# wzf2000/GAMER

Hardware: AMD Instinct MI355X
Metric: train-step sequences/sec, Qwen3Multi SMB decoder, his_len=100 (higher is better)
Workload: dtype f32 tensors/accumulators, products = 3 x fp16 pieces (split3)

## Files before the change

gamer_amd/_lib.py:

```python
from __future__ import annotations

import ctypes as C
import os
import re
from typing import Optional

import torch

_HERE = os.path.dirname(os.path.abspath(__file__))
LIB_PATH = os.path.join(_HERE, "lib", "libgamer_hip.so")
if os.environ.get("GAMER_LIB_PATH"):
    LIB_PATH = os.path.abspath(os.environ["GAMER_LIB_PATH"])
HEADER_PATH = os.path.join(os.path.dirname(_HERE), "include", "gamer_hip.h")

_lib: Optional[C.CDLL] = None

c_void_p, c_int, c_float, c_int64, c_uint64 = C.c_void_p, C.c_int, C.c_float, C.c_int64, C.c_uint64


class GemmDesc(C.Structure):
    _fields_ = [
        ("A", c_void_p), ("a_rs", c_int64), ("a_ks", c_int64),
        ("B", c_void_p), ("b_rs", c_int64), ("b_ks", c_int64),
        ("C", c_void_p), ("ldc", c_int64),
        ("M", c_int), ("N", c_int), ("K", c_int),
        ("alpha", c_float),
        ("accumulate", c_int),
        ("groups", c_int),
        ("group_mode", c_int),
        ("group_offsets", c_void_p),
        ("strideB", c_int64), ("strideC", c_int64),
        ("kchunk", c_int),
        ("resid", c_void_p),
        ("row_map", c_void_p),
        ("p_drop", c_float),
        ("seed", c_uint64),
        ("rowdot_other", c_void_p),
        ("rowdot_out", c_void_p),
        ("rowdot_S", c_int),
        ("qk_wq", c_void_p), ("qk_wk", c_void_p),
        ("qk_eps", c_float),
        ("qk_cos", c_void_p), ("qk_sin", c_void_p),
        ("qk_bias_q", c_void_p), ("qk_bias_k", c_void_p), ("qk_bias_v", c_void_p),
        ("qk_act_idx", c_void_p),
        ("qk_pos_ids", c_void_p),
        ("qk_q_rot", c_void_p), ("qk_k_rot", c_void_p),
        ("qk_S", c_int), ("qk_nq", c_int), ("qk_nkv", c_int),
        ("b_planes", c_void_p), ("b_plane_stride", c_int64),
        ("amax_a", c_void_p), ("amax_b", c_void_p),
        ("amax_c", c_void_p), ("amax_c_col0", c_int),
        ("wgrad_ws", c_void_p), ("wgrad_ws_floats", c_int64),
        ("sw_gu", c_void_p), ("sw_ld", c_int64),
        ("group_div", c_int), ("sw_tbl", c_void_p), ("b_planes_t", c_void_p),
        ("sw_hm", c_void_p), ("sw_row_group", c_void_p),
        ("norm_x", c_void_p), ("norm_w", c_void_p), ("norm_eps", c_float),
        ("norm_dst_rows", c_void_p), ("norm_src_rows", c_void_p),
        ("bias_idx", c_void_p), ("bias_q", c_void_p), ("bias_k", c_void_p), ("bias_v", c_void_p),
        ("bias_rows", c_int), ("bias_nq", c_int), ("bias_nkv", c_int),
    ]


class GemmBf16Desc(C.Structure):
    _fields_ = [
        ("A", c_void_p), ("lda", c_int64),
        ("B", c_void_p), ("ldb", c_int64),
        ("C", c_void_p), ("ldc", c_int64),
        ("M", c_int), ("N", c_int), ("K", c_int),
        ("accumulate", c_int),
        ("groups", c_int),
        ("group_mode", c_int),
        ("group_offsets", c_void_p),
        ("strideB", c_int64), ("strideC", c_int64),
        ("kchunk", c_int),
        ("resid", c_void_p),
        ("row_map", c_void_p),
        ("p_drop", c_float),
        ("seed", c_uint64),
        ("rowdot_other", c_void_p),
        ("rowdot_out", c_void_p),
        ("rowdot_S", c_int),
        ("qk_wq", c_void_p), ("qk_wk", c_void_p), ("qk_eps", c_float),
        ("qk_cos", c_void_p), ("qk_sin", c_void_p),
        ("qk_bias_q", c_void_p), ("qk_bias_k", c_void_p), ("qk_bias_v", c_void_p),
        ("qk_act_idx", c_void_p), ("qk_pos_ids", c_void_p),
        ("qk_q_rot", c_void_p), ("qk_k_rot", c_void_p),
        ("qk_S", c_int), ("qk_nq", c_int), ("qk_nkv", c_int),
        ("sw_gu", c_void_p), ("sw_ld", c_int64),
        ("wgrad_ws", c_void_p), ("wgrad_ws_floats", c_int64),
    ]


P, I, F, L, U = c_void_p, c_int, c_float, c_int64, c_uint64

_SIGNATURES = {
    "gamer_router_fwd": [P, P, P, P, I, I, I, I, I, I, P, P, P, P, P, P, P, P, P, P, P, P],
    "gamer_expert_lists": [P, I, I, I, P, P, P, P, P],
    "gamer_causal_prep": [P, I, I, P, P, P, P, P, P],
    "gamer_session_prep": [P, P, P, I, I, I, I, P, P, P, P, P, P, P],
    "gamer_moe_router_prep": [P, P, P, I, P, I, I, I, I, I, I, I, P, P, P, P, P, P, P, P, P],
    "gamer_embedding_fwd": [P, P, I, I, I, P, P],
    "gamer_embedding_bwd": [P, P, I, I, I, I, P, P],
    "gamer_embedding_bwd_ordered": [P, P, I, I, I, I, P, P, L, P],
    "gamer_embedding_bwd_ordered_ws_bytes": [I, I, I],
    "gamer_rmsnorm_fwd": [P, P, I, I, F, P, P, I, P],
    "gamer_rmsnorm_bwd": [P, P, P, I, P, I, I, F, I, P, P, I, P, P, F, U, P],
    "gamer_colsum_reduce": [P, I, I, I, P, P],
    "gamer_colsum_reduce_batched": [P, L, I, I, I, P, I, P],
    "gamer_rowtable_fwd": [P, P, P, I, I, P, I, I, P],
    "gamer_rowtable_bwd": [P, I, I, P, P, I, I, I, P, P, L, P],
    "gamer_gemm_f32": [C.POINTER(GemmDesc), P],
    "gamer_gemm_f32_split": [C.POINTER(GemmDesc), c_int, P],
    "gamer_split3_guard": [I],
    "gamer_gemm_bf16": [C.POINTER(GemmBf16Desc), P],
    "gamer_cast_params_bf16": [P, P, P, P, I, I, P],
    "gamer_attn_fwd_bf16": [P, I, P, I, P, I, P, P, I, I, I, I, F, F, U, P, P, P, P, P, P, P],
    "gamer_attn_bwd_bf16": [P, I, P, I, P, I, P, P, P, P, P, I, I, I, I, F, F, U, P, P, I, P, I, P, I, P, I, P, P, P, P],
    "gamer_session_spans": [P, P, P, P, P, I, I, I, I, P, P, P, P, P, P, P, P, P],
    "gamer_qknorm_rope_fwd": [P, I, I, I, I, P, P, F, P, P, P, P, P, P, P, P, P, P],
    "gamer_qknorm_rope_bwd": [P, P, P, I, I, I, I, P, P, F, P, P, P, P, P, I, P, P, P, P, P, P, P, P, L, P],
    "gamer_attn_row_order": [P, I, I, P, P, P, P],
    "gamer_attn_fwd": [P, I, P, I, P, I, P, P, P, P, I, I, I, I, F, F, U, P, P, P, P, P, I, P, P],
    "gamer_attn_bwd": [P, I, P, I, P, I, P, P, P, P, P, P, P, I, I, I, I, F, F, U, P, P, I, P, I, P, I, P, P, P, P, P, I, P],
    "gamer_split3_planes": [P, P, L, L, P],
    "gamer_absmax_f32": [P, I, L, I, I, L, P, P],
    "gamer_absmax_multi_f32": [P, P, I, P, P],
    "gamer_split2h_planes_multi": [P, P, I, P, P, P],
    "gamer_amax_sink": [P, P],
    "gamer_amax_sink3": [P, P, P],
    "gamer_attn_split_amax": [P, P, P, P],
    "gamer_attn_fwd_split": [P, I, P, I, P, I, P, P, P, I, I, I, I, F, F, U, P, P, P, P, P, I, P, P],
    "gamer_attn_bwd_split": [P, I, P, I, P, I, P, P, P, P, P, P, P, I, I, I, I, F, F, U, P, P, I, P, I, P, I, P, P, P, I, P, P, P],
    "gamer_residual_dropout_fwd": [P, P, P, I, I, F, U, P, P],
    "gamer_residual_dropout_bwd": [P, P, I, I, F, U, P, P],
    "gamer_swiglu_fwd": [P, P, L, F, U, P, P],
    "gamer_swiglu_bwd": [P, P, P, L, F, U, P],
    "gamer_swiglu_fwd_ld": [P, L, I, I, F, U, P, P],
    "gamer_swiglu_bwd_ld": [P, L, I, I, P, F, U, P],
    "gamer_swiglu_fwd_ld_tbl": [P, L, I, I, F, U, P, P, P, P],
    "gamer_pba_router": [P, I, I, I, I, I, I, I, P, I, I, I, I, I, P, P, P, P, P],
    "gamer_relu_tbl_fwd": [P, L, I, I, F, U, P, P, P, I, P],
    "gamer_relu_tbl_bwd": [P, L, I, I, P, F, U, P, P, I, P],
# ... 156 lines not shown
```

gamer_amd/csrc/common.h:

```cpp
#pragma once
#include <hip/hip_runtime.h>
#include <stdint.h>
#include <stdio.h>
#include <stdarg.h>
#include <stdlib.h>
#include <atomic>
#include <type_traits>

#include "../../include/gamer_hip.h"

namespace gamer {

void set_error(const char* fmt, ...);

#define GAMER_CHECK_ARG(cond, ...)                       \
    do {                                                 \
        if (!(cond)) {                                   \
            gamer::set_error(__VA_ARGS__);               \
            return -1;                                   \
        }                                                \
    } while (0)

#define GAMER_CHECK_LAUNCH(name)                                                        \
    do {                                                                                \
// ... 221 lines not shown
struct AttnDropout {
    uint32_t k0, k1, thr;
    float scale;
    __device__ __forceinline__ AttnDropout(float p, uint64_t seed) {
        k0 = mix32((uint32_t)seed ^ 0x9e3779b9U) ^ mix32((uint32_t)(seed >> 32) + 0x7f4a7c15U);
        k1 = mix32(k0 + 0x632be5abU);
        const float t = p * 4294967296.f;
        thr = t >= 4294967040.f ? 0xffffffffU : (uint32_t)t;
        scale = p > 0.f ? 1.f / (1.f - p) : 1.f;
    }
    __device__ __forceinline__ uint32_t row_word(uint32_t row) const {
        return (mix32(row * 0x9e3779b1U + k0) & 0xffffffU) | 0x800001U;
    }
    __device__ __forceinline__ uint32_t key_word(uint32_t j) const { return mix32(j * 0x85ebca6bU + k1) & 0xffffffU; }
    __device__ __forceinline__ bool keep(uint32_t a, uint32_t b) const { return __umul24(a, b) >= thr; }
};

__device__ __forceinline__ float xor32_max(float v) {
    const auto sw = __builtin_amdgcn_permlane32_swap(__float_as_uint(v), __float_as_uint(v), false, false);
    return fmaxf(__uint_as_float(sw[0]), __uint_as_float(sw[1]));
}
__device__ __forceinline__ float xor32_sum(float v) {
    const auto sw = __builtin_amdgcn_permlane32_swap(__float_as_uint(v), __float_as_uint(v), false, false);
    return __uint_as_float(sw[0]) + __uint_as_float(sw[1]);
}

__device__ __forceinline__ int wave_sum_i32(int v) {
#pragma unroll
    for (int o = 32; o > 0; o >>= 1) v += __shfl_xor(v, o, 64);
    return v;
}
__device__ __forceinline__ int wave_max_i32(int v) {
#pragma unroll
    for (int o = 32; o > 0; o >>= 1) v = max(v, __shfl_xor(v, o, 64));
    return v;
}
__device__ __forceinline__ int wave_min_i32(int v) {
#pragma unroll
    for (int o = 32; o > 0; o >>= 1) v = min(v, __shfl_xor(v, o, 64));
    return v;
}

#define GAMER_DPP_ROW_REDUCE(OP, v)                                                                   \
    v = OP(v, __builtin_amdgcn_update_dpp(v, v, 0xB1, 0xf, 0xf, false));      \
    v = OP(v, __builtin_amdgcn_update_dpp(v, v, 0x4E, 0xf, 0xf, false));      \
    v = OP(v, __builtin_amdgcn_update_dpp(v, v, 0x141, 0xf, 0xf, false));         \
    v = OP(v, __builtin_amdgcn_update_dpp(v, v, 0x140, 0xf, 0xf, false));
__device__ __forceinline__ int wave_min_i32_dpp(int v) {
    GAMER_DPP_ROW_REDUCE(min, v)
    return min(min(__builtin_amdgcn_readlane(v, 0), __builtin_amdgcn_readlane(v, 16)),
               min(__builtin_amdgcn_readlane(v, 32), __builtin_amdgcn_readlane(v, 48)));
}
__device__ __forceinline__ int wave_max_i32_dpp(int v) {
    GAMER_DPP_ROW_REDUCE(max, v)
    return max(max(__builtin_amdgcn_readlane(v, 0), __builtin_amdgcn_readlane(v, 16)),
               max(__builtin_amdgcn_readlane(v, 32), __builtin_amdgcn_readlane(v, 48)));
}

__device__ __forceinline__ float row16_sum_dpp(float v) {
#define GAMER_DPP_F(ctrl) __int_as_float(__builtin_amdgcn_update_dpp(__float_as_int(v), __float_as_int(v), ctrl, 0xf, 0xf, false))
    v += GAMER_DPP_F(0xB1);
    v += GAMER_DPP_F(0x4E);
    v += GAMER_DPP_F(0x141);
    v += GAMER_DPP_F(0x140);
#undef GAMER_DPP_F
    return v;
}

__device__ __forceinline__ float sigmoid_f(float x) { return __builtin_amdgcn_rcpf(1.f + __expf(-x)); }
__device__ __forceinline__ float silu_f(float x) { return x * sigmoid_f(x); }
__device__ __forceinline__ float dsilu_f(float x) {
    const float s = sigmoid_f(x);
    return s * (1.f + x * (1.f - s));
}

bool gemm_as_eligible(const gamer_gemm_desc* d, bool a_kc, bool b_kc, const uint16_t* b_planes);
int launch_gemm_as(const gamer_gemm_desc* d, const uint16_t* b_planes, bool b_kc, hipStream_t st);
int launch_gemm_bias_rows(const gamer_gemm_desc* d, hipStream_t st);
bool gemm_os_eligible(const gamer_gemm_desc* d, bool a_kc, bool b_kc, const uint16_t* b_planes);
int launch_gemm_os(const gamer_gemm_desc* d, const uint16_t* b_planes, int guard, hipStream_t st, bool fwd_t = false);
bool gemm_os_fwd_eligible(const gamer_gemm_desc* d, bool a_kc, bool b_kc);
bool gemm_wg_eligible(const gamer_gemm_desc* d, bool a_kc, bool b_kc);
int launch_gemm_wg(const gamer_gemm_desc* d, hipStream_t st);

int launch_wgrad_reduce(const float* ws, float* C, int64_t ldc, int M, int N, int groups, const int32_t* group_offsets, int K,
                        int kchunk, int64_t strideC, hipStream_t st);

}
```

gamer_amd/csrc/gemm.hip:

```cpp
#include "common.h"
#include <stdlib.h>

namespace gamer {

constexpr int BM = 128, BN = 128, BK = 32;
constexpr int GEMM_THREADS = 256;
constexpr int KC_LD = BK + 4;
constexpr int TILE_FLOATS = BM * KC_LD;
constexpr int GEMM_LDS_BYTES = 4 * TILE_FLOATS * (int)sizeof(float);

typedef float f32x16 __attribute__((ext_vector_type(16)));

constexpr int SP_KC_ROW = 80;
constexpr int SP_KC_IMG = BM * SP_KC_ROW;
constexpr int SP_RC_IMG = BK * 256;
constexpr int SP_OPERAND = 3 * SP_KC_IMG;
constexpr int SP_LDS_BYTES = 2 * SP_OPERAND;

#ifndef SP_ABLATE
#define SP_ABLATE 0
#endif
__device__ __forceinline__ uint32_t pack_hi16(uint32_t w0, uint32_t w1) { return __builtin_amdgcn_perm(w1, w0, 0x07060302u); }
__device__ __forceinline__ void split3(float x, uint32_t (&w)[3]) {
    if (SP_ABLATE & 1) { w[0] = w[1] = w[2] = __float_as_uint(x); return; }
// ... 105 lines not shown
__device__ __forceinline__ bf16x8 read_frag_half(const unsigned char* __restrict__ img, int rbase, int lane) {
    const int r32 = lane & 31, h = lane >> 5;
    if (KC) {
        return *reinterpret_cast<const bf16x8*>(img + (rbase + r32) * SPH_KC_ROW + (h << 4));
    } else {
        const int q = (lane >> 2) & 3, pp = lane & 3, gsel = (lane >> 4) & 1;
        const int row = rbase + 16 * gsel + 4 * pp;
        bf16x8 out;
#pragma unroll
        for (int c = 0; c < 2; ++c) {
            const int k = 8 * h + 4 * c + q;
            const bf16x4 v = __builtin_amdgcn_ds_read_tr16_b64_v4bf16(
                (bf16x4 __attribute__((address_space(3)))*)(img + sp_rc_off(k, row)));
            out[4 * c + 0] = v[0]; out[4 * c + 1] = v[1]; out[4 * c + 2] = v[2]; out[4 * c + 3] = v[3];
        }
        return out;
    }
}

template <bool KC>
__device__ __forceinline__ bf16x8 read_frag_split(const unsigned char* __restrict__ img, int rbase, int sub, int lane) {
    const int r32 = lane & 31, h = lane >> 5;
    if (KC) {
        return *reinterpret_cast<const bf16x8*>(img + (rbase + r32) * SP_KC_ROW + ((2 * sub + h) << 4));
    } else {
        const int q = (lane >> 2) & 3, pp = lane & 3, gsel = (lane >> 4) & 1;
        const int row = rbase + 16 * gsel + 4 * pp;
        bf16x8 out;
#pragma unroll
        for (int c = 0; c < 2; ++c) {
            const int k = 16 * sub + 8 * h + 4 * c + q;
            const bf16x4 v = __builtin_amdgcn_ds_read_tr16_b64_v4bf16(
                (bf16x4 __attribute__((address_space(3)))*)(img + sp_rc_off(k, row)));
            out[4 * c + 0] = v[0]; out[4 * c + 1] = v[1]; out[4 * c + 2] = v[2]; out[4 * c + 3] = v[3];
        }
        return out;
    }
}

__device__ unsigned long long* g_gemm_stamp = nullptr;
__device__ __forceinline__ unsigned long long stamp_now() {
    unsigned long long t;
    asm volatile("s_memtime %0\n\ts_waitcnt lgkmcnt(0)" : "=s"(t) :: "memory");
    return t;
}

struct GemmParams {
    const float* A; int64_t a_rs, a_ks;
    const float* B; int64_t b_rs, b_ks;
    float* C; int64_t ldc;
    int M, N, K;
    float alpha;
    int accumulate;
    int groups;
    const int32_t* group_offsets;
    int64_t strideB, strideC;
    int kchunk;
    int m_tiles, n_tiles;
    const float* resid;
    const int32_t* row_map;
    float p_drop;
    uint64_t seed;
    const float* rowdot_other;
    float* rowdot_out;
    int rowdot_S;
    const float* qk_wq; const float* qk_wk;
    float qk_eps;
    const float* qk_cos; const float* qk_sin;
    const float* qk_bias_q; const float* qk_bias_k; const float* qk_bias_v;
    const int32_t* qk_act_idx;
    const int32_t* qk_pos_ids;
    float* qk_q_rot; float* qk_k_rot;
    int qk_S, qk_nq, qk_nkv;
    const uint32_t* amax_a; const uint32_t* amax_b;
    const uint16_t* b_planes;
    int64_t b_plane_stride;
    int guard;
    uint32_t* amax_c;
    int amax_c_col0;
    float* wgrad_ws;
    float* sw_gu; int64_t sw_ld;
    int group_div;
    const float* sw_tbl;
};

constexpr float SPLIT3_GUARD_RATIO = 1.f / 65536.f;
#ifndef GAMER_GEMM_CAMAX_BUILD
#define GAMER_GEMM_CAMAX_BUILD 1
#endif
#ifndef GAMER_SPLIT3_GUARD_BUILD
#define GAMER_SPLIT3_GUARD_BUILD 1
#endif
static int g_split3_guard = 1;

__device__ __forceinline__ int xcd_remap(int id, int n) {
    const int q = n >> 3, r = n & 7;
    const int xcd = id & 7, idx = id >> 3;
    const int base = xcd < r ? xcd * (q + 1) : r * (q + 1) + (xcd - r) * q;
    return base + idx;
}

template <bool INTERIOR>
__device__ __forceinline__ void load_kc(const float* __restrict__ p, int64_t rs, int row0, int row_end, int k0,
                                        int k_end, int tid, float4 (&r)[4]) {
#pragma unroll
    for (int j = 0; j < 4; ++j) {
        const int f = tid + GEMM_THREADS * j;
        const int row = row0 + (f >> 3);
        const int k = k0 + ((f & 7) << 2);
        if (INTERIOR) {
            r[j] = *reinterpret_cast<const float4*>(p + (int64_t)row * rs + k);
            continue;
        }
        float4 v = make_float4(0.f, 0.f, 0.f, 0.f);
        if (row < row_end && k < k_end) {
            v = *reinterpret_cast<const float4*>(p + (int64_t)row * rs + k);
            if (k + 3 >= k_end) {
                if (k + 1 >= k_end) v.y = 0.f;
                if (k + 2 >= k_end) v.z = 0.f;
                v.w = 0.f;
            }
        }
        r[j] = v;
    }
}
template <bool INTERIOR>
__device__ __forceinline__ void load_rc(const float* __restrict__ p, int64_t ks, int row0, int row_end, int k0,
                                        int k_end, int tid, float4 (&r)[4]) {
#pragma unroll
    for (int j = 0; j < 4; ++j) {
        const int f = tid + GEMM_THREADS * j;
        const int k = k0 + (f >> 5);
        const int row = row0 + ((f & 31) << 2);
        if (INTERIOR) {
            r[j] = *reinterpret_cast<const float4*>(p + (int64_t)k * ks + row);
            continue;
        }
        float4 v = make_float4(0.f, 0.f, 0.f, 0.f);
        if (k < k_end && row < row_end) {
            v = *reinterpret_cast<const float4*>(p + (int64_t)k * ks + row);
            if (row + 3 >= row_end) {
                if (row + 1 >= row_end) v.y = 0.f;
                if (row + 2 >= row_end) v.z = 0.f;
                v.w = 0.f;
            }
        }
        r[j] = v;
    }
}
__device__ __forceinline__ void store_kc(float* __restrict__ lds, int tid, const float4 (&r)[4]) {
#pragma unroll
    for (int j = 0; j < 4; ++j) {
        const int f = tid + GEMM_THREADS * j;
        *reinterpret_cast<float4*>(lds + (f >> 3) * KC_LD + ((f & 7) << 2)) = r[j];
    }
}
__device__ __forceinline__ void store_rc(float* __restrict__ lds, int tid, const float4 (&r)[4]) {
#pragma unroll
    for (int j = 0; j < 4; ++j) {
        const int f = tid + GEMM_THREADS * j;
        *reinterpret_cast<float4*>(lds + (f >> 5) * BM + ((f & 31) << 2)) = r[j];
    }
}

template <bool KC>
__device__ __forceinline__ void read_frag(const float* __restrict__ lds, int row, int kk, int h, float (&f)[4]) {
    if (KC) {
        const float4 v = *reinterpret_cast<const float4*>(lds + row * KC_LD + 8 * kk + 4 * h);
        f[0] = v.x; f[1] = v.y; f[2] = v.z; f[3] = v.w;
    } else {
#pragma unroll
        for (int s = 0; s < 4; ++s) f[s] = lds[(8 * kk + 4 * h + s) * BM + row];
    }
}

template <bool A_KC, bool B_KC, int MODE, bool ACCUM, bool STAMP, int NBUF, int EPI, int SPLIT = 0, bool PP = false>
__device__ __forceinline__ void
gemm_f32_tile(const GemmParams& p, float* __restrict__ smem_all, const int vblock, const int vgrid) {

    const int grp = PP ? (int)(threadIdx.x >> 8) : 0;
    const int tid = threadIdx.x & (GEMM_THREADS - 1);
    float* const smem = smem_all + (PP ? grp * (GEMM_LDS_BYTES / 4) : 0);
    const int lane = tid & 63;
    const int wid = tid >> 6;
    const int wm = wid >> 1, wn = wid & 1;
    const int r32 = lane & 31, h = lane >> 5;

    const int Lx = xcd_remap(vblock, vgrid);
    const int L = (PP && MODE == 0) ? 2 * Lx + grp : Lx;

    int row0, row_end;
    int col0;
    int kbeg, kend;
    const float* Bp = p.B;
    const float* Bsrc = p.B;
    float* Cp = p.C;
    int64_t ws_block = 0;
    int tile_group = 0;
    if (MODE == 0) {
        const int mt = L / p.n_tiles;
        col0 = (L % p.n_tiles) * BN;
        int g = 0, seg_beg = 0, seg_end = p.M, tiles_before = 0;
        bool found = false;
        if (p.group_offsets) {
            int prev = p.group_offsets[0];
            for (int gi = 0; gi < p.groups; ++gi) {
                const int nxt = p.group_offsets[gi + 1];
                const int tiles = (nxt - prev + BM - 1) / BM;
                if (!found && mt < tiles_before + tiles) {
                    g = gi; seg_beg = prev; seg_end = nxt; found = true;
                }
                if (!found) tiles_before += tiles;
                prev = nxt;
            }
        } else {
            found = mt < (p.M + BM - 1) / BM;
        }
        if (!found) return;
        row0 = seg_beg + (mt - tiles_before) * BM;
        row_end = seg_end;
        kbeg = 0;
        kend = p.K;
        tile_group = g;
        Bp += (int64_t)(g / p.group_div) * p.strideB;
        Bsrc = Bp;
        if (SPLIT == 3 && p.b_planes) Bp = reinterpret_cast<const float*>(p.b_planes) + (Bp - p.B);
    } else {
        const int tiles_mn = p.m_tiles * p.n_tiles;
        const int per_chunk = PP ? (tiles_mn + 1) / 2 : tiles_mn;
        const int chunk = L / per_chunk;
        const int tile = PP ? 2 * (L % per_chunk) + grp : L % per_chunk;
        if (PP && tile >= tiles_mn) return;
        ws_block = (int64_t)chunk * tiles_mn + tile;
        row0 = (tile / p.n_tiles) * BM;
        row_end = p.M;
        col0 = (tile % p.n_tiles) * BN;
        int g = 0, seg_beg = 0, seg_end = p.K, chunks_before = 0;
        bool found = false;
        if (p.group_offsets) {
            int prev = p.group_offsets[0];
            for (int gi = 0; gi < p.groups; ++gi) {
                const int nxt = p.group_offsets[gi + 1];
                const int chunks = (nxt - prev + p.kchunk - 1) / p.kchunk;
                if (!found && chunk < chunks_before + chunks) {
                    g = gi; seg_beg = prev; seg_end = nxt; found = true;
                }
                if (!found) chunks_before += chunks;
                prev = nxt;
            }
        } else {
            found = chunk < (p.K + p.kchunk - 1) / p.kchunk;
        }
        if (!found) return;
        kbeg = seg_beg + (chunk - chunks_before) * p.kchunk;
        kend = min(seg_end, kbeg + p.kchunk);
        Cp += (int64_t)g * p.strideC;
    }
    const int col_end = p.N;

    f32x16 acc[2][2];
#pragma unroll
    for (int i = 0; i < 2; ++i)
#pragma unroll
        for (int j = 0; j < 2; ++j)
#pragma unroll
            for (int r = 0; r < 16; ++r) acc[i][j][r] = 0.f;

    const int nkt = (kend - kbeg + BK - 1) / BK;
    const bool a_in = row0 + BM <= row_end, b_in = col0 + BN <= col_end;
    float4 ra[4], rb[4];
    float scale_a = 1.f, scale_b = 1.f, unscale = 1.f;
    constexpr bool GUARD = GAMER_SPLIT3_GUARD_BUILD && SPLIT == 3 && MODE == 0 && A_KC && !PP && !STAMP;
    float rmax[4] = {0.f, 0.f, 0.f, 0.f};
    uint32_t amax_a_bits = 0;
    if (SPLIT == 3) {
        float ia, ib;
        amax_a_bits = amax_read(p.amax_a);
        scale_from_amax(amax_a_bits, scale_a, ia);
        scale_from_amax(amax_read(p.amax_b), scale_b, ib);
        unscale = ia * ib;
    }
    auto load_tile = [&](int k0) {
        const bool k_in = k0 + BK <= kend;
        if (a_in && k_in) {
            if (A_KC) load_kc<true>(p.A, p.a_rs, row0, row_end, k0, kend, tid, ra);
            else load_rc<true>(p.A, p.a_ks, row0, row_end, k0, kend, tid, ra);
        } else {
            if (A_KC) load_kc<false>(p.A, p.a_rs, row0, row_end, k0, kend, tid, ra);
            else load_rc<false>(p.A, p.a_ks, row0, row_end, k0, kend, tid, ra);
        }
        if (b_in && k_in) {
            if (B_KC) load_kc<true>(Bp, p.b_rs, col0, col_end, k0, kend, tid, rb);
            else load_rc<true>(Bp, p.b_ks, col0, col_end, k0, kend, tid, rb);
        } else {
            if (B_KC) load_kc<false>(Bp, p.b_rs, col0, col_end, k0, kend, tid, rb);
            else load_rc<false>(Bp, p.b_ks, col0, col_end, k0, kend, tid, rb);
        }
    };
    constexpr int H2_B_OFF = 2 * (A_KC ? SP_KC_IMG : SP_RC_IMG);
    constexpr int H2_STAGE = H2_B_OFF + 2 * (B_KC ? SP_KC_IMG : SP_RC_IMG);
    auto store_tile_from = [&](float* dst, const float4 (&qa)[4], const float4 (&qb)[4]) {
        if (SPLIT == 3) {
            unsigned char* d8 = reinterpret_cast<unsigned char*>(dst);
            if (A_KC) store_kc_h2(d8, tid, qa, scale_a); else store_rc_h2(d8, tid, qa, scale_a);
            if (GUARD) {
#pragma unroll
// ... 397 lines not shown
            if (wave_live) {
                const int ar0 = row0 + wm * 64 + r32, bc0 = col0 + wn * 64 + r32;
#pragma unroll 1
                for (int k = kbeg; k < kend; k += 2) {
                    const int kk = k + h;
                    const bool kin = kk < kend;
                    float av[2], bv[2];
#pragma unroll
                    for (int i = 0; i < 2; ++i) {
                        const int row = ar0 + i * 32;
                        av[i] = (kin && row < row_end) ? p.A[(int64_t)row * p.a_rs + kk] : 0.f;
                    }
#pragma unroll
                    for (int j = 0; j < 2; ++j) {
                        const int col = bc0 + j * 32;
                        bv[j] = (kin && col < col_end) ? (B_KC ? Bsrc[(int64_t)col * p.b_rs + kk] : Bsrc[(int64_t)kk * p.b_ks + col]) : 0.f;
                    }
#pragma unroll
                    for (int i = 0; i < 2; ++i)
#pragma unroll
                        for (int j = 0; j < 2; ++j)
                            acc[i][j] = __builtin_amdgcn_mfma_f32_32x32x2f32(av[i], bv[j], acc[i][j], 0, 0, 0);
                }
            }
        }
    }

    const bool interior = a_in && b_in;
    const float alpha_eff = (SPLIT == 3 && !redo) ? p.alpha * unscale : p.alpha;
    if (MODE == 0 && (NBUF == 2 || SPLIT) && interior && (p.ldc & 3) == 0) {
        float* patch = smem + wid * (64 * 68);
        float4 oth[EPI == 2 ? 16 : 1];
        if (EPI == 2) {
            const float* ob = p.rowdot_other + (int64_t)(row0 + wm * 64 + (lane >> 4)) * p.ldc + col0 + wn * 64 + ((lane & 15) << 2);
#pragma unroll
            for (int it = 0; it < 16; ++it) oth[it] = *reinterpret_cast<const float4*>(ob + (int64_t)it * 4 * p.ldc);
        }
        if (SPLIT != 3 && p.alpha == 1.f) {
#pragma unroll
            for (int i = 0; i < 2; ++i)
#pragma unroll
                for (int j = 0; j < 2; ++j)
#pragma unroll
                    for (int r = 0; r < 16; ++r)
                        patch[(i * 32 + (r & 3) + 8 * (r >> 2) + 4 * h) * 68 + j * 32 + r32] = acc[i][j][r];
        } else {
#pragma unroll
            for (int i = 0; i < 2; ++i)
#pragma unroll
                for (int j = 0; j < 2; ++j)
#pragma unroll
                    for (int r = 0; r < 16; ++r)
                        patch[(i * 32 + (r & 3) + 8 * (r >> 2) + 4 * h) * 68 + j * 32 + r32] = alpha_eff * acc[i][j][r];
        }
        __builtin_amdgcn_s_waitcnt(0xc07f);
        const int c4 = (lane & 15) << 2;
        const DropoutRng rng((EPI == 1 || EPI == 4) ? p.p_drop : 0.f, p.seed);
        const int row_first = row0 + wm * 64 + (lane >> 4);
        const int col = col0 + wn * 64 + c4;
        float* dst0 = Cp + (int64_t)row_first * p.ldc + col;
        const int64_t step = 4 * p.ldc;
        const int qk_pos0 = EPI == 3 ? row_first % max(p.qk_S, 1) : 0;
        const bool amax_on = GAMER_GEMM_CAMAX_BUILD && p.amax_c != nullptr && !ACCUM && col0 + wn * 64 >= p.amax_c_col0;
        float cmax = 0.f;
        int pre_rc[EPI == 1 ? 16 : 1];
        float4 pre_x[EPI == 1 ? 16 : (EPI == 4 ? 8 : 1)], pre_b[EPI == 4 ? 8 : 1];
        if (EPI == 1) {
            if (p.row_map) {
#pragma unroll
                for (int it = 0; it < 16; ++it) pre_rc[it] = p.row_map[row_first + 4 * it];
            } else {
#pragma unroll
                for (int it = 0; it < 16; ++it) pre_rc[it] = row_first + 4 * it;
            }
#pragma unroll
            for (int it = 0; it < 16; ++it) pre_x[it] = *reinterpret_cast<const float4*>(p.resid + (int64_t)pre_rc[it] * p.ldc + col);
        }
        float4 tb_g = make_float4(0.f, 0.f, 0.f, 0.f), tb_u = tb_g;
        if (EPI == 4 && p.sw_tbl) {
            const float* tb = p.sw_tbl + (int64_t)tile_group * 2 * p.N + col;
            tb_g = *reinterpret_cast<const float4*>(tb);
            tb_u = *reinterpret_cast<const float4*>(tb + p.N);
        }
        auto pre_sw = [&](int it0) {
#pragma unroll
            for (int it = 0; it < 8; ++it) {
                const float* ga = p.sw_gu + (int64_t)(row_first + 4 * (it0 + it)) * p.sw_ld + col;
                pre_x[EPI == 4 ? it : 0] = *reinterpret_cast<const float4*>(ga);
                pre_b[EPI == 4 ? it : 0] = *reinterpret_cast<const float4*>(ga + p.N);
            }
        };
        if (EPI == 4) pre_sw(0);
#pragma unroll
        for (int it = 0; it < 16; ++it) {
            if (EPI == 4 && it == 8) pre_sw(8);
            const int lr = (lane >> 4) + 4 * it;
            const float4 v = *reinterpret_cast<const float4*>(patch + lr * 68 + c4);
            if (EPI == 3) {
                const int row = row_first + 4 * it;
                const int hd = (col0 + wn * 64) >> 6;
                const int g = lane & 15;
                float4 x = v;
                const bool cross = p.qk_bias_q != nullptr;
                const int a = cross ? p.qk_act_idx[row] : 0;
                if (hd < p.qk_nq + p.qk_nkv) {
                    const bool isq = hd < p.qk_nq;
                    if (cross) {
                        const float4 b4 = isq ? reinterpret_cast<const float4*>(p.qk_bias_q + (int64_t)a * p.qk_nq * 64 + hd * 64)[g]
                                              : reinterpret_cast<const float4*>(p.qk_bias_k + (int64_t)a * p.qk_nkv * 64 + (hd - p.qk_nq) * 64)[g];
                        x.x += b4.x; x.y += b4.y; x.z += b4.z; x.w += b4.w;
                    }
                    *reinterpret_cast<float4*>(dst0 + it * step) = x;
                    float ss = x.x * x.x + x.y * x.y + x.z * x.z + x.w * x.w;
                    ss = row16_sum_dpp(ss);
                    const float rstd = rsqrtf(ss * (1.f / 64.f) + p.qk_eps);
                    const float4 w4 = reinterpret_cast<const float4*>(isq ? p.qk_wq : p.qk_wk)[g];
                    float4 y;
                    y.x = w4.x * (x.x * rstd); y.y = w4.y * (x.y * rstd); y.z = w4.z * (x.z * rstd); y.w = w4.w * (x.w * rstd);
                    float4 pr;
                    pr.x = __shfl_xor(y.x, 8, 64); pr.y = __shfl_xor(y.y, 8, 64); pr.z = __shfl_xor(y.z, 8, 64); pr.w = __shfl_xor(y.w, 8, 64);
                    int pos = qk_pos0 + 4 * it;
                    if (p.qk_S >= 64) pos = pos >= p.qk_S ? pos - p.qk_S : pos;
                    else pos %= p.qk_S;
                    if (p.qk_pos_ids) pos = p.qk_pos_ids[row];
                    const float4 cc = reinterpret_cast<const float4*>(p.qk_cos + pos * 64)[g];
                    const float4 sn = reinterpret_cast<const float4*>(p.qk_sin + pos * 64)[g];
                    const float sgn = g < 8 ? -1.f : 1.f;
                    float4 o;
                    o.x = y.x * cc.x + sgn * pr.x * sn.x; o.y = y.y * cc.y + sgn * pr.y * sn.y;
                    o.z = y.z * cc.z + sgn * pr.z * sn.z; o.w = y.w * cc.w + sgn * pr.w * sn.w;
                    float* rot = isq ? p.qk_q_rot + (int64_t)row * p.qk_nq * 64 + hd * 64
                                     : p.qk_k_rot + (int64_t)row * p.qk_nkv * 64 + (hd - p.qk_nq) * 64;
                    *reinterpret_cast<float4*>(rot + 4 * g) = o;
                } else {
                    if (cross) {
                        const float4 b4 = reinterpret_cast<const float4*>(p.qk_bias_v + (int64_t)a * p.qk_nkv * 64 +
                                                                          (hd - p.qk_nq - p.qk_nkv) * 64)[g];
                        x.x += b4.x; x.y += b4.y; x.z += b4.z; x.w += b4.w;
                    }
                    *reinterpret_cast<float4*>(dst0 + it * step) = x;
                }
            } else if (EPI == 4) {
                const int row = row_first + 4 * it;
                float* ga = p.sw_gu + (int64_t)row * p.sw_ld + col;
                float* ua = ga + p.N;
                float4 a = pre_x[EPI == 4 ? (it & 7) : 0], b = pre_b[EPI == 4 ? (it & 7) : 0];
                a.x += tb_g.x; a.y += tb_g.y; a.z += tb_g.z; a.w += tb_g.w;
                b.x += tb_u.x; b.y += tb_u.y; b.z += tb_u.z; b.w += tb_u.w;
                float m[4];
                rng.mult4((uint32_t)(((int64_t)row * p.N + col) >> 2), m);
                const float d0 = m[0] * v.x, d1 = m[1] * v.y, d2 = m[2] * v.z, d3 = m[3] * v.w;
                float4 dg, du;
                dg.x = d0 * b.x * dsilu_f(a.x); du.x = d0 * silu_f(a.x);
                dg.y = d1 * b.y * dsilu_f(a.y); du.y = d1 * silu_f(a.y);
                dg.z = d2 * b.z * dsilu_f(a.z); du.z = d2 * silu_f(a.z);
                dg.w = d3 * b.w * dsilu_f(a.w); du.w = d3 * silu_f(a.w);
                *reinterpret_cast<float4*>(ga) = dg;
                *reinterpret_cast<float4*>(ua) = du;
                if (amax_on) {
                    asm("v_max3_f32 %0, %0, |%1|, |%2|\n\tv_max3_f32 %0, %0, |%3|, |%4|" : "+v"(cmax) : "v"(dg.x), "v"(dg.y), "v"(dg.z), "v"(dg.w));
                    asm("v_max3_f32 %0, %0, |%1|, |%2|\n\tv_max3_f32 %0, %0, |%3|, |%4|" : "+v"(cmax) : "v"(du.x), "v"(du.y), "v"(du.z), "v"(du.w));
                }
            } else if (EPI == 1) {
                const int64_t e = (int64_t)pre_rc[EPI == 1 ? it : 0] * p.ldc + col;
                float* dst = Cp + e;
                const float4 x = pre_x[EPI == 1 ? it : 0];
                float m[4];
                rng.mult4((uint32_t)(e >> 2), m);
                float4 o;
                o.x = x.x + m[0] * v.x; o.y = x.y + m[1] * v.y; o.z = x.z + m[2] * v.z; o.w = x.w + m[3] * v.w;
                *reinterpret_cast<float4*>(dst) = o;
            } else {
                float* dst = dst0 + it * step;
                if (EPI != 1 && EPI != 3 && amax_on)
                    asm("v_max3_f32 %0, %0, |%1|, |%2|\n\tv_max3_f32 %0, %0, |%3|, |%4|" : "+v"(cmax) : "v"(v.x), "v"(v.y), "v"(v.z), "v"(v.w));
                if (EPI == 2) {
                    const float4 o4 = oth[EPI == 2 ? it : 0];
                    float d = v.x * o4.x + v.y * o4.y + v.z * o4.z + v.w * o4.w;
                    d = row16_sum_dpp(d);
                    if ((lane & 15) == 0) {
                        const int row = row_first + 4 * it;
                        const int heads = p.N >> 6, head = (col0 + wn * 64) >> 6;
                        p.rowdot_out[((int64_t)(row / p.rowdot_S) * heads + head) * p.rowdot_S + row % p.rowdot_S] = d;
                    }
                }
                if (ACCUM) {
                    float4 o = *reinterpret_cast<const float4*>(dst);
                    o.x += v.x; o.y += v.y; o.z += v.z; o.w += v.w;
                    *reinterpret_cast<float4*>(dst) = o;
                } else {
                    *reinterpret_cast<float4*>(dst) = v;
                }
            }
        }
        if (EPI != 1 && EPI != 3 && amax_on) {
            uint32_t mw = __float_as_uint(cmax);
#pragma unroll
            for (int o2 = 32; o2 > 0; o2 >>= 1) mw = max(mw, (uint32_t)__shfl_xor((int)mw, o2, 64));
            if (lane == 0 && mw) amax_publish(mw, p.amax_c, (uint32_t)(vblock * 4 + wid));
        }
    } else if (MODE == 1 && p.wgrad_ws != nullptr) {
        float* blk = p.wgrad_ws + ws_block * (int64_t)(BM * BN);
#pragma unroll
        for (int i = 0; i < 2; ++i)
#pragma unroll
            for (int j = 0; j < 2; ++j) {
                const int lc = wn * 64 + j * 32 + r32;
                const int lr0 = wm * 64 + i * 32 + 4 * h;
#pragma unroll
                for (int r = 0; r < 16; ++r) blk[(lr0 + (r & 3) + 8 * (r >> 2)) * BN + lc] = alpha_eff * acc[i][j][r];
            }
    } else {
        float emax = 0.f;
        if (EPI == 4 && p.sw_tbl != nullptr) {
            const float* tb0 = p.sw_tbl + (int64_t)tile_group * 2 * p.N;
            const int nr = min(BM, row_end - row0), nc = min(BN, p.N - col0);
            for (int i = threadIdx.x; i < nr * nc; i += GEMM_THREADS) {
                const int rr = row0 + i / nc, cc = col0 + i % nc;
                float* ga = p.sw_gu + (int64_t)rr * p.sw_ld + cc;
                ga[0] += tb0[cc];
                ga[p.N] += tb0[p.N + cc];
            }
            __syncthreads();
        }
        auto emit = [&](int row, int col, float v) {
            if (EPI == 4) {
                float* ga = p.sw_gu + (int64_t)row * p.sw_ld + col;
                float a = ga[0], b = ga[p.N];
                const int64_t e = (int64_t)row * p.N + col;
                const DropoutRng rng(p.p_drop, p.seed);
                float m[4];
                rng.mult4((uint32_t)(e >> 2), m);
                const float d = m[e & 3] * v;
                const float dg = d * b * dsilu_f(a), du = d * silu_f(a);
                ga[0] = dg; ga[p.N] = du;
                if (GAMER_GEMM_CAMAX_BUILD && p.amax_c != nullptr) emax = fmaxf(emax, fmaxf(fabsf(dg), fabsf(du)));
                return;
            }
            if (GAMER_GEMM_CAMAX_BUILD && EPI != 1 && MODE == 0 && !ACCUM && p.amax_c != nullptr && col >= p.amax_c_col0) emax = fmaxf(emax, fabsf(v));
            if (EPI == 1) {
                const int64_t rc = p.row_map ? p.row_map[row] : row;
                const int64_t e = rc * p.ldc + col;
                const DropoutRng rng(p.p_drop, p.seed);
                float m[4];
                rng.mult4((uint32_t)(e >> 2), m);
                Cp[e] = p.resid[e] + m[e & 3] * v;
            } else {
                float* dst = Cp + (int64_t)row * p.ldc + col;
                if (MODE == 1) atomicAdd(dst, v);
                else if (ACCUM) *dst += v;
                else *dst = v;
            }
        };
#pragma unroll
        for (int i = 0; i < 2; ++i) {
#pragma unroll
            for (int j = 0; j < 2; ++j) {
                const int col = col0 + wn * 64 + j * 32 + r32;
                const int rbase = row0 + wm * 64 + i * 32 + 4 * h;
                if (interior) {
#pragma unroll
                    for (int r = 0; r < 16; ++r) emit(rbase + (r & 3) + 8 * (r >> 2), col, alpha_eff * acc[i][j][r]);
                } else {
#pragma unroll
                    for (int r = 0; r < 16; ++r) {
                        const int rr = (r & 3) + 8 * (r >> 2);
                        if (rbase + rr < row_end && col < col_end) emit(rbase + rr, col, alpha_eff * acc[i][j][r]);
                    }
                }
            }
        }
        if (GAMER_GEMM_CAMAX_BUILD && MODE == 0 && !ACCUM && p.amax_c != nullptr) {
            uint32_t mw = __float_as_uint(emax);
#pragma unroll
            for (int o2 = 32; o2 > 0; o2 >>= 1) mw = max(mw, (uint32_t)__shfl_xor((int)mw, o2, 64));
            if (lane == 0 && mw) amax_publish(mw, p.amax_c, (uint32_t)(vblock * 4 + wid));
        }
    }
    if (STAMP) {
        unsigned long long* st = g_gemm_stamp;
        if (st && threadIdx.x == 0) {
            const unsigned long long t_end = stamp_now();
            unsigned long long* rec = st + 8ull * vblock;
            rec[0] = t_ph[0]; rec[1] = t_ph[1]; rec[2] = t_ph[2]; rec[3] = t_ph[3];
            rec[4] = t_loop_end - t_begin;
            rec[5] = t_end - t_loop_end;
            rec[6] = t_begin;
            rec[7] = t_end;
        }
    }
}

template <bool A_KC, bool B_KC, int MODE, bool ACCUM, bool STAMP, int NBUF, int EPI, int SPLIT = 0, bool PP = false>
__global__ void __launch_bounds__(PP ? 2 * GEMM_THREADS : GEMM_THREADS, (NBUF == 1 && SPLIT == 0) ? 3 : 2)
gemm_f32_kernel(const GemmParams p, const int vgrid) {
    extern __shared__ __attribute__((aligned(16))) float smem_all[];
    for (int v = blockIdx.x; v < vgrid; v += gridDim.x) {
        gemm_f32_tile<A_KC, B_KC, MODE, ACCUM, STAMP, NBUF, EPI, SPLIT, PP>(p, smem_all, v, vgrid);
        if (v + (int)gridDim.x < vgrid) __syncthreads();
    }
}

template <bool A_KC, bool B_KC, int MODE, bool ACCUM, bool STAMP, int NBUF, int EPI = 0, int SPLIT = 0, bool PP = false>
static int launch_gemm_t(const GemmParams& p, int blocks, hipStream_t st, int lds) {
    static int persist = -1;
    if (persist < 0) { const char* e = getenv("GAMER_GEMM_PERSIST"); persist = e ? atoi(e) : 0; }
    const int grid = (persist > 0 && SPLIT != 0 && !PP && !STAMP && blocks > persist) ? persist : blocks;
    return launch<gemm_f32_kernel<A_KC, B_KC, MODE, ACCUM, STAMP, NBUF, EPI, SPLIT, PP>>("gamer_gemm_f32", dim3(grid), dim3(PP ? 2 * GEMM_THREADS : GEMM_THREADS),
                                                                                        lds, st, p, blocks);
}

template <bool A_KC, bool B_KC, int MODE, int SPLIT>
static int launch_gemm_split(const GemmParams& p, int blocks, hipStream_t st) {
    constexpr int h2_stage = 2 * ((A_KC ? SP_KC_IMG : SP_RC_IMG) + (B_KC ? SP_KC_IMG : SP_RC_IMG));
    const int lds = (SPLIT == 3 && SP_WIDE3 && A_KC && B_KC && 2 * h2_stage > GEMM_LDS_BYTES) ? 2 * h2_stage : GEMM_LDS_BYTES;
    static_assert(SP_LDS_BYTES <= GEMM_LDS_BYTES, "split images must fit the fp32 kernel's LDS allocation");
    const bool acc = MODE == 0 && p.accumulate;
    static int stamp = -1, pp = 0;
    if (stamp < 0) {
        const char* e = getenv("GAMER_GEMM_STAMP");
        stamp = (e && e[0] == '1') ? 1 : 0;
        const char* e2 = getenv("GAMER_GEMM_PP");
        pp = (SP_PINGPONG && e2 && e2[0] == '1') ? 1 : 0;
    }
    (void)pp;
#if SP_PINGPONG
    if ((SPLIT == 6 || SPLIT == 3) && pp && !(MODE == 0 && p.b_planes)) {
        int pblocks;
        if (MODE == 0) pblocks = (blocks + 1) / 2;
        else {
            const int tiles_mn = p.m_tiles * p.n_tiles;
            pblocks = blocks / tiles_mn * ((tiles_mn + 1) / 2);
        }
        const int plds = 2 * GEMM_LDS_BYTES;
        if (stamp) return launch_gemm_t<A_KC, B_KC, MODE, false, true, 2, 0, SPLIT, true>(p, pblocks, st, plds);
        if (MODE == 0 && p.resid) return launch_gemm_t<A_KC, B_KC, MODE, false, false, 2, 1, SPLIT, true>(p, pblocks, st, plds);
        if (MODE == 0 && p.rowdot_out) return launch_gemm_t<A_KC, B_KC, MODE, false, false, 2, 2, SPLIT, true>(p, pblocks, st, plds);
        if (MODE == 0 && A_KC && B_KC && p.qk_q_rot) return launch_gemm_t<A_KC, B_KC, MODE, false, false, 2, 3, SPLIT, true>(p, pblocks, st, plds);
        if (acc) return launch_gemm_t<A_KC, B_KC, MODE, true, false, 2, 0, SPLIT, true>(p, pblocks, st, plds);
        return launch_gemm_t<A_KC, B_KC, MODE, false, false, 2, 0, SPLIT, true>(p, pblocks, st, plds);
    }
#endif
    if (stamp && SPLIT == 6) return launch_gemm_t<A_KC, B_KC, MODE, false, true, 2, 0, SPLIT>(p, blocks, st, lds);
    if constexpr (SPLIT == 3 && MODE == 0 && A_KC) {
        if (p.sw_gu) return launch_gemm_t<A_KC, B_KC, MODE, false, false, 2, 4, SPLIT>(p, blocks, st, lds);
    }
    if (MODE == 0 && p.resid) return launch_gemm_t<A_KC, B_KC, MODE, false, false, 2, 1, SPLIT>(p, blocks, st, lds);
    if (MODE == 0 && p.rowdot_out) return launch_gemm_t<A_KC, B_KC, MODE, false, false, 2, 2, SPLIT>(p, blocks, st, lds);
    if (MODE == 0 && A_KC && B_KC && p.qk_q_rot) return launch_gemm_t<A_KC, B_KC, MODE, false, false, 2, 3, SPLIT>(p, blocks, st, lds);
    if (acc) return launch_gemm_t<A_KC, B_KC, MODE, true, false, 2, 0, SPLIT>(p, blocks, st, lds);
    return launch_gemm_t<A_KC, B_KC, MODE, false, false, 2, 0, SPLIT>(p, blocks, st, lds);
}

template <bool A_KC, bool B_KC, int MODE>
static int launch_gemm(const GemmParams& p, int blocks, hipStream_t st, int split = 0) {
    if (split == 6) return launch_gemm_split<A_KC, B_KC, MODE, 6>(p, blocks, st);
    if (split == 9) return launch_gemm_split<A_KC, B_KC, MODE, 9>(p, blocks, st);
    if (split == 3) return launch_gemm_split<A_KC, B_KC, MODE, 3>(p, blocks, st);
    static int stamp = -1, solo = 0, nbuf = 2;
    if (stamp < 0) {
        const char* e = getenv("GAMER_GEMM_STAMP");
        stamp = (e && e[0] == '1') ? 1 : 0;
        const char* s2 = getenv("GAMER_GEMM_SOLO");
        solo = (s2 && s2[0] == '1') ? 1 : 0;
        const char* s3 = getenv("GAMER_GEMM_NBUF");
        nbuf = (s3 && s3[0] == '1') ? 1 : 2;
    }
    const int lds = solo ? 150 * 1024 : GEMM_LDS_BYTES;
    const bool acc = MODE == 0 && p.accumulate;
    if (stamp) return launch_gemm_t<A_KC, B_KC, MODE, false, true, 2>(p, blocks, st, lds);
    if (MODE == 0 && p.resid) return launch_gemm_t<A_KC, B_KC, MODE, false, false, 2, 1>(p, blocks, st, lds);
    if (MODE == 0 && p.rowdot_out) return launch_gemm_t<A_KC, B_KC, MODE, false, false, 2, 2>(p, blocks, st, lds);
    if (MODE == 0 && A_KC && B_KC && p.qk_q_rot) return launch_gemm_t<A_KC, B_KC, MODE, false, false, 2, 3>(p, blocks, st, lds);
    if (nbuf == 1) {
        const int lds1 = 2 * TILE_FLOATS * (int)sizeof(float);
        if (acc) return launch_gemm_t<A_KC, B_KC, MODE, true, false, 1>(p, blocks, st, lds1);
        return launch_gemm_t<A_KC, B_KC, MODE, false, false, 1>(p, blocks, st, lds1);
    }
    if (acc) return launch_gemm_t<A_KC, B_KC, MODE, true, false, 2>(p, blocks, st, lds);
    return launch_gemm_t<A_KC, B_KC, MODE, false, false, 2>(p, blocks, st, lds);
}

__global__ void __launch_bounds__(256)
wgrad_reduce_kernel(const float* __restrict__ ws, float* __restrict__ C, int64_t ldc, int M, int N, int m_tiles, int n_tiles,
                    int groups, const int32_t* __restrict__ group_offsets, int K, int kchunk, int64_t strideC) {
    const int tiles_mn = m_tiles * n_tiles;
    int id = blockIdx.x;
    const int strip = id & 15; id >>= 4;
    const int tile = id % tiles_mn, g = id / tiles_mn;
    int c_beg = 0, c_n;
    if (group_offsets) {
        int prev = group_offsets[0];
        c_n = 0;
        for (int gi = 0; gi <= g; ++gi) {
            const int nxt = group_offsets[gi + 1];
            const int chunks = (nxt - prev + kchunk - 1) / kchunk;
            if (gi < g) c_beg += chunks; else c_n = chunks;
            prev = nxt;
        }
    } else {
        c_n = (K + kchunk - 1) / kchunk;
    }
    const int lr = strip * 8 + (threadIdx.x >> 5), lc = (threadIdx.x & 31) << 2;
    const float4* src = reinterpret_cast<const float4*>(ws + ((int64_t)c_beg * tiles_mn + tile) * (int64_t)(BM * BN) + lr * BN + lc);
    const int64_t step4 = (int64_t)tiles_mn * (BM * BN) / 4;
    float4 s = make_float4(0.f, 0.f, 0.f, 0.f);
    int c = 0;
    for (; c + 4 <= c_n; c += 4) {
        const float4 a0 = src[(int64_t)c * step4], a1 = src[(int64_t)(c + 1) * step4], a2 = src[(int64_t)(c + 2) * step4],
                     a3 = src[(int64_t)(c + 3) * step4];
        s.x = (((s.x + a0.x) + a1.x) + a2.x) + a3.x; s.y = (((s.y + a0.y) + a1.y) + a2.y) + a3.y;
        s.z = (((s.z + a0.z) + a1.z) + a2.z) + a3.z; s.w = (((s.w + a0.w) + a1.w) + a2.w) + a3.w;
    }
    for (; c < c_n; ++c) {
        const float4 a0 = src[(int64_t)c * step4];
        s.x += a0.x; s.y += a0.y; s.z += a0.z; s.w += a0.w;
    }
    const int row = (tile / n_tiles) * BM + lr, col = (tile % n_tiles) * BN + lc;
    if (row < M && c_n > 0) {
        float* dst = C + (int64_t)g * strideC + (int64_t)row * ldc + col;
        const float v[4] = {s.x, s.y, s.z, s.w};
#pragma unroll
        for (int e = 0; e < 4; ++e)
            if (col + e < N) dst[e] += v[e];
    }
}

int launch_wgrad_reduce(const float* ws, float* C, int64_t ldc, int M, int N, int groups, const int32_t* group_offsets, int K,
// ... 2 lines not shown
    const int64_t rblocks = (int64_t)groups * m_tiles * n_tiles * 16;
    hipLaunchKernelGGL(wgrad_reduce_kernel, dim3((int)rblocks), dim3(256), 0, st, ws, C, ldc, M, N, m_tiles, n_tiles, groups,
                       group_offsets, K, kchunk, strideC);
    return (int)hipGetLastError();
}

__global__ void __launch_bounds__(256)
split3_planes_kernel(const float4* __restrict__ x, uint16_t* __restrict__ planes, int64_t n4, int64_t stride) {
    for (int64_t i = (int64_t)blockIdx.x * 256 + threadIdx.x; i < n4; i += (int64_t)gridDim.x * 256) {
        uint2 img[3];
        split3_quad(x[i], img);
#pragma unroll
        for (int s = 0; s < 3; ++s) *reinterpret_cast<uint2*>(planes + s * stride + 4 * i) = img[s];
    }
}

}

using namespace gamer;

extern "C" int gamer_split3_planes(const float* x, gamer_bf16* planes, int64_t n, int64_t plane_stride, void* stream) {
    GAMER_CHECK_ARG(x && planes && n > 0 && n % 4 == 0 && plane_stride >= n && plane_stride % 4 == 0 && aligned16(x) &&
                    (reinterpret_cast<uintptr_t>(planes) & 7u) == 0,
                    "gamer_split3_planes: n=%lld and plane_stride=%lld must be multiples of 4 (stride >= n), x 16-byte and planes 8-byte aligned",
                    (long long)n, (long long)plane_stride);
    const int64_t n4 = n / 4;
    int blocks = (int)((n4 + 255) / 256);
    if (blocks > 4096) blocks = 4096;
    hipLaunchKernelGGL(split3_planes_kernel, dim3(blocks), dim3(256), 0, (hipStream_t)stream, reinterpret_cast<const float4*>(x),
                       reinterpret_cast<uint16_t*>(planes), n4, plane_stride);
    GAMER_CHECK_LAUNCH("gamer_split3_planes");
    return 0;
}

extern "C" int gamer_debug_gemm_stamp(void* p) {
    unsigned long long* v = (unsigned long long*)p;
    return (int)hipMemcpyToSymbol(HIP_SYMBOL(g_gemm_stamp), &v, sizeof(v));
}

static inline bool diag_build_switches() {
    static EnvSwitch stamp("GAMER_GEMM_STAMP"), nbuf("GAMER_GEMM_NBUF");
    return stamp.is_set() || nbuf.is_set();
}
static inline bool diag_pp_switch() { static EnvSwitch pp("GAMER_GEMM_PP"); return pp.is_set(); }
static int gemm_entry(const gamer_gemm_desc* d, void* stream, int split) {
    GAMER_CHECK_ARG(d, "gamer_gemm_f32: null descriptor");
    GAMER_CHECK_ARG(d->A && d->B && d->C, "gamer_gemm_f32: null matrix pointer");
    GAMER_CHECK_ARG(d->M > 0 && d->N > 0 && d->K > 0, "gamer_gemm_f32: bad shape M=%d N=%d K=%d", d->M, d->N, d->K);
    GAMER_CHECK_ARG((d->a_rs == 1) != (d->a_ks == 1) || (d->a_rs == 1 && d->a_ks == 1 && (d->M == 1 || d->K == 1)),
                    "gamer_gemm_f32: exactly one of a_rs/a_ks must be 1 (rs=%lld ks=%lld)", (long long)d->a_rs, (long long)d->a_ks);
    GAMER_CHECK_ARG((d->b_rs == 1) != (d->b_ks == 1) || (d->b_rs == 1 && d->b_ks == 1 && (d->N == 1 || d->K == 1)),
                    "gamer_gemm_f32: exactly one of b_rs/b_ks must be 1 (rs=%lld ks=%lld)", (long long)d->b_rs, (long long)d->b_ks);
    const bool a_kc = d->a_ks == 1, b_kc = d->b_ks == 1;
    const int64_t a_ld = a_kc ? d->a_rs : d->a_ks, b_ld = b_kc ? d->b_rs : d->b_ks;
    GAMER_CHECK_ARG(a_ld % 4 == 0 && b_ld % 4 == 0 && d->ldc >= d->N,
                    "gamer_gemm_f32: leading dims must be multiples of 4 (lda=%lld ldb=%lld ldc=%lld)",
                    (long long)a_ld, (long long)b_ld, (long long)d->ldc);
    GAMER_CHECK_ARG(aligned16(d->A) && aligned16(d->B), "gamer_gemm_f32: A and B must be 16-byte aligned");
    GAMER_CHECK_ARG(d->groups >= 1 && (d->groups == 1 || d->group_offsets), "gamer_gemm_f32: groups=%d needs group_offsets", d->groups);
    GAMER_CHECK_ARG(d->strideB % 4 == 0, "gamer_gemm_f32: strideB must be a multiple of 4");
    GAMER_CHECK_ARG(d->group_mode == 0 || d->group_mode == 1, "gamer_gemm_f32: group_mode=%d", d->group_mode);

    GemmParams p;
    p.A = d->A; p.a_rs = d->a_rs; p.a_ks = d->a_ks;
    p.B = d->B; p.b_rs = d->b_rs; p.b_ks = d->b_ks;
    p.C = d->C; p.ldc = d->ldc;
    p.M = d->M; p.N = d->N; p.K = d->K;
    p.alpha = d->alpha; p.accumulate = d->accumulate;
    p.groups = d->groups; p.group_offsets = d->group_offsets;
    p.strideB = d->strideB; p.strideC = d->strideC;
    p.kchunk = d->kchunk;
    p.resid = d->resid; p.row_map = d->row_map; p.p_drop = d->p_drop; p.seed = d->seed;
    p.rowdot_other = d->rowdot_other; p.rowdot_out = d->rowdot_out; p.rowdot_S = d->rowdot_S;
    p.qk_wq = d->qk_wq; p.qk_wk = d->qk_wk; p.qk_eps = d->qk_eps; p.qk_cos = d->qk_cos; p.qk_sin = d->qk_sin;
    p.qk_bias_q = d->qk_bias_q; p.qk_bias_k = d->qk_bias_k; p.qk_bias_v = d->qk_bias_v;
    p.qk_act_idx = d->qk_act_idx; p.qk_pos_ids = d->qk_pos_ids; p.qk_q_rot = d->qk_q_rot; p.qk_k_rot = d->qk_k_rot;
    p.qk_S = d->qk_S; p.qk_nq = d->qk_nq; p.qk_nkv = d->qk_nkv;
    p.amax_a = d->amax_a; p.amax_b = d->amax_b;
    p.guard = g_split3_guard;
    p.amax_c = d->amax_c; p.amax_c_col0 = d->amax_c_col0;
    p.wgrad_ws = nullptr;
    p.sw_gu = d->sw_gu; p.sw_ld = d->sw_ld;
    p.group_div = d->group_div > 1 ? d->group_div : 1; p.sw_tbl = d->sw_tbl;
    GAMER_CHECK_ARG(d->group_div <= 1 || (d->group_mode == 0 && d->group_offsets && d->groups % d->group_div == 0),
                    "gamer_gemm_f32: group_div = %d needs group_mode 0, group_offsets and groups (%d) a multiple of it", d->group_div, d->groups);
    GAMER_CHECK_ARG(!d->sw_tbl || ((d->sw_gu || d->sw_hm) && aligned16(d->sw_tbl)),
                    "gamer_gemm_f32: sw_tbl is an option of the SwiGLU epilogues (sw_gu, sw_hm)");
    GAMER_CHECK_ARG(!d->sw_gu || (split == 3 && d->group_mode == 0 && !d->accumulate && !d->resid && !d->rowdot_out && !d->qk_q_rot &&
                                  d->alpha == 1.f && d->N % 4 == 0 && d->sw_ld >= 2 * (int64_t)d->N && d->sw_ld % 4 == 0 &&
                                  aligned16(d->sw_gu) && d->p_drop >= 0.f && d->p_drop < 1.f),
                    "gamer_gemm_f32: the SwiGLU-backward epilogue (sw_gu) is built for gamer_gemm_f32_split(terms = 3), a plain input-"
                    "gradient GEMM with alpha = 1, N %% 4 == 0, sw_ld >= 2 N (N=%d sw_ld=%lld)", d->N, (long long)d->sw_ld);
    GAMER_CHECK_ARG(!d->amax_c || (d->group_mode == 0 && !d->accumulate && !d->resid && !d->qk_q_rot && d->amax_c_col0 >= 0 &&
                                   d->amax_c_col0 % 64 == 0),
                    "gamer_gemm_f32: amax_c needs a plain or row-dot Linear-forward / input-gradient GEMM (no accumulate, residual or "
                    "q|k|v epilogue) and amax_c_col0 a multiple of 64 (amax_c_col0=%d)", d->amax_c_col0);
    GAMER_CHECK_ARG(split != 3 || (d->amax_a && d->amax_b), "gamer_gemm_f32_split: terms = 3 needs amax_a and amax_b (gamer_absmax_f32)");
    p.b_planes = (split && d->group_mode == 0) ? (const uint16_t*)d->b_planes : nullptr;
    p.b_plane_stride = d->b_plane_stride;
    GAMER_CHECK_ARG(!p.b_planes || split == 3 || ((reinterpret_cast<uintptr_t>(p.b_planes) & 7u) == 0 && d->b_plane_stride % 4 == 0 && d->b_plane_stride > 0),
                    "gamer_gemm_f32_split: b_planes must be 8-byte aligned with b_plane_stride %% 4 == 0");
    GAMER_CHECK_ARG(!p.b_planes || split != 3 || (reinterpret_cast<uintptr_t>(p.b_planes) & 15u) == 0,
                    "gamer_gemm_f32_split: terms = 3 takes b_planes as packed pieces at B's offsets (16-byte aligned)");
    if (split == 3 && p.b_planes && ((b_kc ? d->K : d->N) % 4) != 0) p.b_planes = nullptr;
    GAMER_CHECK_ARG(!d->qk_q_rot || (d->qk_k_rot && d->qk_wq && d->qk_wk && d->qk_cos && d->qk_sin && d->group_mode == 0 &&
                                     d->groups == 1 && a_kc && b_kc && !d->resid && !d->rowdot_out && !d->accumulate &&
                                     d->alpha == 1.f && d->M % BM == 0 && d->qk_nq > 0 && d->qk_nkv > 0 && d->qk_S > 0 &&
                                     d->N == (d->qk_nq + 2 * d->qk_nkv) * 64 && d->N % BN == 0 && d->ldc % 4 == 0 &&
                                     aligned16(d->C) && aligned16(d->qk_q_rot) && aligned16(d->qk_k_rot) &&
                                     (!d->qk_bias_q || (d->qk_bias_k && d->qk_bias_v && d->qk_act_idx)) &&
                                     !diag_build_switches()),
                    "gamer_gemm_f32: the q|k|v epilogue needs a Linear-forward layout, one group, M %% 128 == 0 (M=%d), "
                    "N = (nq + 2 nkv) * 64 a multiple of 128 (N=%d), alpha = 1 and no other epilogue", d->M, d->N);
    GAMER_CHECK_ARG(!d->rowdot_out || (d->rowdot_other && d->rowdot_S > 0 && d->group_mode == 0 && d->groups == 1 &&
                                       !d->resid && !d->accumulate && d->M % BM == 0 && d->N % BN == 0 &&
                                       d->M % d->rowdot_S == 0 && d->ldc % 4 == 0 && aligned16(d->rowdot_other) &&
                                       aligned16(d->C) && !diag_build_switches()),
                    "gamer_gemm_f32: the row-dot epilogue needs full 128 x 128 tiles (M=%d N=%d), one group, ldc %% 4 == 0",
                    d->M, d->N);
    GAMER_CHECK_ARG(!d->resid || (d->group_mode == 0 && !d->accumulate && a_kc && b_kc && d->ldc % 4 == 0 &&
                                  aligned16(d->resid) && aligned16(d->C) && d->p_drop >= 0.f && d->p_drop < 1.f),
                    "gamer_gemm_f32: the fused residual epilogue needs a Linear-forward layout, ldc %% 4 == 0, no accumulate");
    GAMER_CHECK_ARG(!d->sw_hm || (d->group_mode == 0 && a_kc && b_kc && !d->accumulate && !d->resid && !d->rowdot_out && !d->qk_q_rot &&
                                  !d->sw_gu && d->alpha == 1.f && d->N % 8 == 0 && d->ldc >= d->N && d->ldc % 4 == 0 && aligned16(d->sw_hm) &&
                                  aligned16(d->C) && (!d->sw_tbl || d->sw_row_group) && d->p_drop >= 0.f && d->p_drop < 1.f),
                    "gamer_gemm_f32: the SwiGLU-forward epilogue (sw_hm) needs a Linear-forward layout with N = 2 I (N=%d), alpha = 1, no other "
                    "epilogue, and sw_row_group with sw_tbl", d->N);
    GAMER_CHECK_ARG(!d->norm_x || (d->norm_w && d->group_mode == 0 && a_kc && b_kc && d->norm_eps > 0.f && d->K % 4 == 0 && d->K <= 1024 &&
                                   aligned16(d->norm_x) && aligned16(d->norm_w) &&
                                   (d->norm_dst_rows != nullptr) == (d->norm_src_rows != nullptr)),
                    "gamer_gemm_f32: the RMSNorm prologue (norm_x) needs a Linear-forward layout, norm_w, norm_eps > 0, K %% 4 == 0 (K=%d) "
                    "and norm_dst_rows / norm_src_rows both or neither", d->K);
    GAMER_CHECK_ARG(!d->bias_idx || (d->bias_q && d->bias_k && d->bias_v && d->group_mode == 0 && d->groups == 1 && a_kc && b_kc &&
                                     !d->accumulate && !d->resid && !d->rowdot_out && !d->qk_q_rot && !d->sw_gu && !d->sw_hm &&
                                     d->bias_rows >= 1 && d->bias_nq > 0 && d->bias_nkv > 0 && d->bias_nq % 4 == 0 && d->bias_nkv % 4 == 0 &&
                                     d->N == d->bias_nq + 2 * d->bias_nkv && d->ldc % 4 == 0 && aligned16(d->C) && aligned16(d->bias_q) &&
                                     aligned16(d->bias_k) && aligned16(d->bias_v)),
                    "gamer_gemm_f32: the bias-row epilogue (bias_idx) needs a plain Linear-forward GEMM with one group, three tables and "
                    "N = bias_nq + 2 bias_nkv in multiples of 4 (N=%d)", d->N);
    if (split == 3 && gemm_as_eligible(d, a_kc, b_kc, p.b_planes)) return launch_gemm_as(d, p.b_planes, b_kc, (hipStream_t)stream);
    if (d->norm_x || d->bias_idx) {
        gamer_gemm_desc d2 = *d;
        if (d->norm_x) {
            if (d->amax_a) gamer_amax_sink(const_cast<uint32_t*>(d->amax_a), nullptr);
            GAMER_TRY(gamer_rmsnorm_fwd(d->norm_x, d->norm_w, d->M, d->K, d->norm_eps, d->norm_dst_rows, const_cast<float*>(d->A), (int)d->a_rs,
                                        stream));
            d2.norm_x = nullptr; d2.norm_w = nullptr; d2.norm_dst_rows = nullptr; d2.norm_src_rows = nullptr;
        }
        if (d->bias_idx) { d2.bias_idx = nullptr; d2.amax_c = nullptr; }
        GAMER_TRY(gemm_entry(&d2, stream, split));
        return d->bias_idx ? launch_gemm_bias_rows(d, (hipStream_t)stream) : 0;
    }
    if (d->sw_hm) {
        gamer_gemm_desc d2 = *d;
        d2.sw_hm = nullptr; d2.sw_row_group = nullptr; d2.sw_tbl = nullptr; d2.amax_c = nullptr;
        const int rc = gemm_entry(&d2, stream, split);
        if (rc) return rc;
        if (d->amax_c) gamer_amax_sink(d->amax_c, nullptr);
        return d->sw_tbl ? gamer_swiglu_fwd_ld_tbl(d->C, d->ldc, d->M, d->N / 2, d->p_drop, d->seed, d->sw_hm, d->sw_tbl, d->sw_row_group, stream)
                         : gamer_swiglu_fwd_ld(d->C, d->ldc, d->M, d->N / 2, d->p_drop, d->seed, d->sw_hm, stream);
    }
    if (split == 3 && gemm_os_eligible(d, a_kc, b_kc, p.b_planes)) return launch_gemm_os(d, p.b_planes, g_split3_guard, (hipStream_t)stream);
    if (split == 3 && gemm_os_fwd_eligible(d, a_kc, b_kc))
        return launch_gemm_os(d, reinterpret_cast<const uint16_t*>(d->b_planes_t), g_split3_guard, (hipStream_t)stream, true);
    p.n_tiles = (d->N + BN - 1) / BN;
    hipStream_t st = (hipStream_t)stream;

    if (d->group_mode == 0) {
        p.m_tiles = (d->M + BM - 1) / BM + (d->group_offsets ? d->groups : 0);
        const int64_t blocks = (int64_t)p.m_tiles * p.n_tiles;
        GAMER_CHECK_ARG(blocks < (1LL << 31), "gamer_gemm_f32: grid too large");
        if (a_kc && b_kc) return launch_gemm<true, true, 0>(p, (int)blocks, st, split);
        if (a_kc && !b_kc) return launch_gemm<true, false, 0>(p, (int)blocks, st, split);
        if (!a_kc && !b_kc) return launch_gemm<false, false, 0>(p, (int)blocks, st, split);
        GAMER_CHECK_ARG(false, "gamer_gemm_f32: layout (A row-contiguous, B k-contiguous) is not built");
    } else {
        GAMER_CHECK_ARG(!a_kc && !b_kc, "gamer_gemm_f32: group_mode 1 (wgrad) needs row-contiguous A and B");
        GAMER_CHECK_ARG(d->kchunk >= BK && d->kchunk % BK == 0, "gamer_gemm_f32: kchunk=%d must be a positive multiple of 32", d->kchunk);
        p.m_tiles = (d->M + BM - 1) / BM;
        const int64_t chunks = (d->K + d->kchunk - 1) / d->kchunk + (d->group_offsets ? d->groups : 0);
        const int64_t blocks = chunks * p.m_tiles * p.n_tiles;
        GAMER_CHECK_ARG(blocks < (1LL << 31), "gamer_gemm_f32: grid too large");
        p.wgrad_ws = d->wgrad_ws;
        if (p.wgrad_ws) {
            const int64_t need = chunks * p.m_tiles * p.n_tiles * (int64_t)(BM * BN);
            GAMER_CHECK_ARG(d->wgrad_ws_floats >= need && aligned16(d->wgrad_ws),
                            "gamer_gemm_f32: wgrad_ws holds %lld floats, this weight gradient needs %lld (chunks x tiles x 16384)",
                            (long long)d->wgrad_ws_floats, (long long)need);
            GAMER_CHECK_ARG(!diag_pp_switch(), "gamer_gemm_f32: the deterministic weight gradient is not built for the ping-pong form");
        }
        const int rc = (split == 3 && p.wgrad_ws && gemm_wg_eligible(d, a_kc, b_kc)) ? launch_gemm_wg(d, st)
                                                                                     : launch_gemm<false, false, 1>(p, (int)blocks, st, split);
        if (rc || !p.wgrad_ws) return rc;
        const int64_t rblocks = (int64_t)d->groups * p.m_tiles * p.n_tiles * 16;
        hipLaunchKernelGGL(wgrad_reduce_kernel, dim3((int)rblocks), dim3(256), 0, st, p.wgrad_ws, d->C, d->ldc, d->M, d->N, p.m_tiles,
                           p.n_tiles, d->groups, d->group_offsets, d->K, d->kchunk, d->strideC);
        GAMER_CHECK_LAUNCH("gamer_gemm_f32/wgrad_reduce");
        return 0;
    }
    return 0;
}

__device__ __forceinline__ uint32_t amax4(uint32_t m, const uint4 v) {
    return max(max(m, v.x & 0x7fffffffu), max(max(v.y & 0x7fffffffu, v.z & 0x7fffffffu), v.w & 0x7fffffffu));
}
__device__ __forceinline__ void amax_commit(uint32_t m, uint32_t* __restrict__ out) {
    __shared__ uint32_t part[4];
#pragma unroll
    for (int o = 32; o > 0; o >>= 1) m = max(m, (uint32_t)__shfl_xor((int)m, o, 64));
    if ((threadIdx.x & 63) == 0) part[threadIdx.x >> 6] = m;
    __syncthreads();
    if (threadIdx.x == 0) {
        m = max(max(part[0], part[1]), max(part[2], part[3]));
        if (m) amax_publish(m, out, blockIdx.x);
    }
}
__global__ void __launch_bounds__(256)
absmax_flat_kernel(const uint4* __restrict__ x, int64_t n4, uint32_t* __restrict__ out) {
    uint32_t m = 0;
    const int64_t step = (int64_t)gridDim.x * 256;
    int64_t i = (int64_t)blockIdx.x * 256 + threadIdx.x;
    for (; i + step < n4; i += 2 * step) {
        const uint4 a = x[i], b = x[i + step];
        m = amax4(amax4(m, a), b);
    }
    if (i < n4) m = amax4(m, x[i]);
    amax_commit(m, out);
}
__global__ void __launch_bounds__(256)
absmax_rows_kernel(const float* __restrict__ x, int batch, int64_t stride, int rows, int cols, int64_t ld, uint32_t* __restrict__ out) {
    const int lane = threadIdx.x & 63;
    const int64_t waves = (int64_t)gridDim.x * 4, nrows = (int64_t)batch * rows;
    uint32_t m = 0;
    for (int64_t w = (int64_t)blockIdx.x * 4 + (threadIdx.x >> 6); w < nrows; w += waves) {
        const int64_t b = w / rows, r = w - b * rows;
        const float* src = x + b * stride + r * ld;
        for (int c = lane << 2; c < cols; c += 256) {
            if (c + 3 < cols) m = amax4(m, *reinterpret_cast<const uint4*>(src + c));
            else for (int q = 0; c + q < cols; ++q) m = max(m, __float_as_uint(src[c + q]) & 0x7fffffffu);
        }
    }
    amax_commit(m, out);
}
extern "C" int gamer_absmax_f32(const float* x, int batch, int64_t stride, int rows, int cols, int64_t ld, uint32_t* out, void* stream) {
    GAMER_CHECK_ARG(x && out && batch >= 1 && rows >= 1 && cols >= 1 && ld >= cols && ld % 4 == 0 && stride % 4 == 0 &&
                    (reinterpret_cast<uintptr_t>(x) & 15u) == 0, "gamer_absmax_f32: bad arguments (rows=%d cols=%d ld=%lld)",
                    rows, cols, (long long)ld);
    if (ld == cols && (batch == 1 || stride == (int64_t)rows * ld)) {
        const int64_t n4 = (int64_t)batch * rows * cols / 4;
        int64_t blocks = (n4 + 511) / 512;
        if (blocks < 1) blocks = 1;
        if (blocks > 2048) blocks = 2048;
        hipLaunchKernelGGL(absmax_flat_kernel, dim3((int)blocks), dim3(256), 0, (hipStream_t)stream,
                           reinterpret_cast<const uint4*>(x), n4, out);
// ... 101 lines not shown
```

gamer_amd/csrc/gemm_as.hip:

```cpp
#include "common.h"
#include <stdlib.h>
#include <atomic>

namespace gamer {

typedef float f32x16 __attribute__((ext_vector_type(16)));
typedef uint32_t u32x4a __attribute__((ext_vector_type(4)));

#ifndef AS_WAVES
#define AS_WAVES 4
#endif
#ifndef AS_NT
#define AS_NT 1
#endif
#ifndef AS_DEPTH
#define AS_DEPTH 1
#endif
#ifndef AS_ABLATE
#define AS_ABLATE 0
#endif
constexpr int AS_SLAB = 32 * AS_NT;
constexpr int AS_PANEL = AS_SLAB * 64;

__device__ __forceinline__ int as_f(int row) { return (((row >> 1) & 1) << 2) | (((row >> 3) & 1) << 1) | ((row >> 2) & 1); }
__device__ __forceinline__ int as_off(int row, int col) { return row * 64 + ((((col >> 3) ^ as_f(row))) << 3) + (col & 7); }

struct AsParams {
    const float* A; int64_t lda;
    const uint16_t* Wp;
    int64_t ldw;
    float* C; int64_t ldc;
    int M, N, K;
    float alpha;
    const uint32_t* amax_w;
    uint32_t* amax_c; int amax_c_col0;
    int groups; const int32_t* group_offsets; int64_t strideW;
    int accumulate;
    const float* rowdot_other; float* rowdot_out; int rowdot_S;
    float* sw_gu; int64_t sw_ld; float p_drop; uint64_t seed;
    float* hm; const float* tbl; int group_div;
    const float* norm_w; float norm_eps; float* h; int64_t ldh; const int32_t* src_rows; uint32_t* amax_h;
    const int32_t* act_idx; const float* bias_q; const float* bias_k; const float* bias_v; int bias_c1, bias_c2, nb1;
};

template <int KP, bool WRC, int EPI, int NW, bool NORM = false, bool BIAS = false>
__global__ void __launch_bounds__(64 * NW, AS_DEPTH == 2 ? 1 : 8 / NW)
gemm_as_kernel(const AsParams p) {
    static_assert(!(NORM || BIAS) || !WRC, "the norm prologue and the bias epilogue are built for W k-contiguous");
    static_assert(!BIAS || EPI == 0, "the bias epilogue belongs to the plain store");
    constexpr int AS_WAVES_K = NW, AS_THREADS_K = 64 * NW;
    extern __shared__ __attribute__((aligned(16))) unsigned char as_raw[];
    bf16_t* const wimg = reinterpret_cast<bf16_t*>(as_raw);
    __shared__ uint32_t amax_word;
    const int tid = threadIdx.x, lane = tid & 63, w = tid >> 6;
    const int r = lane & 31, h = lane >> 5;
    int row0 = blockIdx.x * (32 * AS_WAVES_K), row_end = p.M, grp = 0;
    if (p.group_offsets) {
        int prev = p.group_offsets[0], tiles_before = 0;
        bool found = false;
        for (int gi = 0; gi < p.groups; ++gi) {
            const int nxt = p.group_offsets[gi + 1];
            const int tiles = (nxt - prev + 32 * AS_WAVES_K - 1) / (32 * AS_WAVES_K);
            if (!found && (int)blockIdx.x < tiles_before + tiles) {
                grp = gi; row0 = prev + ((int)blockIdx.x - tiles_before) * (32 * AS_WAVES_K); row_end = nxt; found = true;
            }
            if (!found) tiles_before += tiles;
            prev = nxt;
        }
        if (!found) return;
    }
    const int m = row0 + w * 32 + r;
    const bool valid_m = m < row_end;
    if (tid == 0) amax_word = 0;

    bf16x8 af[2][KP * 4];
    float row_inv;
    {
        int64_t src_row = valid_m ? m : row_end - 1;
        if (NORM && p.src_rows) src_row = p.src_rows[src_row];
        const float* arow = p.A + src_row * p.lda + 8 * h;
        float4 raw[KP * 8];
#pragma unroll
        for (int s = 0; s < KP * 4; ++s) {
            raw[2 * s] = *reinterpret_cast<const float4*>(arow + 16 * s);
            raw[2 * s + 1] = *reinterpret_cast<const float4*>(arow + 16 * s + 4);
        }
        if constexpr (NORM) {
            float ss = 0.f;
#pragma unroll
            for (int i = 0; i < KP * 8; ++i) ss += raw[i].x * raw[i].x + raw[i].y * raw[i].y + raw[i].z * raw[i].z + raw[i].w * raw[i].w;
            ss = xor32_sum(ss);
            const float rstd = rsqrtf(ss * (1.f / (float)(KP * 64)) + p.norm_eps);
            float* hrow = p.h + (int64_t)m * p.ldh + 8 * h;
            const float* wrow = p.norm_w + 8 * h;
#pragma unroll
            for (int s = 0; s < KP * 4; ++s) {
#pragma unroll
                for (int j = 0; j < 2; ++j) {
                    const float4 w4 = *reinterpret_cast<const float4*>(wrow + 16 * s + 4 * j);
                    float4 x = raw[2 * s + j];
                    x.x = w4.x * (x.x * rstd); x.y = w4.y * (x.y * rstd); x.z = w4.z * (x.z * rstd); x.w = w4.w * (x.w * rstd);
                    raw[2 * s + j] = x;
                    if (valid_m) *reinterpret_cast<float4*>(hrow + 16 * s + 4 * j) = x;
                }
            }
        }
        float mx = 0.f;
#pragma unroll
        for (int i = 0; i < KP * 8; ++i) {
            if (!valid_m) raw[i] = make_float4(0.f, 0.f, 0.f, 0.f);
            mx = fmaxf(fmaxf(fmaxf(mx, fabsf(raw[i].x)), fabsf(raw[i].y)), fmaxf(fabsf(raw[i].z), fabsf(raw[i].w)));
        }
        mx = xor32_max(mx);
        if constexpr (NORM) {
            if (p.amax_h) {
                uint32_t hm = __float_as_uint(mx);
#pragma unroll
                for (int o2 = 16; o2 > 0; o2 >>= 1) hm = max(hm, (uint32_t)__shfl_xor((int)hm, o2, 64));
                if (lane == 0 && hm) amax_publish(hm, p.amax_h, blockIdx.x * AS_WAVES_K + w);
            }
        }
        float s_row = 1.f;
        row_inv = 1.f;
        if (mx > 0.f) scale_from_amax(__float_as_uint(mx), s_row, row_inv);
#pragma unroll
// ... 11 lines not shown
        }
    }
    float w_s, w_inv;
    scale_from_amax(amax_read(p.amax_w), w_s, w_inv);
    const float out_scale = row_inv * w_inv * p.alpha;

    const int n_slabs = (p.N + AS_SLAB - 1) / AS_SLAB;
    constexpr int QPR = KP * 16;
    constexpr int NLD = AS_SLAB * QPR / AS_THREADS_K;
    uint4 rw[NLD], rw2[NLD];
    int lds_off[NLD], nl_[NLD];
    const uint4* wsrc[NLD];
#pragma unroll
    for (int i = 0; i < NLD; ++i) {
        const int f = tid + AS_THREADS_K * i;
        if (!WRC) {
            const int nl = f / QPR, g = f % QPR;
            nl_[i] = nl;
            lds_off[i] = (g >> 4) * AS_PANEL + as_off(nl, (4 * g) & 63);
            wsrc[i] = reinterpret_cast<const uint4*>(p.Wp) + (((int64_t)(grp / p.group_div) * p.strideW + (int64_t)nl * p.ldw + 4 * g) >> 2);
        } else {
            const int k = f / (AS_SLAB / 4), nq = f % (AS_SLAB / 4);
            nl_[i] = 4 * nq;
            lds_off[i] = k * AS_SLAB + 4 * nq;
            wsrc[i] = reinterpret_cast<const uint4*>(p.Wp) + (((int64_t)(grp / p.group_div) * p.strideW + (int64_t)k * p.ldw + 4 * nq) >> 2);
        }
    }
    const int64_t slab_stride = WRC ? (AS_SLAB >> 2) : (((int64_t)AS_SLAB * p.ldw) >> 2);
    auto load_slab_into = [&](int j, uint4 (&dst)[NLD]) {
        const bool full = (j + 1) * AS_SLAB <= p.N;
#pragma unroll
        for (int i = 0; i < NLD; ++i) {
            const uint4* src = wsrc[i] + (int64_t)j * slab_stride;
            if (!full && j * AS_SLAB + nl_[i] >= p.N) src = wsrc[i];
            dst[i] = *src;
        }
    };
    auto store_slab_from = [&](int j, int buf, const uint4 (&rw)[NLD]) {
        bf16_t* img = wimg + buf * (2 * KP * AS_PANEL);
        const bool full = (j + 1) * AS_SLAB <= p.N;
#pragma unroll
        for (int i = 0; i < NLD; ++i) {
            const bool ok = full || j * AS_SLAB + nl_[i] < p.N;
            *reinterpret_cast<uint2*>(img + lds_off[i]) = ok ? make_uint2(rw[i].x, rw[i].y) : make_uint2(0u, 0u);
            *reinterpret_cast<uint2*>(img + KP * AS_PANEL + lds_off[i]) = ok ? make_uint2(rw[i].z, rw[i].w) : make_uint2(0u, 0u);
        }
    };
    auto load_slab = [&](int j) { load_slab_into(j, rw); };
    auto store_slab = [&](int j, int buf) { store_slab_from(j, buf, rw); };
    int row_off[4];
#pragma unroll
    for (int s = 0; s < 4; ++s) row_off[s] = as_off(r, 16 * s + 8 * h);
    const int tr_lane = (8 * h + ((lane >> 2) & 3)) * AS_SLAB + 16 * ((lane >> 4) & 1) + 4 * (lane & 3);
    auto read_tr = [&](const bf16_t* base) -> bf16x8 {
        bf16x8 out;
#pragma unroll
        for (int c = 0; c < 2; ++c) {
            const bf16x4 v = __builtin_amdgcn_ds_read_tr16_b64_v4bf16((bf16x4 __attribute__((address_space(3)))*)(base + c * 4 * AS_SLAB));
            out[4 * c + 0] = v[0]; out[4 * c + 1] = v[1]; out[4 * c + 2] = v[2]; out[4 * c + 3] = v[3];
        }
        return out;
    };
    float hd_dot = 0.f;
    float emax = 0.f;
    float4 gsave[EPI == 5 ? 4 * AS_NT : 1];
    float* const tbl_lds = reinterpret_cast<float*>(as_raw + (size_t)(AS_DEPTH == 2 ? 3 : 2) * 2 * KP * AS_PANEL * sizeof(bf16_t));
    if (EPI == 5 && p.tbl) {
        const float4* src = reinterpret_cast<const float4*>(p.tbl + (int64_t)grp * p.N);
        for (int i = tid; i < p.N / 4; i += AS_THREADS_K) reinterpret_cast<float4*>(tbl_lds)[i] = src[i];
    }
    int bias_row = 0;
    if constexpr (BIAS) {
        const int n4 = p.N >> 2;
        for (int i = tid; i < p.nb1 * n4; i += AS_THREADS_K) {
            const int a = i / n4, c = 4 * (i - a * n4);
            const float* src = c < p.bias_c1 ? p.bias_q + (int64_t)a * p.bias_c1 + c
                             : c < p.bias_c2 ? p.bias_k + (int64_t)a * (p.bias_c2 - p.bias_c1) + (c - p.bias_c1)
                                             : p.bias_v + (int64_t)a * (p.N - p.bias_c2) + (c - p.bias_c2);
            reinterpret_cast<float4*>(tbl_lds)[i] = *reinterpret_cast<const float4*>(src);
        }
        if (valid_m) bias_row = min(max(p.act_idx[m], 0), p.nb1 - 1) * p.N;
    }

    float cmax = 0.f;
    float* crow = p.C + (int64_t)m * p.ldc;
    f32x16 acc[AS_NT];
    auto mfma_slab = [&](const int j, const int buf) {
        const bf16_t* img = wimg + buf * (2 * KP * AS_PANEL);
#pragma unroll
            for (int i = 0; i < 16; ++i)
#pragma unroll
                for (int nt = 0; nt < AS_NT; ++nt) acc[nt][i] = 0.f;
#pragma unroll
            for (int ks = 0; ks < KP * 4; ++ks) {
                const int pn = ks >> 2, s = ks & 3;
#pragma unroll
                for (int nt = 0; nt < AS_NT; ++nt) {
                    bf16x8 w0, w1;
                    if (!WRC) {
                        w0 = *reinterpret_cast<const bf16x8*>(img + pn * AS_PANEL + nt * 32 * 64 + row_off[s]);
                        w1 = *reinterpret_cast<const bf16x8*>(img + (KP + pn) * AS_PANEL + nt * 32 * 64 + row_off[s]);
                    } else {
                        w0 = read_tr(img + ks * 16 * AS_SLAB + nt * 32 + tr_lane);
                        w1 = read_tr(img + KP * AS_PANEL + ks * 16 * AS_SLAB + nt * 32 + tr_lane);
                    }
                    if (AS_ABLATE & 2) { asm volatile("" :: "v"(w0), "v"(w1)); continue; }
                    acc[nt] = __builtin_amdgcn_mfma_f32_32x32x16_f16(__builtin_bit_cast(f16x8, w1), __builtin_bit_cast(f16x8, af[0][ks]), acc[nt], 0, 0, 0);
                    acc[nt] = __builtin_amdgcn_mfma_f32_32x32x16_f16(__builtin_bit_cast(f16x8, w0), __builtin_bit_cast(f16x8, af[1][ks]), acc[nt], 0, 0, 0);
                    acc[nt] = __builtin_amdgcn_mfma_f32_32x32x16_f16(__builtin_bit_cast(f16x8, w0), __builtin_bit_cast(f16x8, af[0][ks]), acc[nt], 0, 0, 0);
                }
            }
    };
    auto epilogue_slab = [&](const int j) {
            float part = 0.f;
            if (valid_m) {
                const bool track = EPI != 5 && p.amax_c != nullptr && j * AS_SLAB >= p.amax_c_col0;
#pragma unroll
                for (int nt = 0; nt < AS_NT; ++nt)
#pragma unroll
                    for (int g4 = 0; g4 < 4; ++g4) {
                        const int col = j * AS_SLAB + nt * 32 + 8 * g4 + 4 * h;
                        if (col < p.N) {
                            float4 t4 = make_float4(acc[nt][4 * g4] * out_scale, acc[nt][4 * g4 + 1] * out_scale,
                                                    acc[nt][4 * g4 + 2] * out_scale, acc[nt][4 * g4 + 3] * out_scale);
                            if (AS_ABLATE & 1) { asm volatile("" :: "v"(t4.x), "v"(t4.y), "v"(t4.z), "v"(t4.w)); continue; }
                            if constexpr (BIAS) {
                                asm volatile("" : "+v"(t4.x), "+v"(t4.y), "+v"(t4.z), "+v"(t4.w));
                                const float4 b4 = *reinterpret_cast<const float4*>(tbl_lds + bias_row + col);
                                t4.x += b4.x; t4.y += b4.y; t4.z += b4.z; t4.w += b4.w;
                            }
                            if (EPI == 4) {
                                float* ga = p.sw_gu + (int64_t)m * p.sw_ld + col;
                                const float4 a4 = *reinterpret_cast<const float4*>(ga), b4 = *reinterpret_cast<const float4*>(ga + p.N);
                                const DropoutRng rng(p.p_drop, p.seed);
                                float mu[4];
                                rng.mult4((uint32_t)(((int64_t)m * p.N + col) >> 2), mu);
                                const float d0 = mu[0] * t4.x, d1 = mu[1] * t4.y, d2 = mu[2] * t4.z, d3 = mu[3] * t4.w;
                                const float4 dg = make_float4(d0 * b4.x * dsilu_f(a4.x), d1 * b4.y * dsilu_f(a4.y), d2 * b4.z * dsilu_f(a4.z),
                                                              d3 * b4.w * dsilu_f(a4.w));
                                const float4 du = make_float4(d0 * silu_f(a4.x), d1 * silu_f(a4.y), d2 * silu_f(a4.z), d3 * silu_f(a4.w));
                                *reinterpret_cast<float4*>(ga) = dg;
                                *reinterpret_cast<float4*>(ga + p.N) = du;
                                emax = fmaxf(fmaxf(fmaxf(emax, fmaxf(fabsf(dg.x), fabsf(du.x))), fmaxf(fabsf(dg.y), fabsf(du.y))),
                                             fmaxf(fmaxf(fabsf(dg.z), fabsf(du.z)), fmaxf(fabsf(dg.w), fabsf(du.w))));
                                continue;
                            }
                            if (p.accumulate) {
                                const float4 o = *reinterpret_cast<const float4*>(crow + col);
                                t4.x += o.x; t4.y += o.y; t4.z += o.z; t4.w += o.w;
                            }
                            if (col + 4 <= p.N) {
                                *reinterpret_cast<float4*>(crow + col) = t4;
                            } else {
                                const float e[4] = {t4.x, t4.y, t4.z, t4.w};
                                for (int q = 0; q < 4 && col + q < p.N; ++q) crow[col + q] = e[q];
                            }
                            if (EPI == 2) {
                                const float4 o4 = *reinterpret_cast<const float4*>(p.rowdot_other + (int64_t)m * p.ldc + col);
                                part += (t4.x * o4.x + t4.y * o4.y) + (t4.z * o4.z + t4.w * o4.w);
                            }
                            if (EPI == 5) {
                                const int half = p.N >> 1;
                                float4 x4 = t4;
                                if (p.tbl) {
                                    const float4 tb = *reinterpret_cast<const float4*>(tbl_lds + col);
                                    x4.x += tb.x; x4.y += tb.y; x4.z += tb.z; x4.w += tb.w;
                                }
                                if (col < half) {
                                    gsave[EPI == 5 ? nt * 4 + g4 : 0] = x4;
                                } else {
                                    const float4 g = gsave[EPI == 5 ? nt * 4 + g4 : 0];
                                    const int hc = col - half;
                                    const DropoutRng rng(p.p_drop, p.seed);
                                    float mu[4];
                                    rng.mult4((uint32_t)(((int64_t)m * half + hc) >> 2), mu);
                                    const float4 o = make_float4(mu[0] * (silu_f(g.x) * x4.x), mu[1] * (silu_f(g.y) * x4.y),
                                                                 mu[2] * (silu_f(g.z) * x4.z), mu[3] * (silu_f(g.w) * x4.w));
                                    *reinterpret_cast<float4*>(p.hm + (int64_t)m * half + hc) = o;
                                    emax = fmaxf(fmaxf(fmaxf(emax, fabsf(o.x)), fabsf(o.y)), fmaxf(fabsf(o.z), fabsf(o.w)));
                                }
                            }
                            if (track) cmax = fmaxf(fmaxf(fmaxf(cmax, fabsf(t4.x)), fabsf(t4.y)), fmaxf(fabsf(t4.z), fabsf(t4.w)));
                        }
                    }
            }
            if (EPI == 2) {
                const float sl = xor32_sum(part);
                constexpr int SPH = 64 / AS_SLAB;
                hd_dot = (j % SPH == 0) ? sl : hd_dot + sl;
                if (j % SPH == SPH - 1 && valid_m && h == 0) {
                    const int heads = p.N >> 6, head = (j * AS_SLAB) >> 6;
                    p.rowdot_out[((int64_t)(m / p.rowdot_S) * heads + head) * p.rowdot_S + m % p.rowdot_S] = hd_dot;
                }
            }
    };
    if (AS_DEPTH == 1) {
        load_slab(0);
        store_slab(0, 0);
        __syncthreads();
        auto slab_of = [&](int i) { return EPI == 5 ? (i >> 1) + (i & 1) * (n_slabs >> 1) : i; };
#pragma unroll 1
        for (int i = 0; i < n_slabs; ++i) {
            const int j = slab_of(i), buf = i & 1, jn = slab_of(min(i + 1, n_slabs - 1));
            if (!(AS_ABLATE & 4)) load_slab(jn);
            __builtin_amdgcn_sched_barrier(0);
            mfma_slab(j, buf);
            __builtin_amdgcn_sched_barrier(0);
            if (!(AS_ABLATE & 4)) store_slab(jn, buf ^ 1);
            epilogue_slab(j);
            __syncthreads();
        }
    } else {
        load_slab_into(0, rw);
        store_slab_from(0, 0, rw);
        if (n_slabs > 1) load_slab_into(1, rw);
        if (n_slabs > 2) load_slab_into(2, rw2);
        __syncthreads();
        int bufc = 0;
#pragma unroll 1
        for (int j = 0; j < n_slabs; j += 2) {
            const int b1 = bufc == 2 ? 0 : bufc + 1, b2 = b1 == 2 ? 0 : b1 + 1;
            mfma_slab(j, bufc); epilogue_slab(j);
            if (j + 1 < n_slabs) store_slab_from(j + 1, b1, rw);
            if (j + 3 < n_slabs) load_slab_into(j + 3, rw);
            __syncthreads();
            if (j + 1 >= n_slabs) break;
            mfma_slab(j + 1, b1); epilogue_slab(j + 1);
            if (j + 2 < n_slabs) store_slab_from(j + 2, b2, rw2);
            if (j + 4 < n_slabs) load_slab_into(j + 4, rw2);
            __syncthreads();
            bufc = b2;
        }
    }
    if (p.amax_c) {
        uint32_t mw = __float_as_uint((EPI == 4 || EPI == 5) ? emax : cmax);
#pragma unroll
        for (int o2 = 32; o2 > 0; o2 >>= 1) mw = max(mw, (uint32_t)__shfl_xor((int)mw, o2, 64));
        if (lane == 0 && mw) atomicMax(&amax_word, mw);
        __syncthreads();
        if (tid == 0 && amax_word) amax_publish(amax_word, p.amax_c, blockIdx.x);
    }
}

static std::atomic<long long> g_as_launches{0};
static std::atomic<long long> g_as_fused_launches{0};

static inline bool gemm_as_enabled() {
    static EnvSwitch sw("GAMER_GEMM_AS");
    return sw.get(1) != 0;
}

bool gemm_as_eligible(const gamer_gemm_desc* d, bool a_kc, bool b_kc, const uint16_t* b_planes) {
    if (!gemm_as_enabled() || !a_kc || !b_planes || !d->amax_b) return false;
    if (d->group_mode != 0 || d->resid || d->qk_q_rot) return false;
    if ((d->group_div > 1 || d->sw_tbl) && !d->sw_hm) return false;
    if (d->norm_x) {
        static EnvSwitch swn("GAMER_GEMM_AS_NORM");
        if (swn.get(1) == 0 || !b_kc || !d->norm_w || !aligned16(d->norm_x) || !aligned16(d->norm_w) || !aligned16(d->A) ||
            (d->norm_dst_rows != nullptr) != (d->norm_src_rows != nullptr))
            return false;
    }
    if (d->bias_idx) {
        static EnvSwitch swb("GAMER_GEMM_AS_BIAS");
        if (swb.get(1) == 0 || !b_kc || d->sw_hm || d->groups != 1 || d->accumulate || d->bias_rows < 1 ||
            (int64_t)d->bias_rows * d->N * (int64_t)sizeof(float) > 16384)
            return false;
    }
    if (d->sw_hm) {
        static EnvSwitch sw5("GAMER_GEMM_AS_SWIGLU");
        if (sw5.get(1) == 0 || !b_kc || d->accumulate || d->rowdot_out || d->sw_gu || d->N % (2 * AS_SLAB) != 0 || d->alpha != 1.f ||
            !aligned16(d->sw_hm) || (d->sw_tbl && (!aligned16(d->sw_tbl) || !d->group_offsets)) || d->p_drop < 0.f || d->p_drop >= 1.f)
            return false;
        if (d->group_div > 1 && (!d->group_offsets || d->groups % d->group_div != 0)) return false;
    }
    static EnvSwitch min_m("GAMER_GEMM_AS_MIN_M");
    if (d->K % 64 != 0 || d->K < 64 || d->K > 256 || d->M < min_m.get(16384)) return false;
    if (d->a_rs % 4 != 0 || d->ldc % 4 != 0 || !aligned16(d->C) || !aligned16(b_planes)) return false;
    if (d->groups != 1 && (!d->group_offsets || d->strideC != 0)) return false;
    if (d->groups == 1 && d->group_offsets) return false;
    if (b_kc) {
        if (d->accumulate || d->rowdot_out || d->sw_gu || d->b_rs % 4 != 0) return false;
        if (d->groups != 1 && d->amax_c && !d->sw_hm) return false;
        if (d->amax_c && !d->sw_hm && d->amax_c_col0 % AS_SLAB != 0) return false;
        return true;
    }
    static EnvSwitch rc("GAMER_GEMM_AS_RC");
    const int rc_mode = rc.get(1);
    if (rc_mode == 0) return false;
    if (d->K != 256 || d->N % 4 != 0 || d->b_ks % 4 != 0) return false;
    if ((d->sw_gu || d->rowdot_out) && rc_mode < 2) return false;
    if (d->sw_gu) {
        return !d->amax_c || d->amax_c_col0 == 0;
    }
    if (d->groups != 1) return false;
    if (d->rowdot_out) return !d->accumulate && d->N % 64 == 0 && 64 % AS_SLAB == 0 && (!d->amax_c || d->amax_c_col0 % AS_SLAB == 0);
    return !d->amax_c || (!d->accumulate && d->amax_c_col0 % AS_SLAB == 0);
}

template <int KP, bool WRC, int EPI>
static int launch_as(int nw, dim3 grid, size_t shmem, hipStream_t st, const AsParams& p) {
    const char* who = "gamer_gemm_f32_split/activation-stationary";
    [[maybe_unused]] const bool norm = p.norm_w != nullptr, bias = p.act_idx != nullptr;
    if constexpr (WRC) {
        return with_flags([&](auto eight) { return launch<gemm_as_kernel<KP, WRC, EPI, eight() ? 8 : 4>>(who, grid, dim3(eight() ? 512 : 256), shmem, st, p); },
                          nw == 8);
    } else if constexpr (EPI == 5) {
        return with_flags([&](auto nm) { return launch<gemm_as_kernel<KP, WRC, EPI, 4, nm()>>(who, grid, dim3(64 * 4), shmem, st, p); }, norm);
    } else {
        return with_flags([&](auto eight, auto nm, auto bs) {
            return launch<gemm_as_kernel<KP, WRC, EPI, eight() ? 8 : 4, nm(), bs()>>(who, grid, dim3(eight() ? 512 : 256), shmem, st, p); },
                          nw == 8, norm, bias);
    }
}

int launch_gemm_as(const gamer_gemm_desc* d, const uint16_t* b_planes, bool b_kc, hipStream_t st) {
    AsParams p;
    p.A = d->A; p.lda = d->a_rs;
    p.Wp = b_planes; p.ldw = b_kc ? d->b_rs : d->b_ks;
    p.C = d->C; p.ldc = d->ldc;
    p.M = d->M; p.N = d->N; p.K = d->K;
    p.alpha = d->alpha;
    p.amax_w = d->amax_b;
    p.amax_c = d->amax_c; p.amax_c_col0 = d->amax_c_col0;
    p.groups = d->groups; p.group_offsets = d->groups > 1 ? d->group_offsets : nullptr; p.strideW = d->strideB;
    p.accumulate = d->accumulate;
    p.rowdot_other = d->rowdot_other; p.rowdot_out = d->rowdot_out; p.rowdot_S = d->rowdot_S;
    p.sw_gu = d->sw_gu; p.sw_ld = d->sw_ld; p.p_drop = d->p_drop; p.seed = d->seed;
    p.hm = d->sw_hm; p.tbl = d->sw_hm ? d->sw_tbl : nullptr; p.group_div = d->group_div > 1 ? d->group_div : 1;
    const bool norm = b_kc && d->norm_x, bias = b_kc && d->bias_idx;
    p.norm_w = norm ? d->norm_w : nullptr; p.norm_eps = d->norm_eps; p.src_rows = norm ? d->norm_src_rows : nullptr;
    p.h = const_cast<float*>(d->A); p.ldh = d->a_rs; p.amax_h = norm ? const_cast<uint32_t*>(d->amax_a) : nullptr;
    if (norm) { p.A = d->norm_x; p.lda = d->K; }
    p.act_idx = bias ? d->bias_idx : nullptr; p.bias_q = d->bias_q; p.bias_k = d->bias_k; p.bias_v = d->bias_v;
    p.bias_c1 = d->bias_nq; p.bias_c2 = d->bias_nq + d->bias_nkv; p.nb1 = d->bias_rows;
    const int kp = d->K / 64;
    const size_t shmem = (size_t)(AS_DEPTH == 2 ? 3 : 2) * 2 * kp * AS_PANEL * sizeof(bf16_t) + (d->sw_hm ? (size_t)d->N * sizeof(float) : 0) +
                         (bias ? (size_t)d->bias_rows * d->N * sizeof(float) : 0);
    static EnvSwitch wv("GAMER_GEMM_AS_WAVES");
    const int nw = d->sw_hm ? 4 : (wv.is_set() ? (wv.get(4) == 8 ? 8 : 4) : ((b_kc && d->groups == 1 && d->N >= 512 && AS_WAVES == 4) ? 8 : AS_WAVES));
    const dim3 grid((d->M + 32 * nw - 1) / (32 * nw) + (p.group_offsets ? d->groups : 0));
    int rc;
    if (b_kc && d->sw_hm) {
        switch (kp) {
            case 1: rc = launch_as<1, false, 5>(nw, grid, shmem, st, p); break;
            case 2: rc = launch_as<2, false, 5>(nw, grid, shmem, st, p); break;
            case 3: rc = launch_as<3, false, 5>(nw, grid, shmem, st, p); break;
            default: rc = launch_as<4, false, 5>(nw, grid, shmem, st, p); break;
        }
    } else if (b_kc) {
        switch (kp) {
            case 1: rc = launch_as<1, false, 0>(nw, grid, shmem, st, p); break;
            case 2: rc = launch_as<2, false, 0>(nw, grid, shmem, st, p); break;
            case 3: rc = launch_as<3, false, 0>(nw, grid, shmem, st, p); break;
            default: rc = launch_as<4, false, 0>(nw, grid, shmem, st, p); break;
        }
    } else if (d->sw_gu) {
        rc = launch_as<4, true, 4>(nw, grid, shmem, st, p);
    } else if (d->rowdot_out) {
        rc = launch_as<4, true, 2>(nw, grid, shmem, st, p);
    } else {
        rc = launch_as<4, true, 0>(nw, grid, shmem, st, p);
    }
    if (rc) return rc;
    g_as_launches.fetch_add(1, std::memory_order_relaxed);
    if (norm || bias) g_as_fused_launches.fetch_add(1, std::memory_order_relaxed);
    return 0;
}

__global__ void __launch_bounds__(256)
gemm_bias_rows_kernel(float* __restrict__ Cm, int64_t ldc, int M, int N, const int32_t* __restrict__ idx, const float* __restrict__ bq,
                      const float* __restrict__ bk, const float* __restrict__ bv, int c1, int c2, int nb1, uint32_t* __restrict__ amax_c,
                      int col0) {
    __shared__ uint32_t amax_lds[4];
    uint32_t am = 0;
    const int n4 = N >> 2;
    const int64_t total = (int64_t)M * n4;
    for (int64_t i = (int64_t)blockIdx.x * 256 + threadIdx.x; i < total; i += (int64_t)gridDim.x * 256) {
        const int m = (int)(i / n4), c = 4 * (int)(i - (int64_t)m * n4);
        const int a = min(max(idx[m], 0), nb1 - 1);
        const float* src = c < c1 ? bq + (int64_t)a * c1 + c : c < c2 ? bk + (int64_t)a * (c2 - c1) + (c - c1) : bv + (int64_t)a * (N - c2) + (c - c2);
        const float4 b4 = *reinterpret_cast<const float4*>(src);
        float4* dst = reinterpret_cast<float4*>(Cm + (int64_t)m * ldc + c);
        float4 x = *dst;
        x.x += b4.x; x.y += b4.y; x.z += b4.z; x.w += b4.w;
        *dst = x;
        if (c >= col0) am = amax_f4(am, x);
    }
    amax_block_commit(am, amax_c, amax_lds);
}

int launch_gemm_bias_rows(const gamer_gemm_desc* d, hipStream_t st) {
    const int64_t total = (int64_t)d->M * (d->N >> 2);
    const int blocks = total > 8192 * 256 ? 8192 : (int)((total + 255) / 256);
    return launch<gemm_bias_rows_kernel>("gamer_gemm_f32/bias rows", dim3(blocks), dim3(256), 0, st, d->C, d->ldc, d->M, d->N, d->bias_idx,
                                         d->bias_q, d->bias_k, d->bias_v, d->bias_nq, d->bias_nq + d->bias_nkv, d->bias_rows, d->amax_c,
                                         d->amax_c_col0);
}

}

extern "C" long long gamer_debug_gemm_as_launches(void) { return gamer::g_as_launches.load(std::memory_order_relaxed); }
extern "C" long long gamer_debug_gemm_as_fused_launches(void) { return gamer::g_as_fused_launches.load(std::memory_order_relaxed); }
```

gamer_amd/csrc/inject.hip:

```cpp
#include "common.h"

namespace gamer {

constexpr int INJ_MAX_NB1 = 16;
constexpr int INJ_MAX_EB = 256;

__global__ void __launch_bounds__(256)
inject_table_fwd_kernel(const float* __restrict__ Eb, const float* __restrict__ W, int64_t ldw, int col0, int rows_total, int twoI,
                        int NB1, int EB, float* __restrict__ tbl) {
    __shared__ float eb[INJ_MAX_NB1 * INJ_MAX_EB];
    for (int i = threadIdx.x; i < NB1 * EB; i += 256) eb[i] = Eb[i];
    __syncthreads();
    const int row = blockIdx.x * 256 + threadIdx.x;
    if (row >= rows_total) return;
    const int e = row / twoI, n = row - e * twoI;
    const float* w = W + (int64_t)row * ldw + col0;
    float acc[INJ_MAX_NB1];
#pragma unroll
    for (int b = 0; b < INJ_MAX_NB1; ++b) acc[b] = 0.f;
    for (int j = 0; j < EB; j += 4) {
        const float4 w4 = *reinterpret_cast<const float4*>(w + j);
#pragma unroll
        for (int b = 0; b < INJ_MAX_NB1; ++b) {
            if (b < NB1) {
                const float* e4 = eb + b * EB + j;
                acc[b] = fmaf(e4[0], w4.x, acc[b]); acc[b] = fmaf(e4[1], w4.y, acc[b]);
                acc[b] = fmaf(e4[2], w4.z, acc[b]); acc[b] = fmaf(e4[3], w4.w, acc[b]);
            }
        }
    }
#pragma unroll
    for (int b = 0; b < INJ_MAX_NB1; ++b)
        if (b < NB1) tbl[((int64_t)e * NB1 + b) * twoI + n] = acc[b];
}

constexpr int SEG_CH = 256;
__device__ __forceinline__ bool seg_find(const int32_t* __restrict__ offsets, int nseg, int wg, int& seg, int& r0, int& r1) {
    int prev = offsets[0], before = 0;
    for (int s = 0; s < nseg; ++s) {
        const int nxt = offsets[s + 1];
        const int chunks = (nxt - prev + SEG_CH - 1) / SEG_CH;
        if (wg < before + chunks) {
            seg = s; r0 = prev + (wg - before) * SEG_CH; r1 = min(nxt, r0 + SEG_CH);
            return true;
        }
        before += chunks;
        prev = nxt;
    }
    return false;
}
__global__ void __launch_bounds__(256)
segment_colsum_partial_kernel(const float* __restrict__ x, int64_t ld, int cols4, const int32_t* __restrict__ offsets, int nseg,
                              float4* __restrict__ partial) {
    int seg, r0, r1;
    if (!seg_find(offsets, nseg, blockIdx.x, seg, r0, r1)) return;
    for (int c = threadIdx.x; c < cols4; c += 256) {
        float4 a0 = make_float4(0.f, 0.f, 0.f, 0.f), a1 = a0, a2 = a0, a3 = a0;
        const float* p = x + (int64_t)r0 * ld + 4 * c;
        int r = r0;
        for (; r + 3 < r1; r += 4, p += 4 * ld) {
            const float4 v0 = *reinterpret_cast<const float4*>(p), v1 = *reinterpret_cast<const float4*>(p + ld);
            const float4 v2 = *reinterpret_cast<const float4*>(p + 2 * ld), v3 = *reinterpret_cast<const float4*>(p + 3 * ld);
            a0.x += v0.x; a0.y += v0.y; a0.z += v0.z; a0.w += v0.w; a1.x += v1.x; a1.y += v1.y; a1.z += v1.z; a1.w += v1.w;
            a2.x += v2.x; a2.y += v2.y; a2.z += v2.z; a2.w += v2.w; a3.x += v3.x; a3.y += v3.y; a3.z += v3.z; a3.w += v3.w;
        }
        for (; r < r1; ++r, p += ld) {
            const float4 v0 = *reinterpret_cast<const float4*>(p);
            a0.x += v0.x; a0.y += v0.y; a0.z += v0.z; a0.w += v0.w;
        }
        float4 s;
        s.x = (a0.x + a1.x) + (a2.x + a3.x); s.y = (a0.y + a1.y) + (a2.y + a3.y);
        s.z = (a0.z + a1.z) + (a2.z + a3.z); s.w = (a0.w + a1.w) + (a2.w + a3.w);
        partial[(int64_t)blockIdx.x * cols4 + c] = s;
    }
}
__global__ void __launch_bounds__(256)
segment_colsum_reduce_kernel(const float4* __restrict__ partial, int cols4, const int32_t* __restrict__ offsets, int nseg,
                             float4* __restrict__ out) {
    __shared__ float4 red[4][64];
    const int seg = blockIdx.x;
    int first = 0;
    for (int s = 0; s < seg; ++s) first += (offsets[s + 1] - offsets[s] + SEG_CH - 1) / SEG_CH;
    const int n = (offsets[seg + 1] - offsets[seg] + SEG_CH - 1) / SEG_CH;
    const int cl = threadIdx.x & 63, g = threadIdx.x >> 6;
    const int c = blockIdx.y * 64 + cl;
    float4 a = make_float4(0.f, 0.f, 0.f, 0.f), b = a;
    if (c < cols4) {
        int i = g;
        for (; i + 4 < n; i += 8) {
            const float4 v = partial[(int64_t)(first + i) * cols4 + c], w = partial[(int64_t)(first + i + 4) * cols4 + c];
            a.x += v.x; a.y += v.y; a.z += v.z; a.w += v.w; b.x += w.x; b.y += w.y; b.z += w.z; b.w += w.w;
        }
        if (i < n) {
            const float4 v = partial[(int64_t)(first + i) * cols4 + c];
            a.x += v.x; a.y += v.y; a.z += v.z; a.w += v.w;
        }
    }
    red[g][cl] = make_float4(a.x + b.x, a.y + b.y, a.z + b.z, a.w + b.w);
    __syncthreads();
    if (g == 0 && c < cols4) {
        float4 s = red[0][cl];
#pragma unroll
        for (int k = 1; k < 4; ++k) { s.x += red[k][cl].x; s.y += red[k][cl].y; s.z += red[k][cl].z; s.w += red[k][cl].w; }
        out[(int64_t)seg * cols4 + c] = s;
    }
}

__global__ void __launch_bounds__(256)
inject_table_bwd_w_kernel(const float* __restrict__ seg, const float* __restrict__ Eb, int rows_total, int twoI, int NB1, int EB,
                          float* __restrict__ dW, int64_t ldw, int col0) {
    __shared__ float eb[INJ_MAX_NB1 * INJ_MAX_EB];
    for (int i = threadIdx.x; i < NB1 * EB; i += 256) eb[i] = Eb[i];
    __syncthreads();
    const int q = EB / 4;
    const int64_t item = (int64_t)blockIdx.x * 256 + threadIdx.x;
    if (item >= (int64_t)rows_total * q) return;
    const int row = (int)(item / q), j = (int)(item % q) * 4;
    const int e = row / twoI, n = row - e * twoI;
    float* dst = dW + (int64_t)row * ldw + col0 + j;
    float4 a = *reinterpret_cast<const float4*>(dst);
    for (int b = 0; b < NB1; ++b) {
        const float s = seg[((int64_t)e * NB1 + b) * twoI + n];
        const float* e4 = eb + b * EB + j;
        a.x = fmaf(s, e4[0], a.x); a.y = fmaf(s, e4[1], a.y); a.z = fmaf(s, e4[2], a.z); a.w = fmaf(s, e4[3], a.w);
    }
    *reinterpret_cast<float4*>(dst) = a;
}
__global__ void __launch_bounds__(1024)
inject_table_bwd_e_kernel(const float* __restrict__ seg, const float* __restrict__ W, int64_t ldw, int col0, int E, int twoI, int NB1,
                          int EB, float* __restrict__ scratch) {
    __shared__ float red[16][64];
    const int b = blockIdx.x, e = blockIdx.y, jl = threadIdx.x & 63, part = threadIdx.x >> 6;
    const float* sg = seg + ((int64_t)e * NB1 + b) * twoI;
    for (int j0 = 0; j0 < EB; j0 += 64) {
        const int j = j0 + jl;
        float a0 = 0.f, a1 = 0.f, a2 = 0.f, a3 = 0.f;
        if (j < EB) {
            const float* w = W + (int64_t)e * twoI * ldw + col0 + j;
            int n = part;
            for (; n + 48 < twoI; n += 64) {
                a0 = fmaf(sg[n], w[(int64_t)n * ldw], a0); a1 = fmaf(sg[n + 16], w[(int64_t)(n + 16) * ldw], a1);
                a2 = fmaf(sg[n + 32], w[(int64_t)(n + 32) * ldw], a2); a3 = fmaf(sg[n + 48], w[(int64_t)(n + 48) * ldw], a3);
            }
            for (; n < twoI; n += 16) a0 = fmaf(sg[n], w[(int64_t)n * ldw], a0);
        }
        red[part][jl] = (a0 + a1) + (a2 + a3);
        __syncthreads();
        if (part == 0 && j < EB) {
            float s = red[0][jl];
#pragma unroll
            for (int p2 = 1; p2 < 16; ++p2) s += red[p2][jl];
            scratch[((int64_t)b * E + e) * EB + j] = s;
        }
        __syncthreads();
    }
}
__global__ void __launch_bounds__(256)
inject_table_bwd_e_reduce_kernel(const float* __restrict__ scratch, int E, int NB1, int EB, float* __restrict__ dEb) {
    const int i = blockIdx.x * 256 + threadIdx.x;
    if (i >= NB1 * EB) return;
    const int b = i / EB, j = i - b * EB;
    float s = 0.f;
    for (int e = 0; e < E; ++e) s += scratch[((int64_t)b * E + e) * EB + j];
    dEb[i] += s;
}

}

using namespace gamer;

#define ST(s) ((hipStream_t)(s))

extern "C" int gamer_inject_table_fwd(const float* Eb, const float* W, int64_t ldw, int col0, int E, int twoI, int NB1, int EB,
                                      float* tbl, void* stream) {
    GAMER_CHECK_ARG(Eb && W && tbl, "gamer_inject_table_fwd: null pointer");
    GAMER_CHECK_ARG(E > 0 && twoI > 0 && NB1 > 0 && NB1 <= INJ_MAX_NB1 && EB > 0 && EB % 4 == 0 && EB <= INJ_MAX_EB && col0 >= 0 &&
                    col0 % 4 == 0 && ldw % 4 == 0 && ldw >= col0 + EB && aligned16(W),
                    "gamer_inject_table_fwd: bad shape E=%d 2I=%d NB1=%d EB=%d col0=%d ldw=%lld", E, twoI, NB1, EB, col0, (long long)ldw);
    const int rows = E * twoI;
    hipLaunchKernelGGL(inject_table_fwd_kernel, dim3((rows + 255) / 256), dim3(256), 0, ST(stream), Eb, W, ldw, col0, rows, twoI, NB1, EB,
                       tbl);
    GAMER_CHECK_LAUNCH("gamer_inject_table_fwd");
    return 0;
}

extern "C" int64_t gamer_segment_colsum_ws_floats(int rows, int cols, int nseg) {
    return ((int64_t)(rows + SEG_CH - 1) / SEG_CH + nseg) * (int64_t)cols;
}

extern "C" int gamer_segment_colsum(const float* x, int64_t ld, int rows, int cols, const int32_t* offsets, int nseg, float* ws,
                                    int64_t ws_floats, float* out, void* stream) {
    GAMER_CHECK_ARG(x && offsets && ws && out, "gamer_segment_colsum: null pointer");
    GAMER_CHECK_ARG(rows > 0 && cols > 0 && cols % 4 == 0 && ld % 4 == 0 && ld >= cols && nseg > 0 && aligned16(x) && aligned16(ws) &&
                    aligned16(out), "gamer_segment_colsum: bad shape rows=%d cols=%d ld=%lld nseg=%d", rows, cols, (long long)ld, nseg);
    GAMER_CHECK_ARG(ws_floats >= gamer_segment_colsum_ws_floats(rows, cols, nseg),
                    "gamer_segment_colsum: ws holds %lld floats, needs %lld (gamer_segment_colsum_ws_floats)", (long long)ws_floats,
                    (long long)gamer_segment_colsum_ws_floats(rows, cols, nseg));
    const int wgs = (rows + SEG_CH - 1) / SEG_CH + nseg;
    hipLaunchKernelGGL(segment_colsum_partial_kernel, dim3(wgs), dim3(256), 0, ST(stream), x, ld, cols / 4, offsets, nseg, (float4*)ws);
    GAMER_CHECK_LAUNCH("gamer_segment_colsum/partial");
    hipLaunchKernelGGL(segment_colsum_reduce_kernel, dim3(nseg, (cols / 4 + 63) / 64), dim3(256), 0, ST(stream), (const float4*)ws,
                       cols / 4, offsets, nseg, (float4*)out);
    GAMER_CHECK_LAUNCH("gamer_segment_colsum/reduce");
    return 0;
}

extern "C" int gamer_inject_table_bwd(const float* seg, const float* Eb, const float* W, int64_t ldw, int col0, int E, int twoI, int NB1,
                                      int EB, float* dW, float* dEb, float* scratch, void* stream) {
    GAMER_CHECK_ARG(seg && Eb && W && dW && dEb && scratch, "gamer_inject_table_bwd: null pointer");
    GAMER_CHECK_ARG(E > 0 && twoI > 0 && NB1 > 0 && NB1 <= INJ_MAX_NB1 && EB > 0 && EB % 4 == 0 && EB <= INJ_MAX_EB && col0 >= 0 &&
                    col0 % 4 == 0 && ldw % 4 == 0 && ldw >= col0 + EB && aligned16(dW) && aligned16(W),
                    "gamer_inject_table_bwd: bad shape E=%d 2I=%d NB1=%d EB=%d col0=%d ldw=%lld", E, twoI, NB1, EB, col0, (long long)ldw);
    const int64_t items = (int64_t)E * twoI * (EB / 4);
    hipLaunchKernelGGL(inject_table_bwd_w_kernel, dim3((int)((items + 255) / 256)), dim3(256), 0, ST(stream), seg, Eb, E * twoI, twoI, NB1,
                       EB, dW, ldw, col0);
    GAMER_CHECK_LAUNCH("gamer_inject_table_bwd/dW");
    hipLaunchKernelGGL(inject_table_bwd_e_kernel, dim3(NB1, E), dim3(1024), 0, ST(stream), seg, W, ldw, col0, E, twoI, NB1, EB, scratch);
    GAMER_CHECK_LAUNCH("gamer_inject_table_bwd/dEb partial");
    hipLaunchKernelGGL(inject_table_bwd_e_reduce_kernel, dim3((NB1 * EB + 255) / 256), dim3(256), 0, ST(stream), scratch, E, NB1, EB, dEb);
    GAMER_CHECK_LAUNCH("gamer_inject_table_bwd/dEb");
    return 0;
}
```

gamer_amd/engine.py:

```python
from __future__ import annotations

import contextlib
import functools
import math
import os
from types import SimpleNamespace
from typing import Dict, List, Optional, Tuple

import torch

from . import ops
from .config import Qwen3MultiConfig

IGNORE_INDEX = -100


def _round_up(x: int, m: int) -> int:
    return (x + m - 1) // m * m


class _FlatLayout:

    def __init__(self, decay: List[Tuple[str, tuple]], nodecay: List[Tuple[str, tuple]]):
        self.entries: Dict[str, Tuple[int, tuple]] = {}
# ... 767 lines not shown
            self.shadow.refresh()
        if self.weight_planes is not None:
            ops.split3_planes(self.flat_p, self.weight_planes)
        use_drop = train if dropout is None else dropout
        c = self._pass(B, S, float(dropout_rate) if use_drop else 0.0,
                       float(self.cfg.attention_dropout) if use_drop else 0.0)
        if use_drop:
            self.dropout_step += 1
        ws = c.ws = self.ws = self.workspace(B, S, train)
        if self._amax is not None:
            self._amax.reset()
            if train:
                self._amax.stable(ws.xn, *[A[k] for A in ws.layers for k in ("h1", "h2", "ao", "ao_c", "hin", "hm") if k in A])
                if self.h2_attention:
                    self._amax.stable(*[A[k] for A in ws.layers for k in ("q", "k", "q_c", "k_c") if k in A],
                                      *[A[k][:, c.NQ + c.NKV:] for A in ws.layers for k in ("qkv", "qkv_c") if k in A])
        c.ids = input_ids.to(self.device, torch.int64).contiguous()
        c.am = attention_mask.to(self.device, torch.int64).contiguous() if attention_mask is not None else None
        c.lab = labels.to(self.device, torch.int64).contiguous() if labels is not None else None
        c.uniform_len, c.train = uniform_len, train
        if c.lab is not None:
            ws.bad_label.zero_()
            ops.check_labels(c.lab, self.cfg.vocab_size, IGNORE_INDEX, ws.bad_label)
        return c

    def _attention(self, c, qb, kb, vb, kl_, ql_, empty_, tile_empty_, seed_, ob, lseb, order_, span_):
        B, S, nq, nkv, NQ, NKV, QKV = c.B, c.S, c.nq, c.nkv, c.NQ, c.NKV, c.QKV
        if c.split_attn and (span_ is None or c.h2):
            ops.attn_fwd_split(qb, NQ, kb, NKV, vb, QKV, kl_, ql_, empty_, B, S, nq, nkv, c.scale, c.p_att, seed_, ob, lseb,
                               order=order_, h2=c.h2, uniform_len=c.uniform_len, q_span=span_)
        elif c.bf16:
            ord16 = (order_[0], order_[2], empty_) if (order_ is not None and span_ is None) else None
            ops.attn_fwd_bf16(qb, NQ, kb, NKV, vb, QKV, kl_, ql_, B, S, nq, nkv, c.scale, c.p_att, seed_, ob, lseb,
                              q_span=span_, order=ord16)
        else:
            ops.attn_fwd(qb, NQ, kb, NKV, vb, QKV, kl_, ql_, empty_, tile_empty_, B, S, nq, nkv, c.scale, c.p_att, seed_,
                         ob, lseb, order=order_, uniform_len=c.uniform_len, q_span=span_)

    def _self_attention(self, c, l: int, masks: dict, span, pos_ids, fuse_qkv: bool, kv_dest, kv_sink):
        W, Wm, A, xs = self.W[l], self.Wm[l], c.ws.layers[l], c.ws.x[l]
        T, H, NQ, NKV, QKV, eps = c.T, c.H, c.NQ, c.NKV, c.QKV, c.eps
        nrm = dict(norm=dict(x=xs[0], w=W.ln1, eps=eps)) if (c.fuse_norm and not fuse_qkv) else {}
        if not nrm:
            ops.rmsnorm_fwd(xs[0], W.ln1, eps, A["h1"])
        qkv_s, k_s = kv_dest(l, "self") if kv_dest is not None else (A["qkv"], A["k"])
        if fuse_qkv:
            ops.gemm(A["h1"], H, 1, Wm.self_attn["qkv"], H, 1, qkv_s, QKV, T, QKV, H,
                     qknorm=dict(wq=W.self_attn["qn"], wk=W.self_attn["kn"], eps=eps, cos=c.cos, sin=c.sin, q_rot=A["q"],
                                 k_rot=k_s, pos_ids=pos_ids, S=c.S, nq=c.nq, nkv=c.nkv))
        else:
            v_amax = dict(c_amax=(qkv_s[:, NQ + NKV:], NQ + NKV)) if (c.h2 and self.gemm_c_amax) else {}
            ops.linear_fwd(A["h1"], H, Wm.self_attn["qkv"], H, qkv_s, QKV, T, QKV, H, **v_amax, **nrm)
            ops.qknorm_rope_fwd(qkv_s, c.S, c.nq, c.nkv, W.self_attn["qn"], W.self_attn["kn"], eps, c.cos, c.sin, A["q"], k_s,
                                pos_ids=pos_ids)
        if kv_sink is not None:
            kv_sink(l, "self", k_s, qkv_s[:, NQ + NKV:])
        self._attention(c, A["q"], k_s, qkv_s[:, NQ + NKV:], masks["kl_self"], None, masks["empty_self"],
                        masks["tile_empty_self"], self._seed(l, 0), A["ao"], A["lse"], None, span)
        ops.gemm(A["ao"], NQ, 1, Wm.self_attn["o"], NQ, 1, xs[1], H, T, H, NQ, resid=xs[0], p_drop=c.p_res,
                 seed=self._seed(l, 1))

    def _head(self, c, x_last: Optional[torch.Tensor], num_items_in_batch, hidden_sink):
        ws, B, S, H, eps = c.ws, c.B, c.S, c.H, c.eps
        V = self.cfg.vocab_size
        if x_last is not None:
            xn = torch.empty_like(x_last, dtype=self.act_dtype)
            ops.rmsnorm_fwd(x_last, self.params["model.norm.weight"], eps, xn)
            small = torch.empty(B, ws.ldl, dtype=torch.float32, device=self.device)
            if c.bf16:
                small16 = torch.zeros(B, ws.ldl, dtype=torch.bfloat16, device=self.device)
                ops.linear_fwd(xn, H, self.shadow.params16["model.embed_tokens.weight"], H, small16, ws.ldl, B, V, H)
                small.copy_(small16)
            else:
                ops.linear_fwd(xn, H, self.params["model.embed_tokens.weight"], H, small, ws.ldl, B, V, H)
            self._saved = None
            self.last_logits_buf = small
            return None, small.view(B, 1, ws.ldl)[:, :, :V]
        nrm = dict(norm=dict(x=ws.x_final, w=self.params["model.norm.weight"], eps=eps)) if c.fuse_norm else {}
        if not nrm:
            ops.rmsnorm_fwd(ws.x_final, self.params["model.norm.weight"], eps, ws.xn)
        emb_m = self.shadow.params16["model.embed_tokens.weight"] if c.bf16 else self.params["model.embed_tokens.weight"]
        lab = c.lab
        head_alpha = (1.0 / self.temperature) if (lab is not None and ws.logits.dtype == torch.float32) else 1.0
        ops.linear_fwd(ws.xn, H, emb_m, H, ws.logits, ws.ldl, c.T, V, H, alpha=head_alpha, **nrm)
        if hidden_sink is not None:
            hidden_sink.append(ws.xn.view(B, S, H).clone())
        loss = None
        if lab is not None:
            ops.ce_fwd(ws.logits, ws.ldl, lab, V, 1.0 if head_alpha != 1.0 else self.temperature, IGNORE_INDEX, ws.lse_ce,
                       ws.row_loss, ws.loss_sum, ws.count)
            if torch.is_tensor(num_items_in_batch):
                num_items_in_batch = num_items_in_batch.to(self.device, torch.float32).reshape(1)
                loss = ws.loss_sum[0] / num_items_in_batch[0]
            elif num_items_in_batch is not None:
                loss = ws.loss_sum[0] / float(num_items_in_batch)
            else:
                loss = ws.loss_sum[0] / ws.count[0]
        self._saved = dict(ids=c.ids, labels=lab, num_items=num_items_in_batch, train=c.train, p_res=c.p_res, p_att=c.p_att,
                           B=B, S=S, dropout_step=self.dropout_step)
        return loss, ws.logits.view(B, S, ws.ldl)[:, :, :V]

    def check_inputs(self):
        n = int(self.ws.router["bad_token"].item())
        if n:
            raise IndexError(f"{n} item(s) start with a token that is not in config.behavior_maps "
                             "(the reference fails with an embedding IndexError, router.py:170-171)")
        n = int(self.ws.bad_label.item())
        if n:
            raise IndexError(f"{n} label(s) outside [0, vocab_size={self.cfg.vocab_size}) that are not -100 "
                             "(nn.CrossEntropyLoss raises 'Target out of bounds' in the reference)")
        if self.variant == "session" and self.ws.session is not None:
            n = int(self.ws.session["violations"].item())
            if n:
                raise ValueError(f"{n} row(s) with session ids that decrease along the sequence or RoPE positions "
                                 "outside [0, S): the session masks are built as causal key spans "
                                 "(gamer_session_spans), which needs the dataset's layout (SMB_dataset.py:194-222)")

    def zero_grad(self):
        ops.fill(self.flat_g, 0.0)

    @ops.scoped_f32_matmul(lambda self, *a: self.matmul, lambda self, *a: self._planes())
    @ops.scoped_amax(lambda self, *a: self._amax)
    def backward(self, dloss: float = 1.0, layer_done=None, dloss_dev: Optional[torch.Tensor] = None):
        sv = self._saved
        if sv is None or not sv["train"] or sv["labels"] is None:
            raise RuntimeError("backward() needs forward(train=True, labels=...) first")
        with ops.deterministic(True if self.deterministic else ops.DETERMINISTIC_WGRAD, bf16=True if self.deterministic else None):
            return self._backward(dloss, layer_done, dloss_dev)

    def _backward(self, dloss: float = 1.0, layer_done=None, dloss_dev: Optional[torch.Tensor] = None):
        cfg = self.cfg
        c = self._backward_head(dloss, dloss_dev, rows=self._ffn_rows(cfg.num_hidden_layers - 1))
        ws, B, S, T, H, I, E = c.ws, c.B, c.S, c.T, c.H, c.I, cfg.num_experts
        nq, nkv, NQ, NKV, QKV, eps, cos, sin, p_res = c.nq, c.nkv, c.NQ, c.NKV, c.QKV, c.eps, c.cos, c.sin, c.p_res
        NB1 = cfg.num_behavior + 1
        span_self = span_cross = pos_ids = None
        if self.variant == "session":
            span_self, span_cross, pos_ids = ws.session["span_self"], ws.session["span_cross"], ws.session["pos_ids"]
        r = ws.router
        NP = ws.norm_partial[-1]
        hold, fuse_delta, do_amax, fuse_swiglu_bwd = c.hold, c.fuse_delta, c.do_amax, c.fuse_swiglu_bwd
        dgrad, norm_bwd = functools.partial(self._dgrad, c), functools.partial(self._norm_bwd, c)
        attention_bwd = functools.partial(self._attention_bwd, c)
        t0, t1, t2, t3 = ws.tmpH
        bf16 = c.bf16
        for l in reversed(range(cfg.num_hidden_layers)):
            W, G, A, xs = self.W[l], self.G[l], ws.layers[l], ws.x[l]
            WT = self.WT[l] if bf16 else None
            din = W.din
            grp = dict(groups=E, group_offsets=ws.offsets)
            xlast = xs[2] if W.cross else xs[1]
            if not self._shipped_ffn_layer(W):
                self._ffn_bwd_plain(c, l, xlast)
            else:
                split_inj = W.inject and self.split_inject
                tb = ws._buf(f"l{l}_inject_tbl", (E * NB1, 2 * I)) if split_inj else None
                with hold(t0):
                    ops.linear_wgrad(t0, H, A["hm"], I, G.down, I, T, H, I, strideC=H * I, **grp)
                    if fuse_swiglu_bwd and split_inj:
                        ops.gemm(t0, H, 1, W.down, 1, I, ws.dhm, I, T, I, H, strideB=H * I, p_drop=p_res, seed=self._seed(l, 4),
                                 swiglu_bwd=(A["gu"], 2 * I), groups=E * NB1, group_offsets=ws.grp_offsets, group_div=NB1, sw_tbl=tb)
                    elif fuse_swiglu_bwd:
                        if bf16:
                            ops.linear_dgrad_t(t0, H, WT.down, WT.down.shape[1], ws.dhm, I, T, H, I, strideB=H * I, p_drop=p_res,
                                               seed=self._seed(l, 4), swiglu_bwd=(A["gu"], 2 * I), **grp)
                        else:
                            ops.gemm(t0, H, 1, W.down, 1, I, ws.dhm, I, T, I, H, strideB=H * I, p_drop=p_res, seed=self._seed(l, 4),
                                     swiglu_bwd=(A["gu"], 2 * I), **grp)
                    else:
                        dgrad(t0, H, W.down, WT.down if bf16 else None, I, ws.dhm, I, H, I, strideB=H * I, **grp)
                if not fuse_swiglu_bwd:
                    if split_inj:
                        ops.swiglu_bwd_ld_tbl(A["gu"], 2 * I, T, I, ws.dhm, p_res, self._seed(l, 4), tb, ws.row_group)
                    else:
                        ops.swiglu_bwd_ld(A["gu"], 2 * I, T, I, ws.dhm, p_res, self._seed(l, 4))
                if split_inj:
                    hin = A["hin"].view(-1)[:T * H].view(T, H)
                    dhin = ws.dhin.view(-1)[:T * H].view(T, H)
                    with hold(A["gu"]):
                        ops.linear_wgrad(A["gu"], 2 * I, hin, H, G.gu, din, T, 2 * I, H, strideC=2 * I * din, **grp)
                        dgrad(A["gu"], 2 * I, W.gu, None, din, dhin, H, 2 * I, H, strideB=2 * I * din, **grp)
                    seg = ws._buf("inject_segsum", (E * NB1, 2 * I))
                    seg_ws = ws._buf("inject_seg_ws", (ops.segment_colsum_ws_floats(T, 2 * I, E * NB1),))
                    ops.segment_colsum(A["gu"], 2 * I, T, 2 * I, ws.grp_offsets, E * NB1, seg_ws, seg)
                    ops.inject_table_bwd(seg, W.beh, W.gu, din, H, E, 2 * I, G.gu, G.beh,
                                         ws._buf("inject_scratch", (NB1 * E * cfg.behavior_embedding_dim,)))
                    norm_bwd(xlast, W.ln3, dhin, H, G.ln3, True, ws.slot, branch=None if W.cross else (self._seed(l, 1), None))
                else:
                    with hold(A["gu"]):
                        ops.linear_wgrad(A["gu"], 2 * I, A["hin"], din, G.gu, din, T, 2 * I, din, strideC=2 * I * din, **grp)
                        dgrad(A["gu"], 2 * I, W.gu, WT.gu if bf16 else None, din, ws.dhin, din, 2 * I, din, strideB=2 * I * din, **grp)
                    if W.inject:
                        ops.rowtable_bwd(ws.dhin, din, H, r["beh_idx"], G.beh, ws.slot, partial=NP)
                    norm_bwd(xlast, W.ln3, ws.dhin, din, G.ln3, True, ws.slot,
                             branch=None if W.cross else (self._seed(l, 1), None))
            if W.cross:
                C, GC = W.cross_attn, G.cross_attn
                CT = WT.cross_attn if bf16 else dict(o=None, gate=None, qkv=None)
                ops.silu_gate_bwd(A["op_c"], A["gate_c"], ws.dx, t1, t2, p=p_res, seed=self._seed(l, 3))
                hold_t2 = hold(t2)
                hold_t2.__enter__()
                with hold(t1):
                    ops.linear_wgrad(t1, H, A["ao_c"], NQ, GC["o"], NQ, T, H, NQ)
                    ops.linear_wgrad(t2, H, A["h2"], H, GC["gate"], H, T, H, H)
                    dgrad(t1, H, C["o"], CT["o"], NQ, ws.dao, NQ, H, NQ,
                          rowdot=(A["ao_c"], ws.delta, S) if fuse_delta else None, **do_amax)
                attention_bwd(A["q_c"], A["k_c"], A["qkv_c"][:, NQ + NKV:], A["ao_c"], A["lse_c"], r["kl_cross"],
                              r["ql_cross"], r["empty_cross"], r["tile_empty_cross"], self._seed(l, 2), ws.cross_order,
                              span_cross)
                ops.qknorm_rope_bwd(A["qkv_c"], ws.dq, ws.dk, S, nq, nkv, C["qn"], C["kn"], eps, cos, sin, ws.dqkv,
                                    GC["qn"], GC["kn"], bias_q=C["bq"], bias_k=C["bk"], act_idx=r["act_idx"], nb1=NB1,
                                    dbias_q=GC["bq"], dbias_k=GC["bk"], dbias_v=GC["bv"], pos_ids=pos_ids,
                                    partial=ws.qk_partial)
                with hold(ws.dqkv):
                    ops.linear_wgrad(ws.dqkv, QKV, A["h2"], H, GC["qkv"], H, T, QKV, H)
                    dgrad(ws.dqkv, QKV, C["qkv"], CT["qkv"], H, t3, H, QKV, H)
                dgrad(t2, H, C["gate"], CT["gate"], H, t3, H, H, H, accumulate=True)
                hold_t2.__exit__(None, None, None)
                norm_bwd(xs[1], W.ln2, t3, H, G.ln2, True, branch=(self._seed(l, 1), None))
            self._self_attention_bwd(c, l, r, span_self, pos_ids, rows=self._ffn_rows(l - 1) if l > 0 else None)
            if layer_done is not None:
                layer_done(l)
        self._backward_tail(c)

    def _backward_head(self, dloss, dloss_dev, rows) -> SimpleNamespace:
        sv = self._saved
        c = self._pass(sv["B"], sv["S"], sv["p_res"], sv["p_att"])
        ws = c.ws = self.ws
        c.saved_step = self.dropout_step
        self.dropout_step = sv["dropout_step"]
        c.ids, c.norm_dws = sv["ids"], []
        c.fuse_delta = (ws.ds_work is not None or c.bf16 or c.split_attn) and c.T % 128 == 0 and c.NQ % 128 == 0
        c.do_amax = dict(c_amax=(ws.dao, 0)) if (c.h2 and self.gemm_c_amax) else {}
        c.hold = self._amax.hold if self._amax is not None else (lambda *t: contextlib.nullcontext())
        V, H, T, L = self.cfg.vocab_size, c.H, c.T, self.cfg.num_hidden_layers
        if torch.is_tensor(sv["num_items"]):
            ops.ce_bwd(ws.logits, ws.ldl, sv["labels"], V, self.temperature, IGNORE_INDEX, ws.lse_ce, sv["num_items"], 0.0,
                       dloss, dloss_dev)
        elif sv["num_items"] is not None:
            ops.ce_bwd(ws.logits, ws.ldl, sv["labels"], V, self.temperature, IGNORE_INDEX, ws.lse_ce, None,
                       float(sv["num_items"]), dloss, dloss_dev)
        else:
            ops.ce_bwd(ws.logits, ws.ldl, sv["labels"], V, self.temperature, IGNORE_INDEX, ws.lse_ce, ws.count, 0.0,
                       dloss, dloss_dev)
        t3 = ws.tmpH[3]
        with c.hold(ws.logits):
            ops.linear_wgrad(ws.logits, ws.ldl, ws.xn, H, self.grads["model.embed_tokens.weight"], H, T, V, H)
            self._dgrad(c, ws.logits, ws.ldl, self.params["model.embed_tokens.weight"],
                        self.shadow.t("model.embed_tokens.weight") if c.bf16 else None, H, t3, H, V, H)
        self._norm_bwd(c, ws.x_final, self.params["model.norm.weight"], t3, H, self.grads["model.norm.weight"], False,
                       branch=(self._seed(L - 1, 5), rows))
        return c

    def _dgrad(self, c, dy, lddy, Wf, Wt, ldw, dx, lddx, n_out, k_in, **kw):
        if c.bf16:
            ops.linear_dgrad_t(dy, lddy, Wt, Wt.shape[1], dx, lddx, c.T, n_out if Wt.shape[1] == n_out else Wt.shape[1],
                               k_in, **kw)
        else:
            ops.linear_dgrad(dy, lddy, Wf, ldw, dx, lddx, c.T, n_out, k_in, **kw)

    def _norm_bwd(self, c, xin, w, dy, lddy, dw, accumulate_dx, dy_rows=None, branch=None):
        ws = c.ws
        part = ws.norm_partial[len(c.norm_dws)]
        c.norm_dws.append(dw)
        if branch is None:
            ops.rmsnorm_bwd(xin, w, dy, lddy, c.eps, ws.dx, part, accumulate_dx, dy_rows)
        else:
# ... 102 lines not shown
```

gamer_amd/ops.py:

```python
from __future__ import annotations

import ctypes as C
from typing import Optional

import os

import torch

from . import _lib
from ._lib import GemmBf16Desc, GemmDesc, call, ptr, stream_ptr


def _sfx(t: torch.Tensor) -> str:
    if t.dtype == torch.float32:
        return ""
    if t.dtype == torch.bfloat16:
        return "_bf16"
    raise RuntimeError(f"activations must be float32 or bfloat16, got {t.dtype}")


def _chk(t: torch.Tensor, dtype, name: str):
    if not t.is_cuda:
        raise RuntimeError(f"{name} must be on the HIP device (gamer_amd has no CPU path)")
    if t.dtype != dtype:
# ... 404 lines not shown

def _arm_sink(*outs):
    if _AMAX_REUSE is None or F32_MATMUL_TERMS != 3 or outs[0][0].dtype != torch.float32:
        return
    slots = [_AMAX_REUSE.preset(t, g, acc) for t, g, acc in outs]
    if slots[0] is None:
        return
    if len(slots) > 2:
        call("gamer_amax_sink3", slots[0], slots[1], slots[2])
    else:
        call("gamer_amax_sink", slots[0], slots[1] if len(slots) > 1 else None)


def scoped_amax(get_cache):
    import functools

    def deco(fn):
        @functools.wraps(fn)
        def wrapper(*args, **kwargs):
            cache = get_cache(*args)
            if cache is None:
                return fn(*args, **kwargs)
            with cache:
                return fn(*args, **kwargs)
        return wrapper
    return deco


def absmax_slot(x, batch, stride, rows, cols, ld, produced=False):
    if _AMAX_REUSE is not None:
        if produced:
            _AMAX_REUSE.preset(x, (batch, stride, rows, cols, ld))
        return _AMAX_REUSE.slot(x, (batch, stride, rows, cols, ld))
    key = (x.device.index, stream_ptr())
    ring = _AMAX_RING.get(key)
    if ring is None:
        ring = _AMAX_RING[key] = [torch.zeros(_AMAX_SLOTS * AMAX_WORDS, dtype=torch.int32, device=x.device), 0]
    if ring[1] == _AMAX_SLOTS:
        ring[0].zero_()
        ring[1] = 0
    slot = ring[0].data_ptr() + 4 * AMAX_WORDS * ring[1]
    ring[1] += 1
    if not produced:
        call("gamer_absmax_f32", ptr(x), batch, stride, rows, cols, ld, slot, stream_ptr())
    return slot


def split3_planes(x, planes):
    call("gamer_split3_planes", ptr(x), ptr(planes), x.numel(), planes.stride(0), stream_ptr())


DETERMINISTIC_WGRAD = os.environ.get("GAMER_WGRAD_TWO_PASS", "1") != "0"
DETERMINISTIC_WGRAD_BF16 = os.environ.get("GAMER_WGRAD_TWO_PASS_BF16", "0") == "1"
_WGRAD_WS = {}


class deterministic:

    def __init__(self, on: bool = True, bf16=None):
        self.on, self.bf16 = bool(on), bf16

    def __enter__(self):
        global DETERMINISTIC_WGRAD, DETERMINISTIC_WGRAD_BF16
        self.prev, DETERMINISTIC_WGRAD = DETERMINISTIC_WGRAD, self.on
        self.prev16 = DETERMINISTIC_WGRAD_BF16
        if self.bf16 is not None:
            DETERMINISTIC_WGRAD_BF16 = bool(self.bf16)
        return self

    def __exit__(self, *exc):
        global DETERMINISTIC_WGRAD, DETERMINISTIC_WGRAD_BF16
        DETERMINISTIC_WGRAD, DETERMINISTIC_WGRAD_BF16 = self.prev, self.prev16
        return False


def _wgrad_workspace(device, floats: int) -> torch.Tensor:
    t = _WGRAD_WS.get(device)
    if t is None or t.numel() < floats:
        _WGRAD_WS[device] = None
        t = _WGRAD_WS[device] = torch.empty(int(floats), dtype=torch.float32, device=device)
    return t


class split3_guard:

    def __init__(self, on: bool):
        self.on = bool(on)

    def __enter__(self):
        self.prev = _lib.load().gamer_split3_guard(1 if self.on else 0)
        return self

    def __exit__(self, *exc):
        _lib.load().gamer_split3_guard(self.prev)
        return False


def set_f32_matmul(mode) -> int:
    global F32_MATMUL_TERMS
    prev = F32_MATMUL_TERMS
    terms = MATMUL_MODES[mode] if isinstance(mode, str) else int(mode)
    if terms not in (0, 3, 6, 9):
        raise ValueError(f"fp32 matmul mode {mode!r}: one of {sorted(MATMUL_MODES)}")
    F32_MATMUL_TERMS = terms
    return prev


def gemm(A, a_rs, a_ks, Bm, b_rs, b_ks, Cm, ldc, M, N, K, alpha=1.0, accumulate=False, groups=1, group_mode=0,
         group_offsets=None, strideB=0, strideC=0, kchunk=0, resid=None, row_map=None, p_drop=0.0, seed=0,
         rowdot=None, qknorm=None, c_amax=None, swiglu_bwd=None, group_div=0, sw_tbl=None, swiglu_fwd=None, norm=None, bias=None):
    if A.dtype == torch.bfloat16:
        if group_div > 1 or sw_tbl is not None or swiglu_fwd is not None or norm is not None or bias is not None:
            raise RuntimeError("group_div / sw_tbl / swiglu_fwd / norm / bias are options of the fp32 GEMM")
        return _gemm_bf16(A, a_rs, a_ks, Bm, b_rs, b_ks, Cm, ldc, M, N, K, alpha, accumulate, groups, group_mode,
                          group_offsets, strideB, strideC, kchunk, resid, row_map, p_drop, seed, rowdot, qknorm, swiglu_bwd)
    d = GemmDesc()
    d.A = ptr(A); d.a_rs = a_rs; d.a_ks = a_ks
    d.B = ptr(Bm); d.b_rs = b_rs; d.b_ks = b_ks
    d.C = ptr(Cm); d.ldc = ldc
    d.M = M; d.N = N; d.K = K
    d.alpha = alpha
    d.accumulate = 1 if accumulate else 0
    d.groups = groups
    d.group_mode = group_mode
    d.group_offsets = ptr(group_offsets)
    d.strideB = strideB; d.strideC = strideC
    d.kchunk = kchunk
    d.resid = ptr(resid)
    d.row_map = ptr(row_map)
    d.p_drop = p_drop
    d.seed = seed
    if rowdot is not None:
        d.rowdot_other, d.rowdot_out, d.rowdot_S = ptr(rowdot[0]), ptr(rowdot[1]), int(rowdot[2])
    if qknorm is not None:
        q = qknorm
        d.qk_wq, d.qk_wk, d.qk_eps = ptr(q["wq"]), ptr(q["wk"]), float(q["eps"])
        d.qk_cos, d.qk_sin = ptr(q["cos"]), ptr(q["sin"])
        d.qk_bias_q, d.qk_bias_k, d.qk_bias_v = ptr(q.get("bias_q")), ptr(q.get("bias_k")), ptr(q.get("bias_v"))
        d.qk_act_idx, d.qk_pos_ids = ptr(q.get("act_idx")), ptr(q.get("pos_ids"))
        d.qk_q_rot, d.qk_k_rot = ptr(q["q_rot"]), ptr(q["k_rot"])
        d.qk_S, d.qk_nq, d.qk_nkv = int(q["S"]), int(q["nq"]), int(q["nkv"])
    if (c_amax is not None and _AMAX_REUSE is not None and F32_MATMUL_TERMS == 3 and group_mode == 0 and not accumulate
            and resid is None and qknorm is None and c_amax[1] % 64 == 0):
        view, col0 = c_amax
        slot_c = _AMAX_REUSE.preset(view, (1, 0, M, N - col0, ldc))
        d.amax_c, d.amax_c_col0 = slot_c, int(col0)
    if swiglu_bwd is not None:
        gu, ld_gu = swiglu_bwd
        d.sw_gu, d.sw_ld = ptr(gu), int(ld_gu)
        d.sw_tbl = ptr(sw_tbl)
        if _AMAX_REUSE is not None and F32_MATMUL_TERMS == 3 and ld_gu == 2 * N:
            d.amax_c, d.amax_c_col0 = _AMAX_REUSE.preset(gu, (1, 0, 1, M * ld_gu, M * ld_gu)), 0
    d.group_div = int(group_div)
    if norm is not None:
        nx = norm["x"]
        if group_mode != 0 or a_ks != 1 or b_ks != 1 or nx.dim() != 2 or nx.shape[0] < M or nx.shape[1] != K or not nx.is_contiguous():
            raise RuntimeError("gemm(norm=...): a Linear-forward GEMM whose rows are the RMSNorm of a dense [M, K] tensor")
        d.norm_x, d.norm_w, d.norm_eps = ptr(norm["x"]), ptr(norm["w"]), float(norm["eps"])
        d.norm_dst_rows, d.norm_src_rows = ptr(norm.get("dst_rows")), ptr(norm.get("src_rows"))
    if bias is not None:
        d.bias_idx, d.bias_q, d.bias_k, d.bias_v = ptr(bias["idx"]), ptr(bias["q"]), ptr(bias["k"]), ptr(bias["v"])
        d.bias_rows, d.bias_nq, d.bias_nkv = int(bias["q"].shape[0]), int(bias["q"].shape[1]), int(bias["k"].shape[1])
    if swiglu_fwd is not None:
        hm, tbl, row_group = swiglu_fwd
        d.sw_hm, d.sw_tbl, d.sw_row_group = ptr(hm), ptr(tbl), ptr(row_group)
        if _AMAX_REUSE is not None and F32_MATMUL_TERMS == 3:
            d.amax_c, d.amax_c_col0 = _AMAX_REUSE.preset(hm, (1, 0, 1, M * (N // 2), M * (N // 2))), 0
    if group_mode == 1 and DETERMINISTIC_WGRAD:
        n_chunks = (K + kchunk - 1) // kchunk + (groups if group_offsets is not None else 0)
        need = n_chunks * ((M + 127) // 128) * ((N + 127) // 128) * 16384
        ws = _wgrad_workspace(A.device, need)
        d.wgrad_ws, d.wgrad_ws_floats = ws.data_ptr(), ws.numel()
    if F32_MATMUL_TERMS == 3:
        ga = (M, K, a_rs) if a_ks == 1 else (K, M, a_ks)
        gb = (N, K, b_rs) if b_ks == 1 else (K, N, b_ks)
        nb = (groups // max(1, int(group_div))) if (group_mode == 0 and groups > 1) else 1
        d.amax_a = absmax_slot(A, 1, 0, *ga, produced=norm is not None)
        geom_b = (nb, strideB if nb > 1 else 0) + gb
        c = _AMAX_REUSE
        parent = c.plane_parent(Bm.data_ptr(), geom_b) if (c is not None and c.planes is not None and group_mode == 0) else None
        if parent is not None:
            d.amax_b = parent
            d.b_planes = c.planes.data_ptr() + (Bm.data_ptr() - c.stable_ranges[0][0])
            call("gamer_gemm_f32_split", C.byref(d), 3, stream_ptr())
            return
        d.amax_b = absmax_slot(Bm, *geom_b)
        if c is not None and c.planes is not None and group_mode == 0 and c._key(Bm.data_ptr(), geom_b) in c._plane_keys:
            d.b_planes = c.planes.data_ptr() + (Bm.data_ptr() - c.stable_ranges[0][0])
            if a_ks == 1 and b_ks == 1 and c._key(Bm.data_ptr(), geom_b) in c._tplane_keys:
                d.b_planes_t = c.planes_t.data_ptr() + (Bm.data_ptr() - c.stable_ranges[0][0])
        call("gamer_gemm_f32_split", C.byref(d), 3, stream_ptr())
        return
    if F32_MATMUL_TERMS:
        if WEIGHT_PLANES is not None and group_mode == 0:
            base, nbytes, pl, stride = WEIGHT_PLANES
            off = Bm.data_ptr() - base
            if 0 <= off < nbytes:
                d.b_planes, d.b_plane_stride = pl + off // 2, stride
        call("gamer_gemm_f32_split", C.byref(d), F32_MATMUL_TERMS, stream_ptr())
    else:
        call("gamer_gemm_f32", C.byref(d), stream_ptr())


def _gemm_bf16(A, a_rs, a_ks, Bm, b_rs, b_ks, Cm, ldc, M, N, K, alpha, accumulate, groups, group_mode, group_offsets,
               strideB, strideC, kchunk, resid, row_map, p_drop, seed, rowdot, qknorm=None, swiglu_bwd=None):
    if Bm.dtype != torch.bfloat16 or alpha != 1.0:
        raise RuntimeError("gamer_gemm_bf16 takes two bf16 operands and alpha = 1")
    d = GemmBf16Desc()
    if group_mode == 0:
        if a_ks != 1 or b_ks != 1:
            raise RuntimeError("bf16 GEMM: both operands must be k-contiguous (dgrad runs on the transposed weight copy)")
        d.lda, d.ldb = a_rs, b_rs
        want = torch.float32 if resid is not None else torch.bfloat16
    else:
        if a_rs != 1 or b_rs != 1:
            raise RuntimeError("bf16 wgrad: both operands must be token-major")
        d.lda, d.ldb = a_ks, b_ks
        want = torch.float32
    if Cm.dtype != want:
        raise RuntimeError(f"bf16 GEMM: C must be {want}, got {Cm.dtype}")
    d.A, d.B, d.C, d.ldc = ptr(A), ptr(Bm), ptr(Cm), ldc
    d.M, d.N, d.K = M, N, K
    d.accumulate = 1 if accumulate else 0
    d.groups, d.group_mode, d.group_offsets = groups, group_mode, ptr(group_offsets)
    d.strideB, d.strideC, d.kchunk = strideB, strideC, kchunk
    d.resid, d.row_map, d.p_drop, d.seed = ptr(resid), ptr(row_map), p_drop, seed
    if rowdot is not None:
        d.rowdot_other, d.rowdot_out, d.rowdot_S = ptr(rowdot[0]), ptr(rowdot[1]), int(rowdot[2])
    if qknorm is not None:
        q = qknorm
        d.qk_wq, d.qk_wk, d.qk_eps = ptr(q["wq"]), ptr(q["wk"]), float(q["eps"])
        d.qk_cos, d.qk_sin = ptr(q["cos"]), ptr(q["sin"])
        d.qk_bias_q, d.qk_bias_k, d.qk_bias_v = ptr(q.get("bias_q")), ptr(q.get("bias_k")), ptr(q.get("bias_v"))
        d.qk_act_idx, d.qk_pos_ids = ptr(q.get("act_idx")), ptr(q.get("pos_ids"))
        d.qk_q_rot, d.qk_k_rot = ptr(q["q_rot"]), ptr(q["k_rot"])
        d.qk_S, d.qk_nq, d.qk_nkv = int(q["S"]), int(q["nq"]), int(q["nkv"])
    if swiglu_bwd is not None:
        d.sw_gu, d.sw_ld = ptr(swiglu_bwd[0]), int(swiglu_bwd[1])
    if group_mode == 1 and DETERMINISTIC_WGRAD_BF16:
        n_chunks = (K + kchunk - 1) // kchunk + (groups if group_offsets is not None else 0)
        need = n_chunks * ((M + 127) // 128) * ((N + 127) // 128) * 16384
        ws = _wgrad_workspace(A.device, need)
        d.wgrad_ws, d.wgrad_ws_floats = ws.data_ptr(), ws.numel()
    call("gamer_gemm_bf16", C.byref(d), stream_ptr())

# ... 1351 lines not shown
```

include/gamer_hip.h:

```cpp
#ifndef GAMER_HIP_H
#define GAMER_HIP_H

#include <stdint.h>

#ifdef __cplusplus
extern "C" {
#endif

#define GAMER_ABI_VERSION 9
#define GAMER_AMAX_WORDS 256

typedef uint16_t gamer_bf16;

int gamer_abi_version(void);
const char* gamer_last_error(void);
int gamer_reload_env(void);

int gamer_router_fwd(const int64_t* ids, const int64_t* attn_mask, const int64_t* actions,
                     const int32_t* behavior_lut, int vocab, int B, int S, int num_positions,
                     int pad_id, int eos_id,
                     int32_t* expert, int32_t* beh_idx, int32_t* act_idx,
                     int32_t* kl_self, int32_t* kl_cross, int32_t* ql_cross,
                     int32_t* empty_self, int32_t* empty_cross,
                     int32_t* tile_empty_self, int32_t* tile_empty_cross,
// ... 30 lines not shown
                        void* stream);
int64_t gamer_embedding_bwd_ordered_ws_bytes(int V, int T, int H);
int gamer_embedding_bwd_ordered(const int64_t* ids, const float* dx, int V, int T, int H, int pad_id, float* dW,
                                void* ws, int64_t ws_bytes, void* stream);

int gamer_rmsnorm_fwd(const float* x, const float* w, int T, int H, float eps,
                      const int32_t* dst_rows, float* y, int ldy, void* stream);
int gamer_rmsnorm_bwd(const float* x, const float* w, const float* dy, int lddy,
                      const int32_t* dy_rows, int T, int H, float eps, int accumulate_dx,
                      float* dx, float* dw_partial, int n_partial,
                      float* mask_out, const int32_t* mask_rows, float p_drop, uint64_t seed, void* stream);
int gamer_rmsnorm_fwd_bf16(const float* x, const float* w, int T, int H, float eps,
                           const int32_t* dst_rows, gamer_bf16* y, int ldy, void* stream);
int gamer_rmsnorm_bwd_bf16(const float* x, const float* w, const gamer_bf16* dy, int lddy,
                           const int32_t* dy_rows, int T, int H, float eps, int accumulate_dx,
                           float* dx, float* dw_partial, int n_partial,
                           gamer_bf16* mask_out, const int32_t* mask_rows, float p_drop, uint64_t seed, void* stream);
int gamer_colsum_reduce(const float* partial, int rows, int cols, int accumulate, float* out,
                        void* stream);
int gamer_colsum_reduce_batched(const float* partial, int64_t stride, int rows, int cols, int n, float* const* outs,
                                int accumulate, void* stream);

int gamer_rowtable_fwd(const float* table, const int32_t* idx, const int32_t* dst_rows, int T, int E,
                       float* y, int ldy, int col0, void* stream);
int gamer_rowtable_bwd(const float* dy, int lddy, int col0, const int32_t* idx,
                       const int32_t* dy_rows, int T, int E, int n_rows_table, float* dtable,
                       float* partial, int64_t partial_numel, void* stream);
int gamer_rowtable_fwd_bf16(const float* table, const int32_t* idx, const int32_t* dst_rows, int T, int E,
                            gamer_bf16* y, int ldy, int col0, void* stream);
int gamer_rowtable_bwd_bf16(const gamer_bf16* dy, int lddy, int col0, const int32_t* idx,
                            const int32_t* dy_rows, int T, int E, int n_rows_table, float* dtable,
                            float* partial, int64_t partial_numel, void* stream);

typedef struct {
    const float* A; int64_t a_rs, a_ks;
    const float* B; int64_t b_rs, b_ks;
    float* C; int64_t ldc;
    int M, N, K;
    float alpha;
    int accumulate;
    int groups;
    int group_mode;
    const int32_t* group_offsets;
    int64_t strideB, strideC;
    int kchunk;
    const float* resid;
    const int32_t* row_map;
    float p_drop;
    uint64_t seed;
    const float* rowdot_other;
    float* rowdot_out;
    int rowdot_S;
    const float* qk_wq; const float* qk_wk;
    float qk_eps;
    const float* qk_cos; const float* qk_sin;
    const float* qk_bias_q; const float* qk_bias_k; const float* qk_bias_v;
    const int32_t* qk_act_idx;
    const int32_t* qk_pos_ids;
    float* qk_q_rot; float* qk_k_rot;
    int qk_S, qk_nq, qk_nkv;
    const gamer_bf16* b_planes;
    int64_t b_plane_stride;
    const uint32_t* amax_a;
    const uint32_t* amax_b;
    uint32_t* amax_c;
    int amax_c_col0;
    float* wgrad_ws;
    int64_t wgrad_ws_floats;
    float* sw_gu;
    int64_t sw_ld;
    int group_div;
    const float* sw_tbl;
    const gamer_bf16* b_planes_t;
    float* sw_hm;
    const int32_t* sw_row_group;
    const float* norm_x;
    const float* norm_w;
    float norm_eps;
    const int32_t* norm_dst_rows;
    const int32_t* norm_src_rows;
    const int32_t* bias_idx;
    const float* bias_q; const float* bias_k; const float* bias_v;
    int bias_rows, bias_nq, bias_nkv;
} gamer_gemm_desc;

int gamer_gemm_f32(const gamer_gemm_desc* d, void* stream);
int gamer_split2h_transpose_multi(const gamer_bf16* planes, const int64_t* table, int n, gamer_bf16* planes_t, void* stream);

int gamer_gemm_f32_split(const gamer_gemm_desc* d, int terms, void* stream);
int gamer_split3_guard(int on);
int gamer_absmax_f32(const float* x, int batch, int64_t stride, int rows, int cols, int64_t ld, uint32_t* out, void* stream);
int gamer_absmax_multi_f32(const float* base, const int64_t* table, int n, uint32_t* out, void* stream);
int gamer_split2h_planes_multi(const float* base, const int64_t* table, int n, const uint32_t* slots, gamer_bf16* planes,
                               void* stream);
int gamer_amax_sink(uint32_t* out0, uint32_t* out1);
int gamer_amax_sink3(uint32_t* out0, uint32_t* out1, uint32_t* out2);
int gamer_attn_split_amax(const uint32_t* q, const uint32_t* k, const uint32_t* v, const uint32_t* d_o);
int gamer_split3_planes(const float* x, gamer_bf16* planes, int64_t n, int64_t plane_stride, void* stream);

typedef struct {
    const gamer_bf16* A; int64_t lda;
    const gamer_bf16* B; int64_t ldb;
    void* C; int64_t ldc;
    int M, N, K;
    int accumulate;
    int groups;
    int group_mode;
    const int32_t* group_offsets;
    int64_t strideB, strideC;
    int kchunk;
    const float* resid;
    const int32_t* row_map;
    float p_drop;
    uint64_t seed;
    const gamer_bf16* rowdot_other;
    float* rowdot_out;
    int rowdot_S;
    const float* qk_wq; const float* qk_wk; float qk_eps;
    const float* qk_cos; const float* qk_sin;
    const float* qk_bias_q; const float* qk_bias_k; const float* qk_bias_v;
    const int32_t* qk_act_idx; const int32_t* qk_pos_ids;
    gamer_bf16* qk_q_rot; gamer_bf16* qk_k_rot;
    int qk_S, qk_nq, qk_nkv;
    gamer_bf16* sw_gu;
    int64_t sw_ld;
    float* wgrad_ws;
    int64_t wgrad_ws_floats;
} gamer_gemm_bf16_desc;

int gamer_gemm_bf16(const gamer_gemm_bf16_desc* d, void* stream);

int gamer_cast_params_bf16(const float* flat, gamer_bf16* out, gamer_bf16* out_t, const int64_t* table,
                           int n_entries, int n_tiles, void* stream);

int gamer_qknorm_rope_fwd(float* qkv, int T, int S, int nq, int nkv,
                          const float* wq, const float* wk, float eps,
                          const float* cos_t, const float* sin_t,
                          const float* bias_q, const float* bias_k, const float* bias_v,
                          const int32_t* act_idx,
                          float* q_rot, float* k_rot, const int32_t* pos_ids, void* stream);
int gamer_qknorm_rope_bwd(const float* qkv, const float* dq_rot, const float* dk_rot,
                          int T, int S, int nq, int nkv,
                          const float* wq, const float* wk, float eps,
                          const float* cos_t, const float* sin_t,
                          const float* bias_q, const float* bias_k,
                          const int32_t* act_idx, int nb1,
                          float* dqkv, float* dwq, float* dwk,
                          float* dbias_q, float* dbias_k, float* dbias_v, const int32_t* pos_ids,
                          float* partial, int64_t partial_numel, void* stream);
int gamer_qknorm_rope_fwd_bf16(gamer_bf16* qkv, int T, int S, int nq, int nkv,
                               const float* wq, const float* wk, float eps,
                               const float* cos_t, const float* sin_t,
                               const float* bias_q, const float* bias_k, const float* bias_v,
                               const int32_t* act_idx,
                               gamer_bf16* q_rot, gamer_bf16* k_rot, const int32_t* pos_ids, void* stream);
int gamer_qknorm_rope_bwd_bf16(const gamer_bf16* qkv, const gamer_bf16* dq_rot, const gamer_bf16* dk_rot,
                               int T, int S, int nq, int nkv,
                               const float* wq, const float* wk, float eps,
                               const float* cos_t, const float* sin_t,
                               const float* bias_q, const float* bias_k,
                               const int32_t* act_idx, int nb1,
                               gamer_bf16* dqkv, float* dwq, float* dwk,
                               float* dbias_q, float* dbias_k, float* dbias_v, const int32_t* pos_ids,
                               float* partial, int64_t partial_numel, void* stream);

int gamer_attn_row_order(const int32_t* row_empty, int B, int S, int32_t* perm, int32_t* tile_kind,
// ... 304 lines not shown
```

Baseline: 5124.

## Fuse SwiGLU-backward column sums and cross-entropy into GEMM epilogues

The SwiGLU-backward GEMM epilogue now accumulates per-tile column sums of the gate/up gradients and writes them to a workspace. A small segment reduce kernel then combines them, replacing the separate segment_colsum pass that re-read the whole gu gradient buffer. The LM-head GEMM can also take cross-entropy labels and compute an online log-sum-exp, per-row loss and loss/count partials inside the as-kernel epilogue, which removes the separate ce_fwd launch and its re-read of the logits. The cost is extra registers, shuffles and a block sync in the epilogues. The CE path may still fall back to a GEMM followed by a CE call when the as-kernel is not eligible.

```diff
diff --git a/gamer_amd/_lib.py b/gamer_amd/_lib.py
--- a/gamer_amd/_lib.py
+++ b/gamer_amd/_lib.py
@@ -57,6 +57,10 @@
         ("norm_dst_rows", c_void_p), ("norm_src_rows", c_void_p),
         ("bias_idx", c_void_p), ("bias_q", c_void_p), ("bias_k", c_void_p), ("bias_v", c_void_p),
         ("bias_rows", c_int), ("bias_nq", c_int), ("bias_nkv", c_int),
+        ("sw_colsum_out", c_void_p), ("sw_colsum_ws", c_void_p), ("sw_colsum_ws_floats", c_int64),
+        ("ce_labels", c_void_p), ("ce_S", c_int), ("ce_ignore_index", c_int),
+        ("ce_lse", c_void_p), ("ce_row_loss", c_void_p), ("ce_loss_sum", c_void_p), ("ce_count", c_void_p),
+        ("ce_ws", c_void_p), ("ce_ws_floats", c_int64),
     ]
 
 
diff --git a/gamer_amd/csrc/common.h b/gamer_amd/csrc/common.h
--- a/gamer_amd/csrc/common.h
+++ b/gamer_amd/csrc/common.h
@@ -327,6 +327,7 @@
 bool gemm_os_fwd_eligible(const gamer_gemm_desc* d, bool a_kc, bool b_kc);
 bool gemm_wg_eligible(const gamer_gemm_desc* d, bool a_kc, bool b_kc);
 int launch_gemm_wg(const gamer_gemm_desc* d, hipStream_t st);
+int launch_segment_colsum_reduce(const float* partial, int cols, const int32_t* offsets, int nseg, int ch, float* out, hipStream_t st);
 
 int launch_wgrad_reduce(const float* ws, float* C, int64_t ldc, int M, int N, int groups, const int32_t* group_offsets, int K,
                         int kchunk, int64_t strideC, hipStream_t st);
diff --git a/gamer_amd/csrc/gemm.hip b/gamer_amd/csrc/gemm.hip
--- a/gamer_amd/csrc/gemm.hip
+++ b/gamer_amd/csrc/gemm.hip
@@ -211,6 +211,7 @@
     float* sw_gu; int64_t sw_ld;
     int group_div;
     const float* sw_tbl;
+    float* sw_cs;
 };
 
 constexpr float SPLIT3_GUARD_RATIO = 1.f / 65536.f;
@@ -303,9 +304,11 @@
     }
 }
 
-template <bool A_KC, bool B_KC, int MODE, bool ACCUM, bool STAMP, int NBUF, int EPI, int SPLIT = 0, bool PP = false>
+template <bool A_KC, bool B_KC, int MODE, bool ACCUM, bool STAMP, int NBUF, int EPI_T, int SPLIT = 0, bool PP = false>
 __device__ __forceinline__ void
 gemm_f32_tile(const GemmParams& p, float* __restrict__ smem_all, const int vblock, const int vgrid) {
+    constexpr int EPI = EPI_T == 5 ? 4 : EPI_T;
+    constexpr bool CS = EPI_T == 5 && !PP;
 
     const int grp = PP ? (int)(threadIdx.x >> 8) : 0;
     const int tid = threadIdx.x & (GEMM_THREADS - 1);
@@ -326,6 +329,7 @@
     float* Cp = p.C;
     int64_t ws_block = 0;
     int tile_group = 0;
+    int m_tile = 0;
     if (MODE == 0) {
         const int mt = L / p.n_tiles;
         col0 = (L % p.n_tiles) * BN;
@@ -351,6 +355,7 @@
         kbeg = 0;
         kend = p.K;
         tile_group = g;
+        m_tile = mt;
         Bp += (int64_t)(g / p.group_div) * p.strideB;
         Bsrc = Bp;
         if (SPLIT == 3 && p.b_planes) Bp = reinterpret_cast<const float*>(p.b_planes) + (Bp - p.B);
@@ -914,6 +919,12 @@
             tb_g = *reinterpret_cast<const float4*>(tb);
             tb_u = *reinterpret_cast<const float4*>(tb + p.N);
         }
+        if (CS) {
+            if (lane < 16) {
+                *reinterpret_cast<float4*>(patch + lane * 68 + 64) = tb_g;
+                *reinterpret_cast<float4*>(patch + (16 + lane) * 68 + 64) = tb_u;
+            }
+        }
         auto pre_sw = [&](int it0) {
 #pragma unroll
             for (int it = 0; it < 8; ++it) {
@@ -923,6 +934,7 @@
             }
         };
         if (EPI == 4) pre_sw(0);
+        float4 cs_g = make_float4(0.f, 0.f, 0.f, 0.f), cs_u = cs_g;
 #pragma unroll
         for (int it = 0; it < 16; ++it) {
             if (EPI == 4 && it == 8) pre_sw(8);
@@ -977,8 +989,10 @@
                 float* ga = p.sw_gu + (int64_t)row * p.sw_ld + col;
                 float* ua = ga + p.N;
                 float4 a = pre_x[EPI == 4 ? (it & 7) : 0], b = pre_b[EPI == 4 ? (it & 7) : 0];
-                a.x += tb_g.x; a.y += tb_g.y; a.z += tb_g.z; a.w += tb_g.w;
-                b.x += tb_u.x; b.y += tb_u.y; b.z += tb_u.z; b.w += tb_u.w;
+                const float4 tg = CS ? *reinterpret_cast<const float4*>(patch + (lane & 15) * 68 + 64) : tb_g;
+                const float4 tu = CS ? *reinterpret_cast<const float4*>(patch + (16 + (lane & 15)) * 68 + 64) : tb_u;
+                a.x += tg.x; a.y += tg.y; a.z += tg.z; a.w += tg.w;
+                b.x += tu.x; b.y += tu.y; b.z += tu.z; b.w += tu.w;
                 float m[4];
                 rng.mult4((uint32_t)(((int64_t)row * p.N + col) >> 2), m);
                 const float d0 = m[0] * v.x, d1 = m[1] * v.y, d2 = m[2] * v.z, d3 = m[3] * v.w;
@@ -989,6 +1003,10 @@
                 dg.w = d3 * b.w * dsilu_f(a.w); du.w = d3 * silu_f(a.w);
                 *reinterpret_cast<float4*>(ga) = dg;
                 *reinterpret_cast<float4*>(ua) = du;
+                if (CS) {
+                    cs_g.x += dg.x; cs_g.y += dg.y; cs_g.z += dg.z; cs_g.w += dg.w;
+                    cs_u.x += du.x; cs_u.y += du.y; cs_u.z += du.z; cs_u.w += du.w;
+                }
                 if (amax_on) {
                     asm("v_max3_f32 %0, %0, |%1|, |%2|\n\tv_max3_f32 %0, %0, |%3|, |%4|" : "+v"(cmax) : "v"(dg.x), "v"(dg.y), "v"(dg.z), "v"(dg.w));
                     asm("v_max3_f32 %0, %0, |%1|, |%2|\n\tv_max3_f32 %0, %0, |%3|, |%4|" : "+v"(cmax) : "v"(du.x), "v"(du.y), "v"(du.z), "v"(du.w));
@@ -1031,6 +1049,26 @@
             for (int o2 = 32; o2 > 0; o2 >>= 1) mw = max(mw, (uint32_t)__shfl_xor((int)mw, o2, 64));
             if (lane == 0 && mw) amax_publish(mw, p.amax_c, (uint32_t)(vblock * 4 + wid));
         }
+        if (CS) {
+            float cs[8] = {cs_g.x, cs_g.y, cs_g.z, cs_g.w, cs_u.x, cs_u.y, cs_u.z, cs_u.w};
+#pragma unroll
+            for (int k = 0; k < 8; ++k) {
+                cs[k] += __shfl_xor(cs[k], 16, 64);
+                cs[k] += __shfl_xor(cs[k], 32, 64);
+            }
+            if (wm == 1 && lane < 16) {
+                *reinterpret_cast<float4*>(patch + c4) = make_float4(cs[0], cs[1], cs[2], cs[3]);
+                *reinterpret_cast<float4*>(patch + 68 + c4) = make_float4(cs[4], cs[5], cs[6], cs[7]);
+            }
+            __syncthreads();
+            if (wm == 0 && lane < 16) {
+                const float* lo = smem + (wid + 2) * (64 * 68);
+                const float4 g1 = *reinterpret_cast<const float4*>(lo + c4), u1 = *reinterpret_cast<const float4*>(lo + 68 + c4);
+                float* dst = p.sw_cs + (int64_t)m_tile * 2 * p.N + col;
+                *reinterpret_cast<float4*>(dst) = make_float4(cs[0] + g1.x, cs[1] + g1.y, cs[2] + g1.z, cs[3] + g1.w);
+                *reinterpret_cast<float4*>(dst + p.N) = make_float4(cs[4] + u1.x, cs[5] + u1.y, cs[6] + u1.z, cs[7] + u1.w);
+            }
+        }
     } else if (MODE == 1 && p.wgrad_ws != nullptr) {
         float* blk = p.wgrad_ws + ws_block * (int64_t)(BM * BN);
 #pragma unroll
@@ -1108,6 +1146,18 @@
             for (int o2 = 32; o2 > 0; o2 >>= 1) mw = max(mw, (uint32_t)__shfl_xor((int)mw, o2, 64));
             if (lane == 0 && mw) amax_publish(mw, p.amax_c, (uint32_t)(vblock * 4 + wid));
         }
+        if (CS) {
+            __syncthreads();
+            const int r_last = min(row_end, row0 + BM);
+            for (int c = threadIdx.x; c < 2 * BN; c += GEMM_THREADS) {
+                const int cc = col0 + (c & (BN - 1)), half = c >= BN ? p.N : 0;
+                if (cc >= p.N) continue;
+                const float* src = p.sw_gu + (int64_t)row0 * p.sw_ld + half + cc;
+                float s = 0.f;
+                for (int r = row0; r < r_last; ++r, src += p.sw_ld) s += *src;
+                p.sw_cs[(int64_t)m_tile * 2 * p.N + half + cc] = s;
+            }
+        }
     }
     if (STAMP) {
         unsigned long long* st = g_gemm_stamp;
@@ -1175,7 +1225,8 @@
 #endif
     if (stamp && SPLIT == 6) return launch_gemm_t<A_KC, B_KC, MODE, false, true, 2, 0, SPLIT>(p, blocks, st, lds);
     if constexpr (SPLIT == 3 && MODE == 0 && A_KC) {
-        if (p.sw_gu) return launch_gemm_t<A_KC, B_KC, MODE, false, false, 2, 4, SPLIT>(p, blocks, st, lds);
+        if (p.sw_gu) return p.sw_cs ? launch_gemm_t<A_KC, B_KC, MODE, false, false, 2, 5, SPLIT>(p, blocks, st, lds)
+                                    : launch_gemm_t<A_KC, B_KC, MODE, false, false, 2, 4, SPLIT>(p, blocks, st, lds);
     }
     if (MODE == 0 && p.resid) return launch_gemm_t<A_KC, B_KC, MODE, false, false, 2, 1, SPLIT>(p, blocks, st, lds);
     if (MODE == 0 && p.rowdot_out) return launch_gemm_t<A_KC, B_KC, MODE, false, false, 2, 2, SPLIT>(p, blocks, st, lds);
@@ -1344,6 +1395,12 @@
     p.wgrad_ws = nullptr;
     p.sw_gu = d->sw_gu; p.sw_ld = d->sw_ld;
     p.group_div = d->group_div > 1 ? d->group_div : 1; p.sw_tbl = d->sw_tbl;
+    p.sw_cs = nullptr;
+    GAMER_CHECK_ARG(!d->sw_colsum_out || (d->sw_gu && d->sw_colsum_ws && d->group_offsets && d->group_mode == 0 && a_kc && aligned16(d->sw_colsum_ws) &&
+                                          aligned16(d->sw_colsum_out) &&
+                                          d->sw_colsum_ws_floats >= ((int64_t)(d->M + BM - 1) / BM + d->groups) * 2 * (int64_t)d->N),
+                    "gamer_gemm_f32: sw_colsum_out goes with sw_gu, group_offsets and sw_colsum_ws of at least (ceil(M / 128) + groups) x 2 N "
+                    "floats (M=%d N=%d groups=%d, given %lld)", d->M, d->N, d->groups, (long long)d->sw_colsum_ws_floats);
     GAMER_CHECK_ARG(d->group_div <= 1 || (d->group_mode == 0 && d->group_offsets && d->groups % d->group_div == 0),
                     "gamer_gemm_f32: group_div = %d needs group_mode 0, group_offsets and groups (%d) a multiple of it", d->group_div, d->groups);
     GAMER_CHECK_ARG(!d->sw_tbl || ((d->sw_gu || d->sw_hm) && aligned16(d->sw_tbl)),
@@ -1400,7 +1457,21 @@
                                      aligned16(d->bias_k) && aligned16(d->bias_v)),
                     "gamer_gemm_f32: the bias-row epilogue (bias_idx) needs a plain Linear-forward GEMM with one group, three tables and "
                     "N = bias_nq + 2 bias_nkv in multiples of 4 (N=%d)", d->N);
+    GAMER_CHECK_ARG(!d->ce_labels || (d->ce_lse && d->ce_row_loss && d->ce_loss_sum && d->ce_count && d->ce_ws && d->group_mode == 0 &&
+                                      d->groups == 1 && a_kc && b_kc && !d->accumulate && !d->resid && !d->rowdot_out && !d->qk_q_rot &&
+                                      !d->sw_gu && !d->sw_hm && !d->bias_idx && d->ce_S > 0 && d->M % d->ce_S == 0 && d->ldc < (1LL << 31) &&
+                                      aligned16(d->ce_ws) && d->ce_ws_floats >= 4 * ((int64_t)(d->M + 127) / 128)),
+                    "gamer_gemm_f32: the cross-entropy epilogue (ce_labels) needs a plain one-group Linear-forward GEMM, all five outputs, "
+                    "M (%d) a multiple of ce_S (%d) and a 16-byte aligned ce_ws of 4 x ceil(M / 128) floats (given %lld)", d->M, d->ce_S,
+                    (long long)d->ce_ws_floats);
     if (split == 3 && gemm_as_eligible(d, a_kc, b_kc, p.b_planes)) return launch_gemm_as(d, p.b_planes, b_kc, (hipStream_t)stream);
+    if (d->ce_labels) {
+        gamer_gemm_desc d2 = *d;
+        d2.ce_labels = nullptr;
+        GAMER_TRY(gemm_entry(&d2, stream, split));
+        return gamer_ce_fwd(d->C, (int)d->ldc, d->ce_labels, d->M / d->ce_S, d->ce_S, d->N, 1.f, d->ce_ignore_index, d->ce_lse, d->ce_row_loss,
+                            d->ce_loss_sum, d->ce_count, stream);
+    }
     if (d->norm_x || d->bias_idx) {
         gamer_gemm_desc d2 = *d;
         if (d->norm_x) {
@@ -1432,6 +1503,16 @@
         p.m_tiles = (d->M + BM - 1) / BM + (d->group_offsets ? d->groups : 0);
         const int64_t blocks = (int64_t)p.m_tiles * p.n_tiles;
         GAMER_CHECK_ARG(blocks < (1LL << 31), "gamer_gemm_f32: grid too large");
+        if (d->sw_colsum_out) {
+            static EnvSwitch cs_switch("GAMER_SWIGLU_BWD_COLSUM");
+            const bool fused = cs_switch.get(1) != 0 && split == 3 && !diag_pp_switch() && d->N % 4 == 0;
+            if (fused) p.sw_cs = d->sw_colsum_ws;
+            const int rc = b_kc ? launch_gemm<true, true, 0>(p, (int)blocks, st, split) : launch_gemm<true, false, 0>(p, (int)blocks, st, split);
+            if (rc) return rc;
+            if (fused) return launch_segment_colsum_reduce(d->sw_colsum_ws, 2 * d->N, d->group_offsets, d->groups, BM, d->sw_colsum_out, st);
+            return gamer_segment_colsum(d->sw_gu, d->sw_ld, d->M, 2 * d->N, d->group_offsets, d->groups, d->sw_colsum_ws, d->sw_colsum_ws_floats,
+                                        d->sw_colsum_out, stream);
+        }
         if (a_kc && b_kc) return launch_gemm<true, true, 0>(p, (int)blocks, st, split);
         if (a_kc && !b_kc) return launch_gemm<true, false, 0>(p, (int)blocks, st, split);
         if (!a_kc && !b_kc) return launch_gemm<false, false, 0>(p, (int)blocks, st, split);
diff --git a/gamer_amd/csrc/gemm_as.hip b/gamer_amd/csrc/gemm_as.hip
--- a/gamer_amd/csrc/gemm_as.hip
+++ b/gamer_amd/csrc/gemm_as.hip
@@ -41,6 +41,7 @@
     float* hm; const float* tbl; int group_div;
     const float* norm_w; float norm_eps; float* h; int64_t ldh; const int32_t* src_rows; uint32_t* amax_h;
     const int32_t* act_idx; const float* bias_q; const float* bias_k; const float* bias_v; int bias_c1, bias_c2, nb1;
+    const int64_t* ce_labels; int ce_S, ce_ignore; float* ce_lse; float* ce_row_loss; double* ce_part;
 };
 
 template <int KP, bool WRC, int EPI, int NW, bool NORM = false, bool BIAS = false>
@@ -218,6 +219,14 @@
         if (valid_m) bias_row = min(max(p.act_idx[m], 0), p.nb1 - 1) * p.N;
     }
 
+    float ce_mx = -INFINITY, ce_se = 0.f, ce_zt = 0.f;
+    int ce_tgt = -1;
+    if constexpr (EPI == 6) {
+        if (valid_m && (m % p.ce_S) + 1 < p.ce_S) {
+            const int64_t t = p.ce_labels[m + 1];
+            if (t != p.ce_ignore && t >= 0 && t < p.N) ce_tgt = (int)t;
+        }
+    }
     float cmax = 0.f;
     float* crow = p.C + (int64_t)m * p.ldc;
     f32x16 acc[AS_NT];
@@ -320,6 +329,36 @@
                         }
                     }
             }
+            if constexpr (EPI == 6) {
+                if (valid_m) {
+                    const bool full = (j + 1) * AS_SLAB <= p.N;
+                    float v[16 * AS_NT];
+                    float smax = -INFINITY;
+#pragma unroll
+                    for (int nt = 0; nt < AS_NT; ++nt)
+#pragma unroll
+                        for (int k = 0; k < 16; ++k) {
+                            const int col = j * AS_SLAB + nt * 32 + 8 * (k >> 2) + 4 * h + (k & 3);
+                            v[16 * nt + k] = (full || col < p.N) ? acc[nt][k] * out_scale : -INFINITY;
+                            smax = fmaxf(smax, v[16 * nt + k]);
+                        }
+                    if (smax > -INFINITY) {
+                        const float nm = fmaxf(ce_mx, smax);
+                        float se = 0.f;
+#pragma unroll
+                        for (int k = 0; k < 16 * AS_NT; ++k) se += __expf(v[k] - nm);
+                        ce_se = ce_se * __expf(ce_mx - nm) + se;
+                        ce_mx = nm;
+                    }
+                    if (ce_tgt >= 0 && ce_tgt / AS_SLAB == j) {
+#pragma unroll
+                        for (int nt = 0; nt < AS_NT; ++nt)
+#pragma unroll
+                            for (int k = 0; k < 16; ++k)
+                                if (j * AS_SLAB + nt * 32 + 8 * (k >> 2) + 4 * h + (k & 3) == ce_tgt) ce_zt = v[16 * nt + k];
+                    }
+                }
+            }
             if (EPI == 2) {
                 const float sl = xor32_sum(part);
                 constexpr int SPH = 64 / AS_SLAB;
@@ -368,6 +407,33 @@
             bufc = b2;
         }
     }
+    if constexpr (EPI == 6) {
+        __shared__ double ce_wave[2][AS_WAVES_K];
+        const float mx = xor32_max(ce_mx);
+        const float se = xor32_sum(ce_se * __expf(ce_mx - mx));
+        const float zt = xor32_sum(ce_zt);
+        const float lse = mx + logf(se);
+        const float row_loss = (valid_m && ce_tgt >= 0) ? lse - zt : 0.f;
+        double loss = (double)row_loss, cnt = (valid_m && ce_tgt >= 0) ? 1.0 : 0.0;
+        if (valid_m && h == 0) {
+            p.ce_lse[m] = lse;
+            p.ce_row_loss[m] = row_loss;
+        }
+#pragma unroll
+        for (int o2 = 16; o2 > 0; o2 >>= 1) {
+            loss += __shfl_xor(loss, o2, 64);
+            cnt += __shfl_xor(cnt, o2, 64);
+        }
+        if (lane == 0) { ce_wave[0][w] = loss; ce_wave[1][w] = cnt; }
+        __syncthreads();
+        if (tid == 0) {
+            double l = ce_wave[0][0], c = ce_wave[1][0];
+#pragma unroll
+            for (int i = 1; i < AS_WAVES_K; ++i) { l += ce_wave[0][i]; c += ce_wave[1][i]; }
+            p.ce_part[2 * blockIdx.x] = l;
+            p.ce_part[2 * blockIdx.x + 1] = c;
+        }
+    }
     if (p.amax_c) {
         uint32_t mw = __float_as_uint((EPI == 4 || EPI == 5) ? emax : cmax);
 #pragma unroll
@@ -378,8 +444,31 @@
     }
 }
 
+__global__ void __launch_bounds__(1024)
+ce_partials_reduce_kernel(const double* __restrict__ part, int n, float* __restrict__ loss_sum, float* __restrict__ count) {
+    __shared__ double sh_l[1024];
+    __shared__ double sh_c[1024];
+    double l = 0.0, c = 0.0;
+    for (int i = threadIdx.x; i < n; i += 1024) { l += part[2 * i]; c += part[2 * i + 1]; }
+    sh_l[threadIdx.x] = l;
+    sh_c[threadIdx.x] = c;
+    __syncthreads();
+    for (int off = 512; off > 0; off >>= 1) {
+        if (threadIdx.x < off) {
+            sh_l[threadIdx.x] += sh_l[threadIdx.x + off];
+            sh_c[threadIdx.x] += sh_c[threadIdx.x + off];
+        }
+        __syncthreads();
+    }
+    if (threadIdx.x == 0) {
+        loss_sum[0] = (float)sh_l[0];
+        count[0] = (float)sh_c[0];
+    }
+}
+
 static std::atomic<long long> g_as_launches{0};
 static std::atomic<long long> g_as_fused_launches{0};
+static std::atomic<long long> g_as_ce_launches{0};
 
 static inline bool gemm_as_enabled() {
     static EnvSwitch sw("GAMER_GEMM_AS");
@@ -390,6 +479,7 @@
     if (!gemm_as_enabled() || !a_kc || !b_planes || !d->amax_b) return false;
     if (d->group_mode != 0 || d->resid || d->qk_q_rot) return false;
     if ((d->group_div > 1 || d->sw_tbl) && !d->sw_hm) return false;
+    if (d->sw_colsum_out) return false;
     if (d->norm_x) {
         static EnvSwitch swn("GAMER_GEMM_AS_NORM");
         if (swn.get(1) == 0 || !b_kc || !d->norm_w || !aligned16(d->norm_x) || !aligned16(d->norm_w) || !aligned16(d->A) ||
@@ -400,6 +490,12 @@
         static EnvSwitch swb("GAMER_GEMM_AS_BIAS");
         if (swb.get(1) == 0 || !b_kc || d->sw_hm || d->groups != 1 || d->accumulate || d->bias_rows < 1 ||
             (int64_t)d->bias_rows * d->N * (int64_t)sizeof(float) > 16384)
+            return false;
+    }
+    if (d->ce_labels) {
+        static EnvSwitch swc("GAMER_HEAD_CE");
+        if (swc.get(0) == 0 || !b_kc || !d->norm_x || d->K != 256 || d->groups != 1 || d->accumulate || d->rowdot_out || d->sw_gu ||
+            d->sw_hm || d->bias_idx || d->amax_c)
             return false;
     }
     if (d->sw_hm) {
@@ -469,6 +565,9 @@
     if (norm) { p.A = d->norm_x; p.lda = d->K; }
     p.act_idx = bias ? d->bias_idx : nullptr; p.bias_q = d->bias_q; p.bias_k = d->bias_k; p.bias_v = d->bias_v;
     p.bias_c1 = d->bias_nq; p.bias_c2 = d->bias_nq + d->bias_nkv; p.nb1 = d->bias_rows;
+    const bool ce = b_kc && d->ce_labels;
+    p.ce_labels = ce ? d->ce_labels : nullptr; p.ce_S = d->ce_S; p.ce_ignore = d->ce_ignore_index;
+    p.ce_lse = d->ce_lse; p.ce_row_loss = d->ce_row_loss; p.ce_part = reinterpret_cast<double*>(d->ce_ws);
     const int kp = d->K / 64;
     const size_t shmem = (size_t)(AS_DEPTH == 2 ? 3 : 2) * 2 * kp * AS_PANEL * sizeof(bf16_t) + (d->sw_hm ? (size_t)d->N * sizeof(float) : 0) +
                          (bias ? (size_t)d->bias_rows * d->N * sizeof(float) : 0);
@@ -476,7 +575,14 @@
     const int nw = d->sw_hm ? 4 : (wv.is_set() ? (wv.get(4) == 8 ? 8 : 4) : ((b_kc && d->groups == 1 && d->N >= 512 && AS_WAVES == 4) ? 8 : AS_WAVES));
     const dim3 grid((d->M + 32 * nw - 1) / (32 * nw) + (p.group_offsets ? d->groups : 0));
     int rc;
-    if (b_kc && d->sw_hm) {
+    if (ce) {
+        rc = with_flags([&](auto eight) {
+            return launch<gemm_as_kernel<4, false, 6, eight() ? 8 : 4, true, false>>("gamer_gemm_f32_split/activation-stationary", grid,
+                                                                                     dim3(eight() ? 512 : 256), shmem, st, p); }, nw == 8);
+        if (rc == 0)
+            rc = launch<ce_partials_reduce_kernel>("gamer_gemm_f32_split/head ce reduce", dim3(1), dim3(1024), 0, st, p.ce_part, (int)grid.x,
+                                                   d->ce_loss_sum, d->ce_count);
+    } else if (b_kc && d->sw_hm) {
         switch (kp) {
             case 1: rc = launch_as<1, false, 5>(nw, grid, shmem, st, p); break;
             case 2: rc = launch_as<2, false, 5>(nw, grid, shmem, st, p); break;
@@ -500,6 +606,7 @@
     if (rc) return rc;
     g_as_launches.fetch_add(1, std::memory_order_relaxed);
     if (norm || bias) g_as_fused_launches.fetch_add(1, std::memory_order_relaxed);
+    if (ce) g_as_ce_launches.fetch_add(1, std::memory_order_relaxed);
     return 0;
 }
 
@@ -537,3 +644,4 @@
 
 extern "C" long long gamer_debug_gemm_as_launches(void) { return gamer::g_as_launches.load(std::memory_order_relaxed); }
 extern "C" long long gamer_debug_gemm_as_fused_launches(void) { return gamer::g_as_fused_launches.load(std::memory_order_relaxed); }
+extern "C" long long gamer_debug_gemm_as_ce_launches(void) { return gamer::g_as_ce_launches.load(std::memory_order_relaxed); }
diff --git a/gamer_amd/csrc/inject.hip b/gamer_amd/csrc/inject.hip
--- a/gamer_amd/csrc/inject.hip
+++ b/gamer_amd/csrc/inject.hip
@@ -74,21 +74,22 @@
         partial[(int64_t)blockIdx.x * cols4 + c] = s;
     }
 }
-__global__ void __launch_bounds__(256)
-segment_colsum_reduce_kernel(const float4* __restrict__ partial, int cols4, const int32_t* __restrict__ offsets, int nseg,
+template <int NG>
+__global__ void __launch_bounds__(64 * NG)
+segment_colsum_reduce_kernel(const float4* __restrict__ partial, int cols4, const int32_t* __restrict__ offsets, int nseg, int ch,
                              float4* __restrict__ out) {
-    __shared__ float4 red[4][64];
+    __shared__ float4 red[NG][64];
     const int seg = blockIdx.x;
     int first = 0;
-    for (int s = 0; s < seg; ++s) first += (offsets[s + 1] - offsets[s] + SEG_CH - 1) / SEG_CH;
-    const int n = (offsets[seg + 1] - offsets[seg] + SEG_CH - 1) / SEG_CH;
+    for (int s = 0; s < seg; ++s) first += (offsets[s + 1] - offsets[s] + ch - 1) / ch;
+    const int n = (offsets[seg + 1] - offsets[seg] + ch - 1) / ch;
     const int cl = threadIdx.x & 63, g = threadIdx.x >> 6;
     const int c = blockIdx.y * 64 + cl;
     float4 a = make_float4(0.f, 0.f, 0.f, 0.f), b = a;
     if (c < cols4) {
         int i = g;
-        for (; i + 4 < n; i += 8) {
-            const float4 v = partial[(int64_t)(first + i) * cols4 + c], w = partial[(int64_t)(first + i + 4) * cols4 + c];
+        for (; i + NG < n; i += 2 * NG) {
+            const float4 v = partial[(int64_t)(first + i) * cols4 + c], w = partial[(int64_t)(first + i + NG) * cols4 + c];
             a.x += v.x; a.y += v.y; a.z += v.z; a.w += v.w; b.x += w.x; b.y += w.y; b.z += w.z; b.w += w.w;
         }
         if (i < n) {
@@ -101,7 +102,7 @@
     if (g == 0 && c < cols4) {
         float4 s = red[0][cl];
 #pragma unroll
-        for (int k = 1; k < 4; ++k) { s.x += red[k][cl].x; s.y += red[k][cl].y; s.z += red[k][cl].z; s.w += red[k][cl].w; }
+        for (int k = 1; k < NG; ++k) { s.x += red[k][cl].x; s.y += red[k][cl].y; s.z += red[k][cl].z; s.w += red[k][cl].w; }
         out[(int64_t)seg * cols4 + c] = s;
     }
 }
@@ -199,9 +200,16 @@
     const int wgs = (rows + SEG_CH - 1) / SEG_CH + nseg;
     hipLaunchKernelGGL(segment_colsum_partial_kernel, dim3(wgs), dim3(256), 0, ST(stream), x, ld, cols / 4, offsets, nseg, (float4*)ws);
     GAMER_CHECK_LAUNCH("gamer_segment_colsum/partial");
-    hipLaunchKernelGGL(segment_colsum_reduce_kernel, dim3(nseg, (cols / 4 + 63) / 64), dim3(256), 0, ST(stream), (const float4*)ws,
-                       cols / 4, offsets, nseg, (float4*)out);
+    hipLaunchKernelGGL(segment_colsum_reduce_kernel<4>, dim3(nseg, (cols / 4 + 63) / 64), dim3(256), 0, ST(stream), (const float4*)ws,
+                       cols / 4, offsets, nseg, SEG_CH, (float4*)out);
     GAMER_CHECK_LAUNCH("gamer_segment_colsum/reduce");
+    return 0;
+}
+
+int gamer::launch_segment_colsum_reduce(const float* partial, int cols, const int32_t* offsets, int nseg, int ch, float* out, hipStream_t st) {
+    hipLaunchKernelGGL(segment_colsum_reduce_kernel<16>, dim3(nseg, (cols / 4 + 63) / 64), dim3(1024), 0, st, (const float4*)partial, cols / 4,
+                       offsets, nseg, ch, (float4*)out);
+    GAMER_CHECK_LAUNCH("gamer_gemm_f32/sw_colsum reduce");
     return 0;
 }
 
diff --git a/gamer_amd/engine.py b/gamer_amd/engine.py
--- a/gamer_amd/engine.py
+++ b/gamer_amd/engine.py
@@ -873,13 +873,17 @@
         emb_m = self.shadow.params16["model.embed_tokens.weight"] if c.bf16 else self.params["model.embed_tokens.weight"]
         lab = c.lab
         head_alpha = (1.0 / self.temperature) if (lab is not None and ws.logits.dtype == torch.float32) else 1.0
-        ops.linear_fwd(ws.xn, H, emb_m, H, ws.logits, ws.ldl, c.T, V, H, alpha=head_alpha, **nrm)
+        head_ce = lab is not None and ws.logits.dtype == torch.float32
+        ce = dict(ce=dict(labels=lab, ignore_index=IGNORE_INDEX, lse=ws.lse_ce, row_loss=ws.row_loss, loss_sum=ws.loss_sum,
+                          count=ws.count)) if head_ce else {}
+        ops.linear_fwd(ws.xn, H, emb_m, H, ws.logits, ws.ldl, c.T, V, H, alpha=head_alpha, **nrm, **ce)
         if hidden_sink is not None:
             hidden_sink.append(ws.xn.view(B, S, H).clone())
         loss = None
         if lab is not None:
-            ops.ce_fwd(ws.logits, ws.ldl, lab, V, 1.0 if head_alpha != 1.0 else self.temperature, IGNORE_INDEX, ws.lse_ce,
-                       ws.row_loss, ws.loss_sum, ws.count)
+            if not head_ce:
+                ops.ce_fwd(ws.logits, ws.ldl, lab, V, 1.0 if head_alpha != 1.0 else self.temperature, IGNORE_INDEX, ws.lse_ce,
+                           ws.row_loss, ws.loss_sum, ws.count)
             if torch.is_tensor(num_items_in_batch):
                 num_items_in_batch = num_items_in_batch.to(self.device, torch.float32).reshape(1)
                 loss = ws.loss_sum[0] / num_items_in_batch[0]
@@ -949,8 +953,11 @@
                 with hold(t0):
                     ops.linear_wgrad(t0, H, A["hm"], I, G.down, I, T, H, I, strideC=H * I, **grp)
                     if fuse_swiglu_bwd and split_inj:
+                        seg = ws._buf("inject_segsum", (E * NB1, 2 * I))
+                        seg_ws = ws._buf("inject_seg_ws", (ops.swiglu_bwd_colsum_ws_floats(T, I, E * NB1),))
                         ops.gemm(t0, H, 1, W.down, 1, I, ws.dhm, I, T, I, H, strideB=H * I, p_drop=p_res, seed=self._seed(l, 4),
-                                 swiglu_bwd=(A["gu"], 2 * I), groups=E * NB1, group_offsets=ws.grp_offsets, group_div=NB1, sw_tbl=tb)
+                                 swiglu_bwd=(A["gu"], 2 * I), groups=E * NB1, group_offsets=ws.grp_offsets, group_div=NB1, sw_tbl=tb,
+                                 sw_colsum=(seg_ws, seg))
                     elif fuse_swiglu_bwd:
                         if bf16:
                             ops.linear_dgrad_t(t0, H, WT.down, WT.down.shape[1], ws.dhm, I, T, H, I, strideB=H * I, p_drop=p_res,
@@ -971,9 +978,10 @@
                     with hold(A["gu"]):
                         ops.linear_wgrad(A["gu"], 2 * I, hin, H, G.gu, din, T, 2 * I, H, strideC=2 * I * din, **grp)
                         dgrad(A["gu"], 2 * I, W.gu, None, din, dhin, H, 2 * I, H, strideB=2 * I * din, **grp)
-                    seg = ws._buf("inject_segsum", (E * NB1, 2 * I))
-                    seg_ws = ws._buf("inject_seg_ws", (ops.segment_colsum_ws_floats(T, 2 * I, E * NB1),))
-                    ops.segment_colsum(A["gu"], 2 * I, T, 2 * I, ws.grp_offsets, E * NB1, seg_ws, seg)
+                    if not fuse_swiglu_bwd:
+                        seg = ws._buf("inject_segsum", (E * NB1, 2 * I))
+                        seg_ws = ws._buf("inject_seg_ws", (ops.segment_colsum_ws_floats(T, 2 * I, E * NB1),))
+                        ops.segment_colsum(A["gu"], 2 * I, T, 2 * I, ws.grp_offsets, E * NB1, seg_ws, seg)
                     ops.inject_table_bwd(seg, W.beh, W.gu, din, H, E, 2 * I, G.gu, G.beh,
                                          ws._buf("inject_scratch", (NB1 * E * cfg.behavior_embedding_dim,)))
                     norm_bwd(xlast, W.ln3, dhin, H, G.ln3, True, ws.slot, branch=None if W.cross else (self._seed(l, 1), None))
diff --git a/gamer_amd/ops.py b/gamer_amd/ops.py
--- a/gamer_amd/ops.py
+++ b/gamer_amd/ops.py
@@ -510,6 +510,16 @@
     return t
 
 
+_CE_WS = {}
+
+
+def _ce_workspace(device, floats: int) -> torch.Tensor:
+    t = _CE_WS.get(device)
+    if t is None or t.numel() < floats:
+        t = _CE_WS[device] = torch.empty(int(floats), dtype=torch.float32, device=device)
+    return t
+
+
 class split3_guard:
 
     def __init__(self, on: bool):
@@ -534,12 +544,17 @@
     return prev
 
 
+def swiglu_bwd_colsum_ws_floats(M: int, N: int, groups: int) -> int:
+    return ((M + 127) // 128 + groups) * 2 * N
+
+
 def gemm(A, a_rs, a_ks, Bm, b_rs, b_ks, Cm, ldc, M, N, K, alpha=1.0, accumulate=False, groups=1, group_mode=0,
          group_offsets=None, strideB=0, strideC=0, kchunk=0, resid=None, row_map=None, p_drop=0.0, seed=0,
-         rowdot=None, qknorm=None, c_amax=None, swiglu_bwd=None, group_div=0, sw_tbl=None, swiglu_fwd=None, norm=None, bias=None):
+         rowdot=None, qknorm=None, c_amax=None, swiglu_bwd=None, group_div=0, sw_tbl=None, swiglu_fwd=None, norm=None, bias=None,
+         sw_colsum=None, ce=None):
     if A.dtype == torch.bfloat16:
-        if group_div > 1 or sw_tbl is not None or swiglu_fwd is not None or norm is not None or bias is not None:
-            raise RuntimeError("group_div / sw_tbl / swiglu_fwd / norm / bias are options of the fp32 GEMM")
+        if group_div > 1 or sw_tbl is not None or swiglu_fwd is not None or norm is not None or bias is not None or sw_colsum is not None or ce is not None:
+            raise RuntimeError("group_div / sw_tbl / swiglu_fwd / norm / bias / sw_colsum / ce are options of the fp32 GEMM")
         return _gemm_bf16(A, a_rs, a_ks, Bm, b_rs, b_ks, Cm, ldc, M, N, K, alpha, accumulate, groups, group_mode,
                           group_offsets, strideB, strideC, kchunk, resid, row_map, p_drop, seed, rowdot, qknorm, swiglu_bwd)
     d = GemmDesc()
@@ -577,6 +592,9 @@
         gu, ld_gu = swiglu_bwd
         d.sw_gu, d.sw_ld = ptr(gu), int(ld_gu)
         d.sw_tbl = ptr(sw_tbl)
+        if sw_colsum is not None:
+            cs_ws, cs_out = sw_colsum
+            d.sw_colsum_ws, d.sw_colsum_ws_floats, d.sw_colsum_out = ptr(cs_ws), cs_ws.numel(), ptr(cs_out)
         if _AMAX_REUSE is not None and F32_MATMUL_TERMS == 3 and ld_gu == 2 * N:
             d.amax_c, d.amax_c_col0 = _AMAX_REUSE.preset(gu, (1, 0, 1, M * ld_gu, M * ld_gu)), 0
     d.group_div = int(group_div)
@@ -589,6 +607,14 @@
     if bias is not None:
         d.bias_idx, d.bias_q, d.bias_k, d.bias_v = ptr(bias["idx"]), ptr(bias["q"]), ptr(bias["k"]), ptr(bias["v"])
         d.bias_rows, d.bias_nq, d.bias_nkv = int(bias["q"].shape[0]), int(bias["q"].shape[1]), int(bias["k"].shape[1])
+    if ce is not None:
+        lab = ce["labels"]
+        if lab.dim() != 2 or lab.numel() != M or lab.dtype != torch.int64 or not lab.is_contiguous():
+            raise RuntimeError("gemm(ce=...): labels must be a contiguous int64 [B, S] with B S = M")
+        d.ce_labels, d.ce_S, d.ce_ignore_index = ptr(lab), int(lab.shape[1]), int(ce["ignore_index"])
+        d.ce_lse, d.ce_row_loss, d.ce_loss_sum, d.ce_count = ptr(ce["lse"]), ptr(ce["row_loss"]), ptr(ce["loss_sum"]), ptr(ce["count"])
+        ce_ws = _ce_workspace(A.device, 4 * ((M + 127) // 128))
+        d.ce_ws, d.ce_ws_floats = ce_ws.data_ptr(), ce_ws.numel()
     if swiglu_fwd is not None:
         hm, tbl, row_group = swiglu_fwd
         d.sw_hm, d.sw_tbl, d.sw_row_group = ptr(hm), ptr(tbl), ptr(row_group)
diff --git a/include/gamer_hip.h b/include/gamer_hip.h
--- a/include/gamer_hip.h
+++ b/include/gamer_hip.h
@@ -136,6 +136,18 @@
     const int32_t* bias_idx;
     const float* bias_q; const float* bias_k; const float* bias_v;
     int bias_rows, bias_nq, bias_nkv;
+    float* sw_colsum_out;
+    float* sw_colsum_ws;
+    int64_t sw_colsum_ws_floats;
+    const int64_t* ce_labels;
+    int ce_S;
+    int ce_ignore_index;
+    float* ce_lse;
+    float* ce_row_loss;
+    float* ce_loss_sum;
+    float* ce_count;
+    float* ce_ws;
+    int64_t ce_ws_floats;
 } gamer_gemm_desc;
 
 int gamer_gemm_f32(const gamer_gemm_desc* d, void* stream);
```

Result: no change. 5153 (median of 6 runs) (+0.6%).
